# showlab/VideoSwap

Hardware: NVIDIA H100
Metric: denoise-steps/sec, 16f 512^2 SD1.5 UNet3D (CFG UNet fwd + CFG combine + DDIM step) (higher is better)
Workload: dtype f16

## Files before the change

include/videoswap_b200.h:

```cpp
#ifndef VIDEOSWAP_B200_H
#define VIDEOSWAP_B200_H
#include <stddef.h>
#include <stdint.h>

#ifdef __cplusplus
extern "C" {
#endif

const char* vs_last_error(void);
int vs_version(void);

typedef struct vs_unet_config {
  int in_channels, out_channels;
  int block_out_channels[4];
  int layers_per_block;
  int num_heads;
  int cross_attention_dim;
  int norm_num_groups;
  float norm_eps;
  int use_motion_module;
  int motion_down[4];
  int motion_up[4];
  int motion_mid;
  int motion_num_heads;
  int pe_max_len;
} vs_unet_config;

typedef struct vs_unet vs_unet;

int vs_unet_create(const vs_unet_config* cfg, vs_unet** out);
void vs_unet_destroy(vs_unet* h);

int vs_unet_load_weights(vs_unet* h, void* stream, int n, const char* const* names, const void* const* d_ptrs,
                         const int64_t* numels);
int vs_unet_num_params(const vs_unet* h);
const char* vs_unet_param_name(const vs_unet* h, int i);

int vs_unet_forward(vs_unet* h, void* stream, const void* d_sample, int io_f32, int B, int F, int H, int W,
                    const float* d_timesteps, const void* d_ehs, int ehs_tokens, int ehs_layers,
                    const void* const* d_residuals, int residuals_nhwc, float residual_scale, void* d_out);
int vs_unet_forward_features(vs_unet* h, void* stream, const void* d_sample, int io_f32, int B, int F, int H, int W,
                             const float* d_timesteps, const void* d_ehs, int ehs_tokens, int ehs_layers, int up_ft_index,
                             void* d_feat);
int vs_unet_time_embedding(vs_unet* h, void* stream, const float* d_timesteps, int B, float* d_emb, float* d_proj);
size_t vs_unet_workspace_bytes(const vs_unet* h);
int vs_unet_pin_workspace(vs_unet* h, int pin);
int vs_unet_reserve_workspace(vs_unet* h, int B, int F, int H, int W);
typedef struct vs_comm vs_comm;
int vs_comm_unique_id(void* out128);
int vs_comm_create(const void* id128, int rank, int nranks, vs_comm** out);
void vs_comm_destroy(vs_comm* c);
int vs_comm_all_gather(vs_comm* c, void* stream, const void* d_send, void* d_recv, size_t bytes_per_rank);
int vs_comm_all_reduce_sum_f32(vs_comm* c, void* stream, float* d_buf, size_t n);
int vs_unet_set_frame_shard(vs_unet* h, vs_comm* frame_comm, int shard, int nshards);

typedef void (*vs_attention_hook)(void* user, int layer, int is_cross, int place, void* d_probs, int batch, int heads, int nq,
                                  int nk, void* stream);
int vs_unet_set_attention_hook(vs_unet* h, vs_attention_hook hook, void* user, int max_queries);
int vs_attention_probs(void* stream, const void* d_q, int ldq, const void* d_k, int ldk, void* d_probs, int batch, int nq, int nk,
                       int heads, int d, long long q_bstride, long long kv_bstride, int kv_div);
int vs_attention_apply_probs(void* stream, const void* d_probs, const void* d_v, int ldv, void* d_o, int ldo, int batch, int nq,
                             int nk, int heads, int d, long long kv_bstride, long long o_bstride, int kv_div);
int vs_blend_mask(void* stream, const void* const* d_maps, int n_maps, int n_prompts, int frames, int heads, int res_h, int res_w,
                  int words, const float* d_alpha, int pool, int h, int w, float threshold, int both, float* d_mask);
int vs_latent_blend(void* stream, const void* d_x_src, void* d_x_tgt, const float* d_mask, int io_f32, int channels, int frames,
                    int hw);

int vs_unet_enable_taps(vs_unet* h, int enable);
int vs_unet_num_taps(const vs_unet* h);
int vs_unet_get_tap(const vs_unet* h, int i, const char** name, const void** d_ptr, int* nimg, int* hh, int* ww, int* c);
int vs_unet_copy_tap(const vs_unet* h, void* stream, int i, void* d_dst);

int vs_cfg_ddim_step(void* stream, const void* d_eps2, const void* d_latents, int io_f32, size_t n, int cfg,
                     float guidance, float alpha_t, float alpha_prev, void* d_out);

int vs_cfg_ddim_step_dev(void* stream, const void* d_eps2, const void* d_latents, int io_f32, size_t n, int cfg,
                         float guidance, const float* d_coef, void* d_out);

int vs_adapter_level(void* stream, const void* d_w0, const void* d_b0, const void* d_w1, const void* d_b1, int E, int mid,
                     int C, const float* d_point_embedding, const float* d_tracks, const int* d_point_mask, int F, int P,
                     int h, int w, float rate, int coord_fp16, float scale, float* d_ws, void* d_map);

typedef struct vs_gemm_desc {
  const void* A; int K1; int lda1;
  const void* A2; int K2; int lda2;
  const void* Bw;
  int M, N;
  int taps;
  int sub_py, sub_px;
  int nimg, H, W;
  const float* bias;
  const float* rowvec; int ldrv; int pix_per_batch; int rv_mod;
  const float* ln_stats; const float* ln_u;
  const float* ln_parts; int ln_nparts;
  float* ln_sums_out;
  const void* residual; int ldr;
  void* out; int ldc;
  int mode;
  int force_bn;
  int OH, OW;
  int stride2;
} vs_gemm_desc;
int vs_gemm_ex(void* stream, const vs_gemm_desc* desc);
int vs_pack_conv3x3(void* stream, const void* d_w, int cout, int cin, void* d_out);
int vs_pack_geglu(void* stream, const void* d_w, const void* d_b, int hidden, int K, void* d_wout, float* d_bout);
int vs_groupnorm(void* stream, const void* d_x1, int c1, const void* d_x2, int c2, int nimg, int hw, int imgs_per_set,
                 int groups, float eps, const float* d_gamma, const float* d_beta, int silu, float* d_sums, void* d_out);
int vs_groupnorm_stats(void* stream, const void* d_x1, int c1, const void* d_x2, int c2, int nimg, int hw, int imgs_per_set,
                       int groups, float* d_sums, int zero_first);
int vs_groupnorm_apply(void* stream, const void* d_x1, int c1, const void* d_x2, int c2, int nimg, int hw, int imgs_per_set,
                       int groups, const float* d_sums, float eps, const float* d_gamma, const float* d_beta, int silu,
                       int count_scale, void* d_out);
int vs_layernorm(void* stream, const void* d_x, int rows, int C, const float* d_gamma, const float* d_beta,
                 const float* d_pe, int hw, int F, void* d_out);
int vs_ln_linear(void* stream, const void* d_x, int M, int C, const void* d_w, const float* d_bias, int N,
                 const float* d_gamma, const float* d_beta, const float* d_pe, int pe_len, int hw, int frames, int mode,
                 void* d_wf, float* d_u, float* d_c, float* d_cpe, float* d_stats, void* d_out);
int vs_linear_ln_linear(void* stream, const void* d_x0, int M, int K0, const void* d_w0, const float* d_b0,
                        const void* d_residual, int C, void* d_x, const void* d_w, const float* d_bias, int N,
                        const float* d_gamma, const float* d_beta, const float* d_pe, int pe_len, int hw, int frames,
                        int mode, void* d_wf, float* d_u, float* d_c, float* d_cpe, float* d_parts, int parts_capacity,
                        void* d_out);
int vs_attention(void* stream, const void* d_q, int ldq, const void* d_k, int ldk, const void* d_v, int ldv, void* d_o,
                 int ldo, int batch, int nq, int nk, int heads, int d, long long q_bstride, long long kv_bstride,
                 long long o_bstride, int kv_div);
int vs_temporal_attention(void* stream, const void* d_qkv, void* d_o, int B, int F, int HW, int C, int heads);
int vs_conv_in(void* stream, const void* d_x, int nimg, int H, int W, int cin, const void* d_w, const float* d_bias,
               int cout, void* d_scratch, void* d_out);
int vs_upsample2x(void* stream, const void* d_x, int nimg, int H, int W, int C, void* d_out);
int vs_upsample_conv3x3(void* stream, const void* d_x, int nimg, int H, int W, int C, const void* d_w, int Cout,
                        const float* d_bias, void* d_wsub, void* d_out);
int vs_upsample_conv3x3_sized(void* stream, const void* d_x, int nimg, int H, int W, int C, const void* d_w, int Cout,
                              const float* d_bias, int OH, int OW, void* d_wpanels, void* d_out);
int vs_upsample_nearest(void* stream, const void* d_x, int nimg, int H, int W, int C, int OH, int OW, void* d_out);
int vs_conv3x3_s2(void* stream, const void* d_x, int nimg, int H, int W, int C, const void* d_w_packed, int Cout,
                  const float* d_bias, void* d_scratch, void* d_out);

int vs_pack_conv_subpixel(void* stream, const void* d_w, int cout, int cin, void* d_out);
int vs_softmax_rows(void* stream, void* d_s, int rows, int n, int ld, float scale);
int vs_transpose_pad(void* stream, const void* d_src, int rows, int cols, int rows_pad, void* d_dst);
int vs_vae_latent_in(void* stream, const void* d_z, int z_is_f32, int nimg, int h, int w, float divisor, const float* d_wb,
                     void* d_out);
int vs_image_postprocess(void* stream, const void* d_x, int nimg, int H, int W, int channels, int format, void* d_out);

int vs_downsample_conv3x3(void* stream, const void* d_x, int nimg, int H, int W, int C, const void* d_w_packed, int Cout,
                          const float* d_bias, void* d_out);
int vs_vae_image_in(void* stream, const void* d_x, int src_format, int nimg, int H, int W, void* d_out);
int vs_vae_moments(void* stream, const void* d_x, int nimg, int h, int w, const float* d_wb, void* d_out);
int vs_vae_posterior(void* stream, const void* d_params, const void* d_noise, int nimg, int h, int w, float scale, int layout,
                     void* d_out);

int vs_clip_embed(void* stream, const int* d_ids_i32, int n, int L, const void* d_tok, int vocab, const void* d_pos, int C,
                  void* d_out);
int vs_causal_attention(void* stream, const void* d_qkv, int ldqkv, void* d_o, int ldo, int nseq, int L, int heads, int d);

int vs_dift_noise(void* stream, const void* d_moments, const float* d_eps1, const float* d_eps2, int n, int E, int h, int w,
                  float sf, float sqrt_a, float sqrt_1ma, float* d_out);
int vs_dift_point_sample(void* stream, const void* d_feat, int n, int E, int h, int w, int C, int H, int W, const int* d_xy,
                         int P, float* d_out);
int vs_dift_ensemble_mean(void* stream, const void* d_feat, int n, int E, int h, int w, int C, float* d_out);
int vs_dift_point_reduce(void* stream, const float* d_vecs, int n, int P, int C, const float* d_src, const int* d_src_row,
                         float* d_conf, const void* d_accept, float* d_sums, float* d_counts, float* d_means);

typedef struct vs_imlp_desc {
  const float* d_params;
  int input_dim;
  int output_dim;
  int hidden_dim;
  int mlp_layers;
  int pe_dim;
  uint32_t skip_mask;
  int use_tanh;
} vs_imlp_desc;
int vs_imlp_forward(void* stream, const vs_imlp_desc* net, const float* d_x, int rows, float* d_out);
int vs_atlas_propagate(void* stream, const vs_imlp_desc* fg, const vs_imlp_desc* fg_inverse, const vs_imlp_desc* alpha,
                       const float* d_points, float t_key, int P, int F, int larger_dim, float* d_ws, float* d_tracks);

int vs_profile_enable(int on);
int vs_profile_reset(void);
int vs_profile_collect(int category, double* ms, double* work, long long* count);
long long vs_launch_count(void);
int vs_profile_dump(const char* path);
int vs_set_option(const char* name, int value);

#ifdef __cplusplus
}
#endif
#endif
```

videoswap_b200/_lib.py:

```python
from __future__ import annotations

import ctypes as C
import os
import re

HERE = os.path.dirname(os.path.abspath(__file__))
LIB_PATH = os.path.join(HERE, "libvideoswap_b200.so")
HEADER_PATH = os.path.join(os.path.dirname(HERE), "include", "videoswap_b200.h")


class VSError(RuntimeError):
    pass


class UNetConfigStruct(C.Structure):
    _fields_ = [
        ("in_channels", C.c_int), ("out_channels", C.c_int), ("block_out_channels", C.c_int * 4),
        ("layers_per_block", C.c_int), ("num_heads", C.c_int), ("cross_attention_dim", C.c_int),
        ("norm_num_groups", C.c_int), ("norm_eps", C.c_float), ("use_motion_module", C.c_int),
        ("motion_down", C.c_int * 4), ("motion_up", C.c_int * 4), ("motion_mid", C.c_int),
        ("motion_num_heads", C.c_int), ("pe_max_len", C.c_int),
    ]


_P = C.c_void_p
_I = C.c_int
_F = C.c_float
_LL = C.c_longlong
_SZ = C.c_size_t


class ImlpDescStruct(C.Structure):
    _fields_ = [("params", _P), ("input_dim", _I), ("output_dim", _I), ("hidden_dim", _I), ("mlp_layers", _I),
                ("pe_dim", _I), ("skip_mask", C.c_uint32), ("use_tanh", _I)]


class GemmDescStruct(C.Structure):
    _fields_ = [
        ("A", _P), ("K1", _I), ("lda1", _I),
        ("A2", _P), ("K2", _I), ("lda2", _I),
        ("Bw", _P),
        ("M", _I), ("N", _I),
        ("taps", _I),
        ("sub_py", _I), ("sub_px", _I),
        ("nimg", _I), ("H", _I), ("W", _I),
        ("bias", _P),
        ("rowvec", _P), ("ldrv", _I), ("pix_per_batch", _I), ("rv_mod", _I),
        ("ln_stats", _P), ("ln_u", _P),
        ("ln_parts", _P), ("ln_nparts", _I),
        ("ln_sums_out", _P),
        ("residual", _P), ("ldr", _I),
        ("out", _P), ("ldc", _I),
        ("mode", _I),
        ("force_bn", _I),
        ("OH", _I), ("OW", _I),
        ("stride2", _I),
    ]

_SIGNATURES = {
    "vs_last_error": (C.c_char_p, []),
    "vs_version": (_I, []),
    "vs_unet_create": (_I, [C.POINTER(UNetConfigStruct), C.POINTER(_P)]),
    "vs_unet_destroy": (None, [_P]),
    "vs_unet_load_weights": (_I, [_P, _P, _I, C.POINTER(C.c_char_p), C.POINTER(_P), C.POINTER(C.c_int64)]),
    "vs_unet_num_params": (_I, [_P]),
    "vs_unet_param_name": (C.c_char_p, [_P, _I]),
    "vs_unet_forward": (_I, [_P, _P, _P, _I, _I, _I, _I, _I, _P, _P, _I, _I, C.POINTER(_P), _I, _F, _P]),
    "vs_unet_time_embedding": (_I, [_P, _P, _P, _I, _P, _P]),
    "vs_unet_workspace_bytes": (_SZ, [_P]),
    "vs_unet_pin_workspace": (_I, [_P, _I]),
    "vs_unet_reserve_workspace": (_I, [_P, _I, _I, _I, _I]),
    "vs_comm_unique_id": (_I, [_P]),
    "vs_comm_create": (_I, [_P, _I, _I, C.POINTER(_P)]),
    "vs_comm_destroy": (None, [_P]),
    "vs_comm_all_gather": (_I, [_P, _P, _P, _P, _SZ]),
    "vs_comm_all_reduce_sum_f32": (_I, [_P, _P, _P, _SZ]),
    "vs_unet_set_frame_shard": (_I, [_P, _P, _I, _I]),
    "vs_unet_enable_taps": (_I, [_P, _I]),
    "vs_unet_num_taps": (_I, [_P]),
    "vs_unet_get_tap": (_I, [_P, _I, C.POINTER(C.c_char_p), C.POINTER(_P), C.POINTER(_I), C.POINTER(_I), C.POINTER(_I),
                             C.POINTER(_I)]),
    "vs_unet_copy_tap": (_I, [_P, _P, _I, _P]),
    "vs_profile_enable": (_I, [_I]),
    "vs_profile_reset": (_I, []),
    "vs_profile_collect": (_I, [_I, C.POINTER(C.c_double), C.POINTER(C.c_double), C.POINTER(C.c_longlong)]),
    "vs_launch_count": (C.c_longlong, []),
    "vs_set_option": (_I, [C.c_char_p, _I]),
    "vs_profile_dump": (_I, [C.c_char_p]),
    "vs_cfg_ddim_step": (_I, [_P, _P, _P, _I, _SZ, _I, _F, _F, _F, _P]),
    "vs_cfg_ddim_step_dev": (_I, [_P, _P, _P, _I, _SZ, _I, _F, _P, _P]),
    "vs_adapter_level": (_I, [_P, _P, _P, _P, _P, _I, _I, _I, _P, _P, _P, _I, _I, _I, _I, _F, _I, _F, _P, _P]),
    "vs_gemm_ex": (_I, [_P, C.POINTER(GemmDescStruct)]),
    "vs_pack_conv3x3": (_I, [_P, _P, _I, _I, _P]),
    "vs_pack_geglu": (_I, [_P, _P, _P, _I, _I, _P, _P]),
    "vs_groupnorm": (_I, [_P, _P, _I, _P, _I, _I, _I, _I, _I, _F, _P, _P, _I, _P, _P]),
    "vs_groupnorm_stats": (_I, [_P, _P, _I, _P, _I, _I, _I, _I, _I, _P, _I]),
    "vs_groupnorm_apply": (_I, [_P, _P, _I, _P, _I, _I, _I, _I, _I, _P, _F, _P, _P, _I, _I, _P]),
    "vs_layernorm": (_I, [_P, _P, _I, _I, _P, _P, _P, _I, _I, _P]),
    "vs_ln_linear": (_I, [_P, _P, _I, _I, _P, _P, _I, _P, _P, _P, _I, _I, _I, _I, _P, _P, _P, _P, _P, _P]),
    "vs_unet_set_attention_hook": (_I, [_P, _P, _P, _I]),
    "vs_attention_probs": (_I, [_P, _P, _I, _P, _I, _P, _I, _I, _I, _I, _I, _LL, _LL, _I]),
    "vs_attention_apply_probs": (_I, [_P, _P, _P, _I, _P, _I, _I, _I, _I, _I, _I, _LL, _LL, _I]),
    "vs_blend_mask": (_I, [_P, _P, _I, _I, _I, _I, _I, _I, _I, _P, _I, _I, _I, _F, _I, _P]),
    "vs_latent_blend": (_I, [_P, _P, _P, _P, _I, _I, _I, _I]),
    "vs_linear_ln_linear": (_I, [_P, _P, _I, _I, _P, _P, _P, _I, _P, _P, _P, _I, _P, _P, _P, _I, _I, _I, _I, _P, _P, _P, _P,
                                 _P, _I, _P]),
    "vs_attention": (_I, [_P, _P, _I, _P, _I, _P, _I, _P, _I, _I, _I, _I, _I, _I, _LL, _LL, _LL, _I]),
    "vs_temporal_attention": (_I, [_P, _P, _P, _I, _I, _I, _I, _I]),
    "vs_conv_in": (_I, [_P, _P, _I, _I, _I, _I, _P, _P, _I, _P, _P]),
    "vs_upsample2x": (_I, [_P, _P, _I, _I, _I, _I, _P]),
    "vs_upsample_conv3x3": (_I, [_P, _P, _I, _I, _I, _I, _P, _I, _P, _P, _P]),
    "vs_upsample_conv3x3_sized": (_I, [_P, _P, _I, _I, _I, _I, _P, _I, _P, _I, _I, _P, _P]),
    "vs_upsample_nearest": (_I, [_P, _P, _I, _I, _I, _I, _I, _I, _P]),
    "vs_conv3x3_s2": (_I, [_P, _P, _I, _I, _I, _I, _P, _I, _P, _P, _P]),
    "vs_pack_conv_subpixel": (_I, [_P, _P, _I, _I, _P]),
    "vs_softmax_rows": (_I, [_P, _P, _I, _I, _I, _F]),
    "vs_transpose_pad": (_I, [_P, _P, _I, _I, _I, _P]),
    "vs_vae_latent_in": (_I, [_P, _P, _I, _I, _I, _I, _F, _P, _P]),
    "vs_image_postprocess": (_I, [_P, _P, _I, _I, _I, _I, _I, _P]),
    "vs_downsample_conv3x3": (_I, [_P, _P, _I, _I, _I, _I, _P, _I, _P, _P]),
    "vs_vae_image_in": (_I, [_P, _P, _I, _I, _I, _I, _P]),
    "vs_vae_moments": (_I, [_P, _P, _I, _I, _I, _P, _P]),
    "vs_vae_posterior": (_I, [_P, _P, _P, _I, _I, _I, _F, _I, _P]),
    "vs_clip_embed": (_I, [_P, _P, _I, _I, _P, _I, _P, _I, _P]),
    "vs_causal_attention": (_I, [_P, _P, _I, _P, _I, _I, _I, _I, _I]),
    "vs_unet_forward_features": (_I, [_P, _P, _P, _I, _I, _I, _I, _I, _P, _P, _I, _I, _I, _P]),
    "vs_dift_noise": (_I, [_P, _P, _P, _P, _I, _I, _I, _I, _F, _F, _F, _P]),
    "vs_dift_point_sample": (_I, [_P, _P, _I, _I, _I, _I, _I, _I, _I, _P, _I, _P]),
    "vs_dift_ensemble_mean": (_I, [_P, _P, _I, _I, _I, _I, _I, _P]),
    "vs_dift_point_reduce": (_I, [_P, _P, _I, _I, _I, _P, _P, _P, _P, _P, _P, _P]),
    "vs_imlp_forward": (_I, [_P, C.POINTER(ImlpDescStruct), _P, _I, _P]),
    "vs_atlas_propagate": (_I, [_P, C.POINTER(ImlpDescStruct), C.POINTER(ImlpDescStruct), C.POINTER(ImlpDescStruct), _P, _F,
                                _I, _I, _I, _P, _P]),
}

_lib = None


def header_symbols():
    with open(HEADER_PATH) as f:
        text = f.read()
    text = re.sub(r"/\*.*?\*/", "", text, flags=re.S)
    return sorted(set(re.findall(r"\b(vs_[a-z0-9_]+)\s*\(", text)))


def lib() -> C.CDLL:
    global _lib
    if _lib is None:
        if not os.path.exists(LIB_PATH):
            raise VSError(f"{LIB_PATH} is missing: build it with `python -m videoswap_b200.build` "
                          f"(there is no CPU/PyTorch fallback for this path)")
        _lib = C.CDLL(LIB_PATH)
        for name, (res, args) in _SIGNATURES.items():
            fn = getattr(_lib, name)
            fn.restype = res
            fn.argtypes = args
    return _lib


def check(code: int, what: str = ""):
    if code != 0:
        msg = lib().vs_last_error()
        raise VSError(f"{what or 'videoswap_b200 call'} failed ({code}): {msg.decode() if msg else '?'}")


def call(name: str, *args):
    check(getattr(lib(), name)(*args), name)
```

videoswap_b200/build.py:

```python
from __future__ import annotations

import os
import shutil
import subprocess
import sys
from concurrent.futures import ThreadPoolExecutor

HERE = os.path.dirname(os.path.abspath(__file__))
CSRC = os.path.join(HERE, "csrc")
LIB = os.path.join(HERE, "libvideoswap_b200.so")
SOURCES = ["runtime.cu", "gemm.cu", "norm.cu", "attention.cu", "attention_tc.cu", "pointwise.cu", "unet.cu", "api.cu", "comm.cu", "text.cu", "dift.cu", "atlas.cu"]
ARCH = ["-gencode", "arch=compute_90a,code=sm_90a"]
NVCC_FLAGS = ARCH + ["-lineinfo", "-O3", "-std=c++17", "-Xcompiler", "-fPIC",
              "--use_fast_math" if False else "-DVS_NO_FAST_MATH"]


def _nvcc() -> str:
    for cand in (os.environ.get("NVCC"), shutil.which("nvcc"), "/usr/local/cuda/bin/nvcc"):
        if cand and os.path.exists(cand):
            return cand
    raise RuntimeError("nvcc not found")


def _stale(target: str, deps) -> bool:
    if not os.path.exists(target):
        return True
    t = os.path.getmtime(target)
    return any(os.path.getmtime(d) > t for d in deps)


def build(force: bool = False, verbose: bool = False) -> str:
    nvcc = _nvcc()
    objdir = os.path.join(HERE, "build")
    os.makedirs(objdir, exist_ok=True)
    headers = [os.path.join(CSRC, f) for f in os.listdir(CSRC) if f.endswith((".h", ".cuh"))]
    headers.append(os.path.join(os.path.dirname(HERE), "include", "videoswap_b200.h"))

    def compile_one(src):
        obj = os.path.join(objdir, src.replace(".cu", ".o"))
        if force or _stale(obj, [os.path.join(CSRC, src)] + headers):
            cmd = [nvcc] + NVCC_FLAGS + ["-c", os.path.join(CSRC, src), "-o", obj]
            if verbose:
                print(" ".join(cmd))
            r = subprocess.run(cmd, capture_output=True, text=True)
            if r.returncode != 0:
                raise RuntimeError(f"nvcc failed on {src}:\n{r.stdout}\n{r.stderr}")
        return obj

    with ThreadPoolExecutor(max_workers=min(8, len(SOURCES))) as ex:
        objs = list(ex.map(compile_one, SOURCES))
    if force or _stale(LIB, objs):
        cmd = [nvcc, "-shared", "-o", LIB] + objs + ARCH + ["-Xcompiler", "-fPIC", "-ldl"]
        r = subprocess.run(cmd, capture_output=True, text=True)
        if r.returncode != 0:
            raise RuntimeError(f"link failed:\n{r.stdout}\n{r.stderr}")
    return LIB


if __name__ == "__main__":
    print(build(force="--force" in sys.argv, verbose=True))
```

videoswap_b200/csrc/api.cu:

```cuda
#include "../../include/videoswap_b200.h"
#include "common.cuh"
#include "kernels.h"

using namespace vs;

extern "C" const char* vs_last_error(void) { return vs::last_error(); }
extern "C" int vs_version(void) { return 100; }

extern "C" int vs_cfg_ddim_step(void* stream, const void* d_eps2, const void* d_latents, int io_f32, size_t n, int cfg,
                                float guidance, float alpha_t, float alpha_prev, void* d_out) {
  VS_REQUIRE(d_eps2 && d_latents && d_out, "vs_cfg_ddim_step: null pointer");
  VS_REQUIRE(alpha_t > 0.f && alpha_t <= 1.f && alpha_prev > 0.f && alpha_prev <= 1.f, "vs_cfg_ddim_step: alphas must be in (0,1]");
  return cfg_ddim_step((cudaStream_t)stream, d_eps2, d_latents, io_f32, n, cfg, guidance, alpha_t, alpha_prev, d_out);
}

extern "C" int vs_cfg_ddim_step_dev(void* stream, const void* d_eps2, const void* d_latents, int io_f32, size_t n, int cfg,
                                    float guidance, const float* d_coef, void* d_out) {
  VS_REQUIRE(d_eps2 && d_latents && d_out && d_coef, "vs_cfg_ddim_step_dev: null pointer");
  return cfg_ddim_step_dev((cudaStream_t)stream, d_eps2, d_latents, io_f32, n, cfg, guidance, d_coef, d_out);
}

extern "C" int vs_adapter_level(void* stream, const void* d_w0, const void* d_b0, const void* d_w1, const void* d_b1, int E,
                                int mid, int C, const float* d_pe, const float* d_tracks, const int* d_mask, int F, int P,
                                int h, int w, float rate, int coord_fp16, float scale, float* d_ws, void* d_map) {
  cudaStream_t st = (cudaStream_t)stream;
  VS_REQUIRE(d_w0 && d_b0 && d_w1 && d_b1 && d_pe && d_tracks && d_ws && d_map, "vs_adapter_level: null pointer");
  float* b0 = d_ws;
  float* b1 = b0 + mid;
  float* hid = b1 + C;
  float* feat = hid + (size_t)P * mid;
  if (int e = f16_to_f32(st, (const __half*)d_b0, mid, b0)) return e;
  if (int e = f16_to_f32(st, (const __half*)d_b1, C, b1)) return e;
  if (int e = small_linear(st, d_pe, P, E, (const __half*)d_w0, b0, mid, false, true, hid)) return e;
  if (int e = small_linear(st, hid, P, mid, (const __half*)d_w1, b1, C, false, false, feat)) return e;
  return adapter_splat(st, feat, d_tracks, d_mask, F, P, C, h, w, rate, coord_fp16, scale, (__half*)d_map);
}

extern "C" int vs_gemm_ex(void* stream, const vs_gemm_desc* d) {
  VS_REQUIRE(d != nullptr, "vs_gemm_ex: null descriptor");
  GemmArgs g;
  g.A = (const __half*)d->A; g.K1 = d->K1; g.lda1 = d->lda1;
  g.A2 = (const __half*)d->A2; g.K2 = d->K2; g.lda2 = d->lda2;
  g.Bw = (const __half*)d->Bw;
  g.M = d->M; g.N = d->N;
  g.taps = d->taps;
  g.sub_py = d->sub_py; g.sub_px = d->sub_px;
  g.nimg = d->nimg; g.H = d->H; g.W = d->W;
  g.bias = d->bias;
  g.rowvec = d->rowvec; g.ldrv = d->ldrv; g.pix_per_batch = d->pix_per_batch; g.rv_mod = d->rv_mod;
  g.ln_stats = d->ln_stats; g.ln_u = d->ln_u;
  g.ln_parts = d->ln_parts; g.ln_nparts = d->ln_nparts;
  g.ln_sums_out = d->ln_sums_out;
  g.residual = (const __half*)d->residual; g.ldr = d->ldr;
  g.out = (__half*)d->out; g.ldc = d->ldc;
  g.mode = d->mode;
  g.force_bn = d->force_bn;
  g.OH = d->OH; g.OW = d->OW;
  g.stride2 = d->stride2;
  return gemm_tc((cudaStream_t)stream, g);
}

extern "C" int vs_pack_conv3x3(void* stream, const void* d_w, int cout, int cin, void* d_out) {
  return pack_conv3x3((cudaStream_t)stream, (const __half*)d_w, cout, cin, (__half*)d_out);
}
extern "C" int vs_pack_geglu(void* stream, const void* d_w, const void* d_b, int hidden, int K, void* d_wout, float* d_bout) {
  cudaStream_t st = (cudaStream_t)stream;
  if (int e = pack_geglu(st, (const __half*)d_w, nullptr, hidden, K, kGegluGranule, (__half*)d_wout, nullptr)) return e;
  return pack_geglu(st, nullptr, (const __half*)d_b, hidden, 1, kGegluGranule, nullptr, d_bout);
}

extern "C" int vs_groupnorm(void* stream, const void* d_x1, int c1, const void* d_x2, int c2, int nimg, int hw,
                            int imgs_per_set, int groups, float eps, const float* d_gamma, const float* d_beta, int silu,
                            float* d_sums, void* d_out) {
  cudaStream_t st = (cudaStream_t)stream;
  if (imgs_per_set == 1 && c2 == 0) {
    const int e = groupnorm_frame_fused(st, (const __half*)d_x1, c1, nimg, hw, groups, eps, d_gamma, d_beta, silu != 0, (__half*)d_out);
    if (e >= 0) return e;
  }
  if (int e = groupnorm_stats(st, (const __half*)d_x1, c1, (const __half*)d_x2, c2, nimg, hw, imgs_per_set, groups, d_sums)) return e;
  return groupnorm_apply(st, (const __half*)d_x1, c1, (const __half*)d_x2, c2, nimg, hw, imgs_per_set, groups, d_sums, eps,
                         d_gamma, d_beta, silu != 0, (__half*)d_out);
}
extern "C" int vs_groupnorm_stats(void* stream, const void* d_x1, int c1, const void* d_x2, int c2, int nimg, int hw,
                                  int imgs_per_set, int groups, float* d_sums, int zero_first) {
  VS_REQUIRE(d_sums != nullptr, "vs_groupnorm_stats: null sums");
  return groupnorm_stats((cudaStream_t)stream, (const __half*)d_x1, c1, (const __half*)d_x2, c2, nimg, hw, imgs_per_set, groups,
                         d_sums, zero_first != 0);
}
extern "C" int vs_groupnorm_apply(void* stream, const void* d_x1, int c1, const void* d_x2, int c2, int nimg, int hw,
                                  int imgs_per_set, int groups, const float* d_sums, float eps, const float* d_gamma,
                                  const float* d_beta, int silu, int count_scale, void* d_out) {
  VS_REQUIRE(d_sums && d_out, "vs_groupnorm_apply: null pointer");
  VS_REQUIRE(count_scale >= 1, "vs_groupnorm_apply: count_scale must be >= 1");
  return groupnorm_apply((cudaStream_t)stream, (const __half*)d_x1, c1, (const __half*)d_x2, c2, nimg, hw, imgs_per_set, groups,
                         d_sums, eps, d_gamma, d_beta, silu != 0, (__half*)d_out, count_scale);
}
extern "C" int vs_layernorm(void* stream, const void* d_x, int rows, int C, const float* d_gamma, const float* d_beta,
                            const float* d_pe, int hw, int F, void* d_out) {
  return layernorm((cudaStream_t)stream, (const __half*)d_x, rows, C, d_gamma, d_beta, d_pe, hw, F, (__half*)d_out);
}
extern "C" int vs_ln_linear(void* stream, const void* d_x, int M, int C, const void* d_w, const float* d_bias, int N,
                            const float* d_gamma, const float* d_beta, const float* d_pe, int pe_len, int hw, int frames,
                            int mode, void* d_wf, float* d_u, float* d_c, float* d_cpe, float* d_stats, void* d_out) {
  cudaStream_t st = (cudaStream_t)stream;
  if (int e = ln_fold(st, (const __half*)d_w, N, C, d_gamma, d_beta, d_bias, d_pe, pe_len, (__half*)d_wf, d_u, d_c, d_cpe)) return e;
  if (int e = ln_rowstats(st, (const __half*)d_x, M, C, d_stats)) return e;
  GemmArgs g;
  g.A = (const __half*)d_x; g.K1 = C; g.lda1 = C; g.Bw = (const __half*)d_wf; g.M = M; g.N = N; g.bias = d_c;
  g.ln_stats = d_stats; g.ln_u = d_u; g.out = (__half*)d_out; g.ldc = mode == EPI_GEGLU ? N / 2 : N; g.mode = mode;
  if (d_pe) { g.rowvec = d_cpe; g.ldrv = N; g.pix_per_batch = hw; g.rv_mod = frames; }
  return gemm_tc(st, g);
}
extern "C" int vs_upsample_conv3x3(void* stream, const void* d_x, int nimg, int H, int W, int C, const void* d_w, int Cout,
                                   const float* d_bias, void* d_wsub, void* d_out) {
  cudaStream_t st = (cudaStream_t)stream;
  if (int e = pack_conv_subpixel(st, (const __half*)d_w, Cout, C, (__half*)d_wsub)) return e;
  for (int par = 0; par < 4; ++par) {
    GemmArgs g;
    g.A = (const __half*)d_x; g.K1 = C; g.lda1 = C; g.Bw = (const __half*)d_wsub + (size_t)par * Cout * 4 * C; g.taps = 4;
    g.sub_py = par >> 1; g.sub_px = par & 1; g.nimg = nimg; g.H = H; g.W = W; g.M = nimg * H * W; g.N = Cout; g.bias = d_bias;
    g.out = (__half*)d_out; g.ldc = Cout;
    if (int e = gemm_tc(st, g)) return e;
  }
  return 0;
}
extern "C" int vs_upsample_conv3x3_sized(void* stream, const void* d_x, int nimg, int H, int W, int C, const void* d_w, int Cout,
                                         const float* d_bias, int OH, int OW, void* d_wpanels, void* d_out) {
  cudaStream_t st = (cudaStream_t)stream;
  VS_REQUIRE(d_x && d_w && d_wpanels && d_out && nimg >= 1 && H >= 1 && W >= 1, "vs_upsample_conv3x3_sized: bad arguments");
  __half* w3x3 = (__half*)d_wpanels;
  __half* wsub = w3x3 + (size_t)Cout * 9 * C;
  if (int e = pack_conv3x3(st, (const __half*)d_w, Cout, C, w3x3)) return e;
  if (int e = pack_conv_subpixel(st, (const __half*)d_w, Cout, C, wsub, true)) return e;
  return upsample_conv3x3(st, (const __half*)d_x, nimg, H, W, C, w3x3, wsub, d_bias, Cout, OH, OW, (__half*)d_out);
}
extern "C" int vs_upsample_nearest(void* stream, const void* d_x, int nimg, int H, int W, int C, int OH, int OW, void* d_out) {
  return upsample_nearest2x((cudaStream_t)stream, (const __half*)d_x, nimg, H, W, C, (__half*)d_out, OH, OW);
}
extern "C" int vs_attention_probs(void* stream, const void* d_q, int ldq, const void* d_k, int ldk, void* d_probs, int batch, int nq,
                                  int nk, int heads, int d, long long q_bstride, long long kv_bstride, int kv_div) {
  return attention_probs((cudaStream_t)stream, (const __half*)d_q, ldq, (const __half*)d_k, ldk, (__half*)d_probs, batch, nq, nk, heads,
                         d, q_bstride, kv_bstride, kv_div);
}
extern "C" int vs_attention_apply_probs(void* stream, const void* d_probs, const void* d_v, int ldv, void* d_o, int ldo, int batch,
                                        int nq, int nk, int heads, int d, long long kv_bstride, long long o_bstride, int kv_div) {
  return attention_apply_probs((cudaStream_t)stream, (const __half*)d_probs, (const __half*)d_v, ldv, (__half*)d_o, ldo, batch, nq, nk,
                               heads, d, kv_bstride, o_bstride, kv_div);
}
extern "C" int vs_blend_mask(void* stream, const void* const* d_maps, int n_maps, int n_prompts, int frames, int heads, int res_h,
                             int res_w, int words, const float* d_alpha, int pool, int h, int w, float threshold, int both,
                             float* d_mask) {
  const int res[2] = {res_h, res_w};
  return blend_mask((cudaStream_t)stream, (const __half* const*)d_maps, res, n_maps, n_prompts, frames, heads, words, d_alpha, pool, h, w,
                    threshold, both, d_mask);
}
extern "C" int vs_latent_blend(void* stream, const void* d_x_src, void* d_x_tgt, const float* d_mask, int io_f32, int channels,
                               int frames, int hw) {
  return latent_blend((cudaStream_t)stream, d_x_src, d_x_tgt, d_mask, io_f32, channels, frames, hw);
}
extern "C" int vs_linear_ln_linear(void* stream, const void* d_x0, int M, int K0, const void* d_w0, const float* d_b0,
                                   const void* d_residual, int C, void* d_x, const void* d_w, const float* d_bias, int N,
                                   const float* d_gamma, const float* d_beta, const float* d_pe, int pe_len, int hw,
                                   int frames, int mode, void* d_wf, float* d_u, float* d_c, float* d_cpe, float* d_parts,
                                   int parts_capacity, void* d_out) {
  cudaStream_t st = (cudaStream_t)stream;
  if (int e = ln_fold(st, (const __half*)d_w, N, C, d_gamma, d_beta, d_bias, d_pe, pe_len, (__half*)d_wf, d_u, d_c, d_cpe)) return e;
  GemmArgs g0;
  g0.A = (const __half*)d_x0; g0.K1 = K0; g0.lda1 = K0; g0.Bw = (const __half*)d_w0; g0.M = M; g0.N = C; g0.bias = d_b0;
  g0.residual = (const __half*)d_residual; g0.ldr = C; g0.out = (__half*)d_x; g0.ldc = C; g0.ln_sums_out = d_parts;
  const int parts = gemm_n_tiles(g0);
  VS_REQUIRE(parts >= 1 && parts <= parts_capacity, "vs_linear_ln_linear: %d partial-sum slices do not fit the buffer (%d)", parts, parts_capacity);
  if (int e = gemm_tc(st, g0)) return e;
  GemmArgs g;
  g.A = (const __half*)d_x; g.K1 = C; g.lda1 = C; g.Bw = (const __half*)d_wf; g.M = M; g.N = N; g.bias = d_c;
  g.ln_parts = d_parts; g.ln_nparts = parts; g.ln_u = d_u; g.out = (__half*)d_out; g.ldc = mode == EPI_GEGLU ? N / 2 : N; g.mode = mode;
  if (d_pe) { g.rowvec = d_cpe; g.ldrv = N; g.pix_per_batch = hw; g.rv_mod = frames; }
  return gemm_tc(st, g);
}
extern "C" int vs_attention(void* stream, const void* d_q, int ldq, const void* d_k, int ldk, const void* d_v, int ldv,
                            void* d_o, int ldo, int batch, int nq, int nk, int heads, int d, long long q_bstride,
                            long long kv_bstride, long long o_bstride, int kv_div) {
  return attention((cudaStream_t)stream, (const __half*)d_q, ldq, (const __half*)d_k, ldk, (const __half*)d_v, ldv,
                   (__half*)d_o, ldo, batch, nq, nk, heads, d, q_bstride, kv_bstride, o_bstride, kv_div);
}
extern "C" int vs_temporal_attention(void* stream, const void* d_qkv, void* d_o, int B, int F, int HW, int C, int heads) {
  return temporal_attention((cudaStream_t)stream, (const __half*)d_qkv, (__half*)d_o, B, F, HW, C, heads);
}
extern "C" int vs_conv_in(void* stream, const void* d_x, int nimg, int H, int W, int cin, const void* d_w, const float* d_bias,
                          int cout, void* d_scratch, void* d_out) {
  return conv_in_3x3((cudaStream_t)stream, (const __half*)d_x, nimg, H, W, cin, (const __half*)d_w, d_bias, cout, (__half*)d_out,
                     (__half*)d_scratch);
}
extern "C" int vs_upsample2x(void* stream, const void* d_x, int nimg, int H, int W, int C, void* d_out) {
  return upsample_nearest2x((cudaStream_t)stream, (const __half*)d_x, nimg, H, W, C, (__half*)d_out);
}
extern "C" int vs_conv3x3_s2(void* stream, const void* d_x, int nimg, int H, int W, int C, const void* d_w, int Cout,
                             const float* d_bias, void* d_scratch, void* d_out) {
  cudaStream_t st = (cudaStream_t)stream;
  if (int e = im2col_s2(st, (const __half*)d_x, nimg, H, W, C, (__half*)d_scratch)) return e;
  const int Ho = (H - 1) / 2 + 1, Wo = (W - 1) / 2 + 1;
  GemmArgs g;
  g.A = (const __half*)d_scratch; g.K1 = 9 * C; g.lda1 = 9 * C; g.Bw = (const __half*)d_w; g.M = nimg * Ho * Wo; g.N = Cout;
  g.bias = d_bias; g.out = (__half*)d_out; g.ldc = Cout;
  return gemm_tc(st, g);
}

extern "C" int vs_pack_conv_subpixel(void* stream, const void* d_w, int cout, int cin, void* d_out) {
  VS_REQUIRE(d_w && d_out, "vs_pack_conv_subpixel: null pointer");
  return pack_conv_subpixel((cudaStream_t)stream, (const __half*)d_w, cout, cin, (__half*)d_out);
}
extern "C" int vs_softmax_rows(void* stream, void* d_s, int rows, int n, int ld, float scale) {
  return softmax_rows((cudaStream_t)stream, (__half*)d_s, rows, n, ld, scale);
}
extern "C" int vs_transpose_pad(void* stream, const void* d_src, int rows, int cols, int rows_pad, void* d_dst) {
  return transpose_pad((cudaStream_t)stream, (const __half*)d_src, rows, cols, rows_pad, (__half*)d_dst);
}
extern "C" int vs_vae_latent_in(void* stream, const void* d_z, int z_is_f32, int nimg, int h, int w, float divisor,
                                const float* d_wb, void* d_out) {
  return vae_latent_in((cudaStream_t)stream, d_z, z_is_f32, nimg, h, w, divisor, d_wb, (__half*)d_out);
}
extern "C" int vs_image_postprocess(void* stream, const void* d_x, int nimg, int H, int W, int channels, int format, void* d_out) {
  return image_postprocess((cudaStream_t)stream, (const __half*)d_x, nimg, H, W, channels, format, d_out);
}
extern "C" int vs_downsample_conv3x3(void* stream, const void* d_x, int nimg, int H, int W, int C, const void* d_w_packed,
                                     int Cout, const float* d_bias, void* d_out) {
  VS_REQUIRE(d_x && d_w_packed && d_out, "vs_downsample_conv3x3: null pointer");
  GemmArgs g;
  g.A = (const __half*)d_x; g.K1 = C; g.lda1 = C; g.Bw = (const __half*)d_w_packed; g.taps = 9; g.stride2 = 1;
  g.nimg = nimg; g.H = H; g.W = W; g.M = nimg * (H / 2) * (W / 2); g.N = Cout; g.bias = d_bias; g.out = (__half*)d_out;
  g.ldc = Cout;
  return gemm_tc((cudaStream_t)stream, g);
}
extern "C" int vs_vae_image_in(void* stream, const void* d_x, int src_format, int nimg, int H, int W, void* d_out) {
  return vae_image_in((cudaStream_t)stream, d_x, src_format, nimg, H, W, (__half*)d_out);
}
extern "C" int vs_vae_moments(void* stream, const void* d_x, int nimg, int h, int w, const float* d_wb, void* d_out) {
  return vae_moments((cudaStream_t)stream, (const __half*)d_x, nimg, h, w, d_wb, (__half*)d_out);
}
extern "C" int vs_vae_posterior(void* stream, const void* d_params, const void* d_noise, int nimg, int h, int w, float scale,
                                int layout, void* d_out) {
  return vae_posterior((cudaStream_t)stream, (const __half*)d_params, (const __half*)d_noise, nimg, h, w, scale, layout,
                       (__half*)d_out);
}
extern "C" int vs_clip_embed(void* stream, const int* d_ids_i32, int n, int L, const void* d_tok, int vocab, const void* d_pos, int C,
                             void* d_out) {
  return clip_embed((cudaStream_t)stream, d_ids_i32, n, L, (const __half*)d_tok, vocab, (const __half*)d_pos, C, (__half*)d_out);
}
extern "C" int vs_causal_attention(void* stream, const void* d_qkv, int ldqkv, void* d_o, int ldo, int nseq, int L, int heads,
                                   int d) {
  return causal_attention((cudaStream_t)stream, (const __half*)d_qkv, ldqkv, (__half*)d_o, ldo, nseq, L, heads, d);
}

extern "C" int vs_dift_noise(void* stream, const void* d_moments, const float* d_eps1, const float* d_eps2, int n, int E, int h,
                             int w, float sf, float sqrt_a, float sqrt_1ma, float* d_out) {
  return dift_noise((cudaStream_t)stream, (const __half*)d_moments, d_eps1, d_eps2, n, E, h, w, sf, sqrt_a, sqrt_1ma, d_out);
}
extern "C" int vs_dift_point_sample(void* stream, const void* d_feat, int n, int E, int h, int w, int C, int H, int W,
                                    const int* d_xy, int P, float* d_out) {
  return dift_point_sample((cudaStream_t)stream, (const __half*)d_feat, n, E, h, w, C, H, W, d_xy, P, d_out);
}
extern "C" int vs_dift_ensemble_mean(void* stream, const void* d_feat, int n, int E, int h, int w, int C, float* d_out) {
  return dift_ensemble_mean((cudaStream_t)stream, (const __half*)d_feat, n, E, h, w, C, d_out);
}
extern "C" int vs_dift_point_reduce(void* stream, const float* d_vecs, int n, int P, int C, const float* d_src,
                                    const int* d_src_row, float* d_conf, const void* d_accept, float* d_sums, float* d_counts,
                                    float* d_means) {
  return dift_point_reduce((cudaStream_t)stream, d_vecs, n, P, C, d_src, d_src_row, d_conf, (const uint8_t*)d_accept, d_sums,
                           d_counts, d_means);
}

extern "C" int vs_profile_enable(int on) { prof_enable(on != 0); return 0; }
extern "C" int vs_profile_reset(void) { prof_reset(); return 0; }
extern "C" int vs_profile_collect(int category, double* ms, double* work, long long* count) {
  VS_REQUIRE(category >= 0 && category < PC_COUNT && ms && work && count, "vs_profile_collect: bad argument");
  return prof_collect(category, ms, work, count);
}
extern "C" long long vs_launch_count(void) { return launch_count(); }
extern "C" int vs_profile_dump(const char* path) {
  VS_REQUIRE(path != nullptr, "vs_profile_dump: null path");
  return prof_dump(path);
}
extern "C" int vs_set_option(const char* name, int value) {
  VS_REQUIRE(name != nullptr, "vs_set_option: null name");
  return set_option(name, value);
}
```

videoswap_b200/csrc/attention.cu:

```cuda
#include "common.cuh"
#include "kernels.h"

namespace vs {
namespace {

__device__ __forceinline__ void cp_async16(uint32_t dst, const void* src, bool pred) {
  const int sz = pred ? 16 : 0;
  asm volatile("cp.async.cg.shared.global [%0], [%1], 16, %2;" ::"r"(dst), "l"(src), "r"(sz) : "memory");
}
__device__ __forceinline__ void cp_async_commit() { asm volatile("cp.async.commit_group;" ::: "memory"); }
template <int N>
__device__ __forceinline__ void cp_async_wait() {
  asm volatile("cp.async.wait_group %0;" ::"n"(N) : "memory");
}
__device__ __forceinline__ void ldsm_x4(uint32_t addr, uint32_t& r0, uint32_t& r1, uint32_t& r2, uint32_t& r3) {
  asm volatile("ldmatrix.sync.aligned.m8n8.x4.shared.b16 {%0,%1,%2,%3}, [%4];"
               : "=r"(r0), "=r"(r1), "=r"(r2), "=r"(r3)
               : "r"(addr));
}
__device__ __forceinline__ void ldsm_x4_t(uint32_t addr, uint32_t& r0, uint32_t& r1, uint32_t& r2, uint32_t& r3) {
  asm volatile("ldmatrix.sync.aligned.m8n8.x4.trans.shared.b16 {%0,%1,%2,%3}, [%4];"
               : "=r"(r0), "=r"(r1), "=r"(r2), "=r"(r3)
               : "r"(addr));
}
__device__ __forceinline__ void mma16816(float* c, const uint32_t* a, uint32_t b0, uint32_t b1) {
  asm volatile(
      "mma.sync.aligned.m16n8k16.row.col.f32.f16.f16.f32 {%0,%1,%2,%3}, {%4,%5,%6,%7}, {%8,%9}, {%0,%1,%2,%3};"
      : "+f"(c[0]), "+f"(c[1]), "+f"(c[2]), "+f"(c[3])
      : "r"(a[0]), "r"(a[1]), "r"(a[2]), "r"(a[3]), "r"(b0), "r"(b1));
}
__device__ __forceinline__ uint32_t pack_h2(float a, float b) {
  __half2 h = __floats2half2_rn(a, b);
  return *reinterpret_cast<uint32_t*>(&h);
}

template <int DP, int NT>
__device__ __forceinline__ void warp_qk(float (*s)[4], uint32_t q_s, uint32_t k_s, int lds_bytes, int lane) {
#pragma unroll
  for (int n = 0; n < NT; ++n) s[n][0] = s[n][1] = s[n][2] = s[n][3] = 0.f;
#pragma unroll
  for (int kk = 0; kk < DP / 16; ++kk) {
    uint32_t a[4];
    ldsm_x4(q_s + (lane & 15) * lds_bytes + (kk * 16 + (lane >> 4) * 8) * 2, a[0], a[1], a[2], a[3]);
#pragma unroll
    for (int n = 0; n < NT; n += 2) {
      uint32_t b0, b1, b2, b3;
      const int key = n * 8 + (lane & 7) + ((lane >> 4) ? 8 : 0);
      const int ch = kk * 16 + (((lane >> 3) & 1) ? 8 : 0);
      ldsm_x4(k_s + key * lds_bytes + ch * 2, b0, b1, b2, b3);
      mma16816(s[n], a, b0, b1);
      mma16816(s[n + 1], a, b2, b3);
    }
  }
}

template <int NT, int ON>
__device__ __forceinline__ void warp_pv(float (*o)[4], const float (*s)[4], uint32_t v_s, int lds_bytes, int lane) {
#pragma unroll
  for (int kt = 0; kt < NT / 2; ++kt) {
    uint32_t a[4];
    a[0] = pack_h2(s[2 * kt][0], s[2 * kt][1]);
    a[1] = pack_h2(s[2 * kt][2], s[2 * kt][3]);
    a[2] = pack_h2(s[2 * kt + 1][0], s[2 * kt + 1][1]);
    a[3] = pack_h2(s[2 * kt + 1][2], s[2 * kt + 1][3]);
#pragma unroll
    for (int n = 0; n < ON; n += 2) {
      uint32_t b0, b1, b2, b3;
      const int key = kt * 16 + (lane & 7) + (((lane >> 3) & 1) ? 8 : 0);
      const int ch = n * 8 + ((lane >> 4) ? 8 : 0);
      ldsm_x4_t(v_s + key * lds_bytes + ch * 2, b0, b1, b2, b3);
      mma16816(o[n], a, b0, b1);
      mma16816(o[n + 1], a, b2, b3);
    }
  }
}

struct AttnParams {
  const __half* q; const __half* k; const __half* v; __half* o;
  int ldq, ldk, ldv, ldo;
  long long q_bs, kv_bs, o_bs;
  int nq, nk, kv_div;
  float scale_log2;
};

template <int D>
struct ACfg {
  static constexpr int DP = (D + 15) / 16 * 16;
  static constexpr int LDS = DP + 8;
  static constexpr int BQ = 64, BKV = 64;
  static constexpr int SMEM = (BQ + 4 * BKV) * LDS * 2;
};

template <int D>
__device__ __forceinline__ void load_rows(uint32_t dst, const __half* src, int ld, int row0, int nrows_valid, int tid,
                                          int nthreads) {
  using C = ACfg<D>;
  constexpr int CH = C::DP / 8;
  for (int i = tid; i < 64 * CH; i += nthreads) {
    const int r = i / CH, c = i % CH;
    const bool ok = (row0 + r < nrows_valid) && (c * 8 < D);
    const __half* s = ok ? src + (long long)(row0 + r) * ld + c * 8 : src;
    cp_async16(dst + (r * C::LDS + c * 8) * 2, s, ok);
  }
}

template <int D>
__global__ void __launch_bounds__(128) attn_kernel(const AttnParams p) {
  using C = ACfg<D>;
  pdl_trigger();
  pdl_wait();
  constexpr int DP = C::DP, LDSB = C::LDS * 2, NT = C::BKV / 8, ON = DP / 8;
  extern __shared__ __align__(16) uint8_t smem[];
  const uint32_t q_s = smem_u32(smem);
  const uint32_t k_s0 = q_s + C::BQ * LDSB;
  const uint32_t v_s0 = k_s0 + 2 * C::BKV * LDSB;
  const int tid = threadIdx.x, warp = tid >> 5, lane = tid & 31;
  const int qt = blockIdx.x, h = blockIdx.y, b = blockIdx.z;
  const __half* qp = p.q + b * p.q_bs + h * D;
  const __half* kp = p.k + (b / p.kv_div) * p.kv_bs + h * D;
  const __half* vp = p.v + (b / p.kv_div) * p.kv_bs + h * D;
  const int nkt = (p.nk + C::BKV - 1) / C::BKV;

  load_rows<D>(q_s, qp, p.ldq, qt * C::BQ, p.nq, tid, 128);
  load_rows<D>(k_s0, kp, p.ldk, 0, p.nk, tid, 128);
  load_rows<D>(v_s0, vp, p.ldv, 0, p.nk, tid, 128);
  cp_async_commit();

  float o[ON][4];
#pragma unroll
  for (int n = 0; n < ON; ++n) o[n][0] = o[n][1] = o[n][2] = o[n][3] = 0.f;
  float m0 = -INFINITY, m1 = -INFINITY, l0 = 0.f, l1 = 0.f;

  for (int j = 0; j < nkt; ++j) {
    cp_async_wait<0>();
    __syncthreads();
    if (j + 1 < nkt) {
      const int nb = (j + 1) & 1;
      load_rows<D>(k_s0 + nb * C::BKV * LDSB, kp, p.ldk, (j + 1) * C::BKV, p.nk, tid, 128);
      load_rows<D>(v_s0 + nb * C::BKV * LDSB, vp, p.ldv, (j + 1) * C::BKV, p.nk, tid, 128);
      cp_async_commit();
    }
    const uint32_t k_s = k_s0 + (j & 1) * C::BKV * LDSB;
    const uint32_t v_s = v_s0 + (j & 1) * C::BKV * LDSB;
    float s[NT][4];
    warp_qk<DP, NT>(s, q_s + warp * 16 * LDSB, k_s, LDSB, lane);
    const int kbase = j * C::BKV;
    if (kbase + C::BKV > p.nk) {
#pragma unroll
      for (int n = 0; n < NT; ++n) {
        const int c = kbase + n * 8 + (lane & 3) * 2;
        if (c >= p.nk) s[n][0] = s[n][2] = -INFINITY;
        if (c + 1 >= p.nk) s[n][1] = s[n][3] = -INFINITY;
      }
    }
    float mx0 = m0, mx1 = m1;
#pragma unroll
    for (int n = 0; n < NT; ++n) {
      mx0 = fmaxf(mx0, fmaxf(s[n][0], s[n][1]));
      mx1 = fmaxf(mx1, fmaxf(s[n][2], s[n][3]));
    }
    mx0 = fmaxf(mx0, __shfl_xor_sync(0xffffffffu, mx0, 1));
    mx0 = fmaxf(mx0, __shfl_xor_sync(0xffffffffu, mx0, 2));
    mx1 = fmaxf(mx1, __shfl_xor_sync(0xffffffffu, mx1, 1));
    mx1 = fmaxf(mx1, __shfl_xor_sync(0xffffffffu, mx1, 2));
    const float c0 = exp2f((m0 - mx0) * p.scale_log2), c1 = exp2f((m1 - mx1) * p.scale_log2);
    m0 = mx0; m1 = mx1;
    const float ms0 = mx0 * p.scale_log2, ms1 = mx1 * p.scale_log2;
    float rs0 = 0.f, rs1 = 0.f;
#pragma unroll
    for (int n = 0; n < NT; ++n) {
      s[n][0] = exp2f(s[n][0] * p.scale_log2 - ms0);
      s[n][1] = exp2f(s[n][1] * p.scale_log2 - ms0);
      s[n][2] = exp2f(s[n][2] * p.scale_log2 - ms1);
      s[n][3] = exp2f(s[n][3] * p.scale_log2 - ms1);
      rs0 += s[n][0] + s[n][1];
      rs1 += s[n][2] + s[n][3];
    }
    l0 = l0 * c0 + rs0;
    l1 = l1 * c1 + rs1;
#pragma unroll
    for (int n = 0; n < ON; ++n) {
      o[n][0] *= c0; o[n][1] *= c0; o[n][2] *= c1; o[n][3] *= c1;
    }
    warp_pv<NT, ON>(o, s, v_s, LDSB, lane);
  }
  l0 += __shfl_xor_sync(0xffffffffu, l0, 1);
  l0 += __shfl_xor_sync(0xffffffffu, l0, 2);
  l1 += __shfl_xor_sync(0xffffffffu, l1, 1);
  l1 += __shfl_xor_sync(0xffffffffu, l1, 2);
  const float i0 = 1.f / l0, i1 = 1.f / l1;
  const int r0 = qt * C::BQ + warp * 16 + (lane >> 2), r1 = r0 + 8;
  __half* op = p.o + b * p.o_bs + h * D;
#pragma unroll
  for (int n = 0; n < ON; ++n) {
    const int c = n * 8 + (lane & 3) * 2;
    if (c < D) {
      if (r0 < p.nq) *reinterpret_cast<__half2*>(op + (long long)r0 * p.ldo + c) = __floats2half2_rn(o[n][0] * i0, o[n][1] * i0);
      if (r1 < p.nq) *reinterpret_cast<__half2*>(op + (long long)r1 * p.ldo + c) = __floats2half2_rn(o[n][2] * i1, o[n][3] * i1);
    }
  }
}

template <int D>
int launch_attn(cudaStream_t st, const AttnParams& p, int batch, int heads) {
  using C = ACfg<D>;
  static bool configured = false;
  if (!configured) {
    VS_CHECK_CUDA(cudaFuncSetAttribute(attn_kernel<D>, cudaFuncAttributeMaxDynamicSharedMemorySize, C::SMEM));
    configured = true;
  }
  dim3 grid((p.nq + C::BQ - 1) / C::BQ, heads, batch);
  ProfScope prof(st, PC_ATTN, 4.0 * batch * heads * (double)p.nq * p.nk * D);
  return launch_pdl(attn_kernel<D>, grid, dim3(128), C::SMEM, st, 1, p);
}

template <int D>
__global__ void __launch_bounds__(128) attn_probs_kernel(const AttnParams p, __half* __restrict__ probs, int heads) {
  using C = ACfg<D>;
  constexpr int DP = C::DP, LDSB = C::LDS * 2, NT = C::BKV / 8;
  extern __shared__ __align__(16) uint8_t smem[];
  const uint32_t q_s = smem_u32(smem);
  const uint32_t k_s0 = q_s + C::BQ * LDSB;
  const int tid = threadIdx.x, warp = tid >> 5, lane = tid & 31;
  const int qt = blockIdx.x, h = blockIdx.y, b = blockIdx.z;
  const __half* qp = p.q + b * p.q_bs + h * D;
  const __half* kp = p.k + (b / p.kv_div) * p.kv_bs + h * D;
  const int nkt = (p.nk + C::BKV - 1) / C::BKV;
  load_rows<D>(q_s, qp, p.ldq, qt * C::BQ, p.nq, tid, 128);
  float m0 = -INFINITY, m1 = -INFINITY, l0 = 0.f, l1 = 0.f, i0 = 0.f, i1 = 0.f;
  const int r0 = qt * C::BQ + warp * 16 + (lane >> 2), r1 = r0 + 8;
  __half* prow0 = probs + (((long long)b * heads + h) * p.nq + r0) * p.nk;
  __half* prow1 = prow0 + 8LL * p.nk;
  for (int pass = 0; pass < 2; ++pass) {
    load_rows<D>(k_s0, kp, p.ldk, 0, p.nk, tid, 128);
    cp_async_commit();
    for (int j = 0; j < nkt; ++j) {
      cp_async_wait<0>();
      __syncthreads();
      if (j + 1 < nkt) {
        load_rows<D>(k_s0 + ((j + 1) & 1) * C::BKV * LDSB, kp, p.ldk, (j + 1) * C::BKV, p.nk, tid, 128);
        cp_async_commit();
      }
      float s[NT][4];
      warp_qk<DP, NT>(s, q_s + warp * 16 * LDSB, k_s0 + (j & 1) * C::BKV * LDSB, LDSB, lane);
      const int kbase = j * C::BKV;
      if (pass == 0) {
        float mx0 = m0, mx1 = m1;
#pragma unroll
        for (int n = 0; n < NT; ++n) {
          const int c = kbase + n * 8 + (lane & 3) * 2;
          if (c >= p.nk) s[n][0] = s[n][2] = -INFINITY;
          if (c + 1 >= p.nk) s[n][1] = s[n][3] = -INFINITY;
          mx0 = fmaxf(mx0, fmaxf(s[n][0], s[n][1]));
          mx1 = fmaxf(mx1, fmaxf(s[n][2], s[n][3]));
        }
        mx0 = fmaxf(mx0, __shfl_xor_sync(0xffffffffu, mx0, 1));
        mx0 = fmaxf(mx0, __shfl_xor_sync(0xffffffffu, mx0, 2));
        mx1 = fmaxf(mx1, __shfl_xor_sync(0xffffffffu, mx1, 1));
        mx1 = fmaxf(mx1, __shfl_xor_sync(0xffffffffu, mx1, 2));
        float rs0 = 0.f, rs1 = 0.f;
#pragma unroll
        for (int n = 0; n < NT; ++n) {
          rs0 += exp2f((s[n][0] - mx0) * p.scale_log2) + exp2f((s[n][1] - mx0) * p.scale_log2);
          rs1 += exp2f((s[n][2] - mx1) * p.scale_log2) + exp2f((s[n][3] - mx1) * p.scale_log2);
        }
        l0 = l0 * exp2f((m0 - mx0) * p.scale_log2) + rs0;
        l1 = l1 * exp2f((m1 - mx1) * p.scale_log2) + rs1;
        m0 = mx0; m1 = mx1;
      } else {
#pragma unroll
        for (int n = 0; n < NT; ++n) {
          const int c = kbase + n * 8 + (lane & 3) * 2;
          if (r0 < p.nq) {
            if (c < p.nk) prow0[c] = __float2half_rn(exp2f((s[n][0] - m0) * p.scale_log2) * i0);
            if (c + 1 < p.nk) prow0[c + 1] = __float2half_rn(exp2f((s[n][1] - m0) * p.scale_log2) * i0);
          }
          if (r1 < p.nq) {
            if (c < p.nk) prow1[c] = __float2half_rn(exp2f((s[n][2] - m1) * p.scale_log2) * i1);
            if (c + 1 < p.nk) prow1[c + 1] = __float2half_rn(exp2f((s[n][3] - m1) * p.scale_log2) * i1);
          }
        }
      }
      __syncthreads();
    }
    if (pass == 0) {
      l0 += __shfl_xor_sync(0xffffffffu, l0, 1);
      l0 += __shfl_xor_sync(0xffffffffu, l0, 2);
      l1 += __shfl_xor_sync(0xffffffffu, l1, 1);
      l1 += __shfl_xor_sync(0xffffffffu, l1, 2);
      i0 = 1.f / l0; i1 = 1.f / l1;
    }
  }
}

template <int D>
__global__ void __launch_bounds__(128) attn_pv_kernel(const AttnParams p, const __half* __restrict__ probs, int heads) {
  using C = ACfg<D>;
  constexpr int DP = C::DP, LDSB = C::LDS * 2, ON = DP / 8, LDP = C::BKV + 8, LDPB = LDP * 2;
  extern __shared__ __align__(16) uint8_t smem[];
  const uint32_t p_s = smem_u32(smem);
  const uint32_t v_s = p_s + C::BQ * LDPB;
  __half* p_sm = reinterpret_cast<__half*>(smem);
  const int tid = threadIdx.x, warp = tid >> 5, lane = tid & 31;
  const int qt = blockIdx.x, h = blockIdx.y, b = blockIdx.z;
  const __half* vp = p.v + (b / p.kv_div) * p.kv_bs + h * D;
  const __half* pb = probs + (((long long)b * heads + h) * p.nq) * p.nk;
  const int nkt = (p.nk + C::BKV - 1) / C::BKV;
  float o[ON][4];
#pragma unroll
  for (int n = 0; n < ON; ++n) o[n][0] = o[n][1] = o[n][2] = o[n][3] = 0.f;
  for (int j = 0; j < nkt; ++j) {
    __syncthreads();
    load_rows<D>(v_s, vp, p.ldv, j * C::BKV, p.nk, tid, 128);
    cp_async_commit();
    for (int e = tid; e < C::BQ * C::BKV; e += 128) {
      const int r = e / C::BKV, c = e % C::BKV;
      const int q = qt * C::BQ + r, k = j * C::BKV + c;
      p_sm[r * LDP + c] = (q < p.nq && k < p.nk) ? pb[(long long)q * p.nk + k] : __float2half(0.f);
    }
    cp_async_wait<0>();
    __syncthreads();
#pragma unroll
    for (int kt = 0; kt < C::BKV / 16; ++kt) {
      uint32_t a[4];
      ldsm_x4(p_s + (warp * 16 + (lane & 15)) * LDPB + (kt * 16 + (lane >> 4) * 8) * 2, a[0], a[1], a[2], a[3]);
#pragma unroll
      for (int n = 0; n < ON; n += 2) {
        uint32_t b0, b1, b2, b3;
        const int key = kt * 16 + (lane & 7) + (((lane >> 3) & 1) ? 8 : 0);
        const int ch = n * 8 + ((lane >> 4) ? 8 : 0);
        ldsm_x4_t(v_s + key * LDSB + ch * 2, b0, b1, b2, b3);
        mma16816(o[n], a, b0, b1);
        mma16816(o[n + 1], a, b2, b3);
      }
    }
  }
  const int r0 = qt * C::BQ + warp * 16 + (lane >> 2), r1 = r0 + 8;
  __half* op = p.o + b * p.o_bs + h * D;
#pragma unroll
  for (int n = 0; n < ON; ++n) {
    const int c = n * 8 + (lane & 3) * 2;
    if (c < D) {
      if (r0 < p.nq) *reinterpret_cast<__half2*>(op + (long long)r0 * p.ldo + c) = __floats2half2_rn(o[n][0], o[n][1]);
      if (r1 < p.nq) *reinterpret_cast<__half2*>(op + (long long)r1 * p.ldo + c) = __floats2half2_rn(o[n][2], o[n][3]);
    }
  }
}

template <int D>
int launch_explicit(cudaStream_t st, const AttnParams& p, __half* probs, int batch, int heads, bool apply) {
  using C = ACfg<D>;
  constexpr int SMEM_P = (C::BQ + 2 * C::BKV) * C::LDS * 2;
  constexpr int SMEM_V = C::BQ * (C::BKV + 8) * 2 + C::BKV * C::LDS * 2;
  static bool configured = false;
  if (!configured) {
    VS_CHECK_CUDA(cudaFuncSetAttribute(attn_probs_kernel<D>, cudaFuncAttributeMaxDynamicSharedMemorySize, SMEM_P));
    VS_CHECK_CUDA(cudaFuncSetAttribute(attn_pv_kernel<D>, cudaFuncAttributeMaxDynamicSharedMemorySize, SMEM_V));
    configured = true;
  }
  dim3 grid((p.nq + C::BQ - 1) / C::BQ, heads, batch);
  ProfScope prof(st, PC_ATTN, 2.0 * batch * heads * (double)p.nq * p.nk * D);
  if (apply) attn_pv_kernel<D><<<grid, 128, SMEM_V, st>>>(p, probs, heads);
  else attn_probs_kernel<D><<<grid, 128, SMEM_P, st>>>(p, probs, heads);
  count_launch(1);
  VS_CHECK_CUDA(cudaGetLastError());
  return 0;
}

struct TAttnParams {
  const __half* qkv; __half* o;
  int B, F, HW, C, heads;
  float scale_log2;
  long long items;
};

template <int D, int FP, bool VST = true>
__global__ void __launch_bounds__(128) tattn_kernel(const TAttnParams p) {
  pdl_trigger();
  pdl_wait();
  constexpr int DP = (D + 15) / 16 * 16, LDS = DP + 8, LDSB = LDS * 2, CH = DP / 8;
  constexpr int MT = FP / 16, NT = FP / 8, ON = DP / 8;
  extern __shared__ __align__(16) uint8_t smem[];
  const int warp = threadIdx.x >> 5, lane = threadIdx.x & 31;
  const long long item = (long long)blockIdx.x * 4 + warp;
  if (item >= p.items) return;
  const int head = item % p.heads;
  const long long bp = item / p.heads;
  const int pix = bp % p.HW;
  const int b = bp / p.HW;
  const uint32_t base = smem_u32(smem) + warp * (3 * FP * LDSB);
  const uint32_t q_s = base, k_s = base + FP * LDSB, v_s = base + 2 * FP * LDSB;
  const long long row_stride = (long long)p.HW * 3 * p.C;
  const __half* src = p.qkv + ((long long)b * p.F * p.HW + pix) * 3 * p.C + head * D;
  for (int i = lane; i < 3 * FP * CH; i += 32) {
    const int sec = i / (FP * CH), rem = i % (FP * CH), f = rem / CH, c = rem % CH;
    const bool ok = (f < p.F) && (c * 8 < D);
    const __half* s = ok ? src + f * row_stride + sec * p.C + c * 8 : src;
    cp_async16(base + sec * FP * LDSB + (f * LDS + c * 8) * 2, s, ok);
  }
  cp_async_commit();
  cp_async_wait<0>();
  __syncwarp();
  __half* dst = p.o + ((long long)b * p.F * p.HW + pix) * p.C + head * D;
  const long long orow = (long long)p.HW * p.C;
#pragma unroll
  for (int mt = 0; mt < MT; ++mt) {
    float s[NT][4];
    warp_qk<DP, NT>(s, q_s + mt * 16 * LDSB, k_s, LDSB, lane);
    float mx0 = -INFINITY, mx1 = -INFINITY;
#pragma unroll
    for (int n = 0; n < NT; ++n) {
      const int c = n * 8 + (lane & 3) * 2;
      if (c >= p.F) s[n][0] = s[n][2] = -INFINITY;
      if (c + 1 >= p.F) s[n][1] = s[n][3] = -INFINITY;
      mx0 = fmaxf(mx0, fmaxf(s[n][0], s[n][1]));
      mx1 = fmaxf(mx1, fmaxf(s[n][2], s[n][3]));
    }
    mx0 = fmaxf(mx0, __shfl_xor_sync(0xffffffffu, mx0, 1));
    mx0 = fmaxf(mx0, __shfl_xor_sync(0xffffffffu, mx0, 2));
    mx1 = fmaxf(mx1, __shfl_xor_sync(0xffffffffu, mx1, 1));
    mx1 = fmaxf(mx1, __shfl_xor_sync(0xffffffffu, mx1, 2));
    const float ms0 = mx0 * p.scale_log2, ms1 = mx1 * p.scale_log2;
    float l0 = 0.f, l1 = 0.f;
#pragma unroll
    for (int n = 0; n < NT; ++n) {
      s[n][0] = exp2f(s[n][0] * p.scale_log2 - ms0);
      s[n][1] = exp2f(s[n][1] * p.scale_log2 - ms0);
      s[n][2] = exp2f(s[n][2] * p.scale_log2 - ms1);
      s[n][3] = exp2f(s[n][3] * p.scale_log2 - ms1);
      l0 += s[n][0] + s[n][1];
      l1 += s[n][2] + s[n][3];
    }
    l0 += __shfl_xor_sync(0xffffffffu, l0, 1);
    l0 += __shfl_xor_sync(0xffffffffu, l0, 2);
    l1 += __shfl_xor_sync(0xffffffffu, l1, 1);
    l1 += __shfl_xor_sync(0xffffffffu, l1, 2);
    float o[ON][4];
#pragma unroll
    for (int n = 0; n < ON; ++n) o[n][0] = o[n][1] = o[n][2] = o[n][3] = 0.f;
    warp_pv<NT, ON>(o, s, v_s, LDSB, lane);
    const float i0 = 1.f / l0, i1 = 1.f / l1;
    const int f0 = mt * 16 + (lane >> 2), f1 = f0 + 8;
    if (VST) {
      __syncwarp();
      __half* stage = reinterpret_cast<__half*>(smem) + (size_t)warp * (3 * FP * LDS) + (size_t)mt * 16 * LDS;
#pragma unroll
      for (int n = 0; n < ON; ++n) {
        const int c = n * 8 + (lane & 3) * 2;
        *reinterpret_cast<__half2*>(stage + (lane >> 2) * LDS + c) = __floats2half2_rn(o[n][0] * i0, o[n][1] * i0);
        *reinterpret_cast<__half2*>(stage + ((lane >> 2) + 8) * LDS + c) = __floats2half2_rn(o[n][2] * i1, o[n][3] * i1);
      }
      __syncwarp();
      constexpr int VCH = D / 8;
      for (int e = lane; e < 16 * VCH; e += 32) {
        const int fr = e / VCH, ch = e % VCH, f = mt * 16 + fr;
        if (f < p.F) *reinterpret_cast<uint4*>(dst + f * orow + ch * 8) = *reinterpret_cast<const uint4*>(stage + fr * LDS + ch * 8);
      }
    } else {
#pragma unroll
      for (int n = 0; n < ON; ++n) {
        const int c = n * 8 + (lane & 3) * 2;
        if (c < D) {
          if (f0 < p.F) *reinterpret_cast<__half2*>(dst + f0 * orow + c) = __floats2half2_rn(o[n][0] * i0, o[n][1] * i0);
          if (f1 < p.F) *reinterpret_cast<__half2*>(dst + f1 * orow + c) = __floats2half2_rn(o[n][2] * i1, o[n][3] * i1);
        }
      }
    }
  }
}

template <int D, int FP>
int launch_tattn(cudaStream_t st, const TAttnParams& p) {
  constexpr int DP = (D + 15) / 16 * 16;
  constexpr int SMEM = 4 * 3 * FP * (DP + 8) * 2;
  static bool configured = false;
  if (!configured) {
    VS_CHECK_CUDA(cudaFuncSetAttribute(tattn_kernel<D, FP, true>, cudaFuncAttributeMaxDynamicSharedMemorySize, SMEM));
    VS_CHECK_CUDA(cudaFuncSetAttribute(tattn_kernel<D, FP, false>, cudaFuncAttributeMaxDynamicSharedMemorySize, SMEM));
    configured = true;
  }
  const long long blocks = (p.items + 3) / 4;
  ProfScope prof(st, PC_TATTN, 8.0 * p.B * p.F * (double)p.HW * p.C);
  if (get_option("tattn_vst") == 0) return launch_pdl(tattn_kernel<D, FP, false>, dim3((unsigned)blocks), dim3(128), SMEM, st, 1, p);
  return launch_pdl(tattn_kernel<D, FP, true>, dim3((unsigned)blocks), dim3(128), SMEM, st, 1, p);
}

constexpr int kSoftmaxThreads = 256;

__device__ __forceinline__ float block_reduce(float v, bool is_max, float* red) {
#pragma unroll
  for (int o = 16; o > 0; o >>= 1) {
    const float w = __shfl_xor_sync(0xffffffffu, v, o);
    v = is_max ? fmaxf(v, w) : v + w;
  }
  const int lane = threadIdx.x & 31, warp = threadIdx.x >> 5;
  __syncthreads();
  if (lane == 0) red[warp] = v;
  __syncthreads();
  v = red[0];
  for (int i = 1; i < kSoftmaxThreads / 32; ++i) v = is_max ? fmaxf(v, red[i]) : v + red[i];
  return v;
}

__global__ void __launch_bounds__(kSoftmaxThreads) softmax_rows_kernel(__half* __restrict__ s, int n, int ld, float sc) {
  __shared__ float red[kSoftmaxThreads / 32];
  uint4* row = reinterpret_cast<uint4*>(s + (long long)blockIdx.x * ld);
  const int nv = ld / 8;
  float m = -INFINITY;
  for (int v = threadIdx.x; v < nv; v += kSoftmaxThreads) {
    const uint4 x = row[v];
    const __half* h = reinterpret_cast<const __half*>(&x);
#pragma unroll
    for (int j = 0; j < 8; ++j)
      if (v * 8 + j < n) m = fmaxf(m, __half2float(h[j]));
  }
  m = block_reduce(m, true, red);
  float l = 0.f;
  for (int v = threadIdx.x; v < nv; v += kSoftmaxThreads) {
    const uint4 x = row[v];
    const __half* h = reinterpret_cast<const __half*>(&x);
#pragma unroll
    for (int j = 0; j < 8; ++j)
      if (v * 8 + j < n) l += exp2f((__half2float(h[j]) - m) * sc);
  }
  l = block_reduce(l, false, red);
  for (int v = threadIdx.x; v < nv; v += kSoftmaxThreads) {
    const uint4 x = row[v];
    const __half* h = reinterpret_cast<const __half*>(&x);
    uint4 o;
    __half* oh = reinterpret_cast<__half*>(&o);
#pragma unroll
    for (int j = 0; j < 8; ++j)
      oh[j] = v * 8 + j < n ? __float2half_rn(exp2f((__half2float(h[j]) - m) * sc) / l) : __float2half_rn(0.f);
    row[v] = o;
  }
}

__global__ void transpose_pad_kernel(const __half* __restrict__ src, int rows, int cols, int rows_pad, __half* __restrict__ dst) {
  __shared__ __half tile[32][33];
  const int r0 = blockIdx.x * 32, c0 = blockIdx.y * 32;
  for (int j = threadIdx.y; j < 32; j += blockDim.y) {
    const int r = r0 + j, c = c0 + threadIdx.x;
    if (c < cols) tile[j][threadIdx.x] = r < rows ? src[(long long)r * cols + c] : __float2half_rn(0.f);
  }
  __syncthreads();
  for (int j = threadIdx.y; j < 32; j += blockDim.y) {
    const int c = c0 + j, r = r0 + threadIdx.x;
    if (c < cols && r < rows_pad) dst[(long long)c * rows_pad + r] = tile[threadIdx.x][j];
  }
}

}

int attention(cudaStream_t st, const __half* q, int ldq, const __half* k, int ldk, const __half* v, int ldv, __half* o,
              int ldo, int batch, int nq, int nk, int heads, int d, long long q_bstride, long long kv_bstride,
              long long o_bstride, int kv_div) {
  VS_REQUIRE(nq > 0 && nk > 0 && batch > 0, "attention: empty problem");
  VS_REQUIRE((ldq % 8 | ldk % 8 | ldv % 8 | ldo % 2) == 0 && d % 8 == 0, "attention: unaligned leading dims");
  if (get_option("attn_tc") && (d == 40 || d == 80)) {
    const int e = attention_tc(st, q, ldq, k, ldk, v, ldv, o, ldo, batch, nq, nk, heads, d, q_bstride, kv_bstride, o_bstride,
                               kv_div > 0 ? kv_div : 1);
    if (e != -1) return e;
  }
  AttnParams p{q, k, v, o, ldq, ldk, ldv, ldo, q_bstride, kv_bstride, o_bstride, nq, nk, kv_div > 0 ? kv_div : 1,
               1.4426950408889634f / sqrtf((float)d)};
  switch (d) {
    case 40: return launch_attn<40>(st, p, batch, heads);
    case 80: return launch_attn<80>(st, p, batch, heads);
    case 160: return launch_attn<160>(st, p, batch, heads);
    default: VS_REQUIRE(false, "attention: unsupported head dim %d (supported: 40, 80, 160)", d);
  }
}

int attention_probs(cudaStream_t st, const __half* q, int ldq, const __half* k, int ldk, __half* probs, int batch, int nq, int nk,
                    int heads, int d, long long q_bstride, long long kv_bstride, int kv_div) {
  VS_REQUIRE(nq > 0 && nk > 0 && batch > 0 && probs, "attention_probs: empty problem");
  VS_REQUIRE((ldq % 8 | ldk % 8) == 0 && d % 8 == 0, "attention_probs: unaligned leading dims");
  AttnParams p{q, k, nullptr, nullptr, ldq, ldk, 0, 0, q_bstride, kv_bstride, 0, nq, nk, kv_div > 0 ? kv_div : 1,
               1.4426950408889634f / sqrtf((float)d)};
  switch (d) {
    case 40: return launch_explicit<40>(st, p, probs, batch, heads, false);
    case 80: return launch_explicit<80>(st, p, probs, batch, heads, false);
    case 160: return launch_explicit<160>(st, p, probs, batch, heads, false);
    default: VS_REQUIRE(false, "attention_probs: unsupported head dim %d (supported: 40, 80, 160)", d);
  }
}
int attention_apply_probs(cudaStream_t st, const __half* probs, const __half* v, int ldv, __half* o, int ldo, int batch, int nq,
                          int nk, int heads, int d, long long kv_bstride, long long o_bstride, int kv_div) {
  VS_REQUIRE(nq > 0 && nk > 0 && batch > 0 && probs, "attention_apply_probs: empty problem");
  VS_REQUIRE((ldv % 8 | ldo % 2) == 0 && d % 8 == 0, "attention_apply_probs: unaligned leading dims");
  AttnParams p{nullptr, nullptr, v, o, 0, 0, ldv, ldo, 0, kv_bstride, o_bstride, nq, nk, kv_div > 0 ? kv_div : 1, 0.f};
  switch (d) {
    case 40: return launch_explicit<40>(st, p, const_cast<__half*>(probs), batch, heads, true);
    case 80: return launch_explicit<80>(st, p, const_cast<__half*>(probs), batch, heads, true);
    case 160: return launch_explicit<160>(st, p, const_cast<__half*>(probs), batch, heads, true);
    default: VS_REQUIRE(false, "attention_apply_probs: unsupported head dim %d (supported: 40, 80, 160)", d);
  }
}

int temporal_attention(cudaStream_t st, const __half* qkv, __half* o, int B, int F, int HW, int C, int heads) {
  VS_REQUIRE(F >= 1 && F <= 32, "temporal_attention: F=%d out of range (1..32)", F);
  VS_REQUIRE(C % heads == 0, "temporal_attention: C %% heads != 0");
  const int d = C / heads;
  TAttnParams p{qkv, o, B, F, HW, C, heads, 1.4426950408889634f / sqrtf((float)d), (long long)B * HW * heads};
  const bool big = F > 16;
  switch (d) {
    case 40: return big ? launch_tattn<40, 32>(st, p) : launch_tattn<40, 16>(st, p);
    case 80: return big ? launch_tattn<80, 32>(st, p) : launch_tattn<80, 16>(st, p);
    case 160: return big ? launch_tattn<160, 32>(st, p) : launch_tattn<160, 16>(st, p);
    default: VS_REQUIRE(false, "temporal_attention: unsupported head dim %d", d);
  }
}

int softmax_rows(cudaStream_t st, __half* s, int rows, int n, int ld, float scale) {
  VS_REQUIRE(s && rows > 0 && n > 0 && n <= ld && ld % 8 == 0, "softmax_rows: bad shape (rows %d, n %d, ld %d)", rows, n, ld);
  ProfScope prof(st, PC_ATTN, 5.0 * rows * (double)n);
  softmax_rows_kernel<<<rows, kSoftmaxThreads, 0, st>>>(s, n, ld, 1.4426950408889634f * scale);
  VS_CHECK_CUDA(cudaGetLastError());
  return 0;
}

int transpose_pad(cudaStream_t st, const __half* src, int rows, int cols, int rows_pad, __half* dst) {
  VS_REQUIRE(src && dst && rows > 0 && cols > 0 && rows_pad >= rows, "transpose_pad: bad shape (%d x %d, pad %d)", rows, cols, rows_pad);
  ProfScope prof(st, PC_OTHER, 2.0 * ((double)rows + rows_pad) * cols);
  transpose_pad_kernel<<<dim3((rows_pad + 31) / 32, (cols + 31) / 32), dim3(32, 8), 0, st>>>(src, rows, cols, rows_pad, dst);
  VS_CHECK_CUDA(cudaGetLastError());
  return 0;
}

}
```

videoswap_b200/csrc/kernels.h:

```cpp
#pragma once
#include <cuda_fp16.h>
#include <cuda_runtime.h>
#include <stdint.h>

namespace vs {

enum EpiMode { EPI_LINEAR = 0, EPI_GEGLU = 1, EPI_QUICK_GELU = 2 };

struct GemmArgs {
  const __half* A = nullptr;  int K1 = 0;  int lda1 = 0;
  const __half* A2 = nullptr; int K2 = 0;  int lda2 = 0;
  const __half* Bw = nullptr;
  int M = 0, N = 0;
  int taps = 1;
  int sub_py = 0, sub_px = 0;
  int nimg = 0, H = 0, W = 0;
  const float* bias = nullptr;
  const float* rowvec = nullptr;
  int ldrv = 0;
  int pix_per_batch = 1;
  int rv_mod = 0;
  const float* ln_stats = nullptr;
  const float* ln_u = nullptr;
  const float* ln_parts = nullptr;
  int ln_nparts = 0;
  float* ln_sums_out = nullptr;
  const __half* residual = nullptr; int ldr = 0;
  __half* out = nullptr; int ldc = 0;
  int mode = EPI_LINEAR;
  int force_bn = 0;
  int OH = 0, OW = 0;
  int stride2 = 0;
};
int gemm_tc(cudaStream_t st, const GemmArgs& a);
int gemm_n_tiles(const GemmArgs& a);
constexpr int kGegluGranule = 128;

int groupnorm_stats(cudaStream_t st, const __half* x1, int c1, const __half* x2, int c2, int nimg, int hw,
                    int imgs_per_set, int groups, float* sums, bool zero_first = true);
int groupnorm_apply(cudaStream_t st, const __half* x1, int c1, const __half* x2, int c2, int nimg, int hw,
                    int imgs_per_set, int groups, const float* sums, float eps, const float* gamma,
                    const float* beta, bool silu, __half* out, int count_scale = 1);
int groupnorm_frame_fused(cudaStream_t st, const __half* x, int C, int nimg, int hw, int groups, float eps, const float* gamma,
                          const float* beta, bool silu, __half* out);
int layernorm(cudaStream_t st, const __half* x, int rows, int C, const float* gamma, const float* beta,
              const float* pe, int hw, int F, __half* out);

bool ln_fold_supported(int C);
int ln_rowstats(cudaStream_t st, const __half* x, long long rows, int C, float* stats);
int ln_fold(cudaStream_t st, const __half* w, int N, int K, const float* gamma, const float* beta, const float* bias,
            const float* pe, int pe_len, __half* wf, float* u, float* c, float* cpe);

int attention(cudaStream_t st, const __half* q, int ldq, const __half* k, int ldk, const __half* v, int ldv,
              __half* o, int ldo, int batch, int nq, int nk, int heads, int d, long long q_bstride,
              long long kv_bstride, long long o_bstride, int kv_div);
int attention_tc(cudaStream_t st, const __half* q, int ldq, const __half* k, int ldk, const __half* v, int ldv,
                 __half* o, int ldo, int batch, int nq, int nk, int heads, int d, long long q_bstride,
                 long long kv_bstride, long long o_bstride, int kv_div);
int attention_probs(cudaStream_t st, const __half* q, int ldq, const __half* k, int ldk, __half* probs, int batch, int nq, int nk,
                    int heads, int d, long long q_bstride, long long kv_bstride, int kv_div);
int attention_apply_probs(cudaStream_t st, const __half* probs, const __half* v, int ldv, __half* o, int ldo, int batch, int nq,
                          int nk, int heads, int d, long long kv_bstride, long long o_bstride, int kv_div);
int set_option(const char* name, int value);
int get_option(const char* name);
int temporal_attention(cudaStream_t st, const __half* qkv, __half* o, int B, int F, int HW, int C, int heads);
int softmax_rows(cudaStream_t st, __half* s, int rows, int n, int ld, float scale);
int transpose_pad(cudaStream_t st, const __half* src, int rows, int cols, int rows_pad, __half* dst);

int clip_embed(cudaStream_t st, const int* ids, int n, int L, const __half* tok, int vocab, const __half* pos, int C,
               __half* out);
int causal_attention(cudaStream_t st, const __half* qkv, int ldqkv, __half* o, int ldo, int nseq, int L, int heads, int d);

int dift_noise(cudaStream_t st, const __half* moments, const float* eps1, const float* eps2, int n, int E, int h, int w,
               float sf, float sqrt_a, float sqrt_1ma, float* out);
int dift_point_sample(cudaStream_t st, const __half* feat, int n, int E, int h, int w, int C, int H, int W, const int* xy,
                      int P, float* out);
int dift_ensemble_mean(cudaStream_t st, const __half* feat, int n, int E, int h, int w, int C, float* out);
int dift_point_reduce(cudaStream_t st, const float* vecs, int n, int P, int C, const float* src, const int* src_row,
                      float* conf, const uint8_t* accept, float* sums, float* counts, float* means);

int small_linear(cudaStream_t st, const float* x, int rows, int K, const __half* W, const float* bias, int N,
                 bool silu_in, bool silu_out, float* out);
int timestep_embedding(cudaStream_t st, const float* t, int B, int dim, float* out);
int conv_in_3x3(cudaStream_t st, const __half* x, int nimg, int H, int W, int cin, const __half* w, const float* bias,
                int cout, __half* out, __half* scratch = nullptr);
int upsample_nearest2x(cudaStream_t st, const __half* x, int nimg, int H, int W, int C, __half* out, int OH = 0, int OW = 0);
int im2col_s2(cudaStream_t st, const __half* x, int nimg, int H, int W, int C, __half* out);
int add_inplace(cudaStream_t st, __half* x, const __half* r, size_t n, float scale);
int ncfhw_to_nhwc(cudaStream_t st, const void* src, int src_is_f32, int B, int C, int F, int H, int W, __half* dst);
int nhwc_to_ncfhw(cudaStream_t st, const __half* src, int B, int C, int F, int H, int W, void* dst, int dst_is_f32);
int nchw_to_nhwc(cudaStream_t st, const __half* src, int n, int C, int H, int W, float scale, __half* dst);
int vae_latent_in(cudaStream_t st, const void* z, int z_is_f32, int nimg, int h, int w, float divisor, const float* wb, __half* out);
enum ImageFormat { IMG_SAMPLE = 0, IMG_PT = 1, IMG_NP = 2, IMG_PIL = 3 };
int image_postprocess(cudaStream_t st, const __half* x, int nimg, int H, int W, int cs, int format, void* out);
enum VaeImageSource { VAE_IN_U8_NHWC = 0, VAE_IN_F16_NCHW = 1, VAE_IN_F32_NCHW = 2 };
int vae_image_in(cudaStream_t st, const void* x, int src, int nimg, int H, int W, __half* out);
int vae_moments(cudaStream_t st, const __half* x, int nimg, int h, int w, const float* wb, __half* out);
int vae_posterior(cudaStream_t st, const __half* params, const __half* noise, int nimg, int h, int w, float scale, int layout,
                  __half* out);
int cfg_ddim_step(cudaStream_t st, const void* eps2, const void* latents, int is_f32, size_t n, int cfg,
                  float guidance, float a_t, float a_prev, void* out);
int cfg_ddim_step_dev(cudaStream_t st, const void* eps2, const void* latents, int is_f32, size_t n, int cfg,
                      float guidance, const float* d_coef, void* out);
int adapter_splat(cudaStream_t st, const float* feat, const float* tracks, const int* point_mask, int F, int P, int C,
                  int h, int w, float rate, int coord_fp16, float scale, __half* maps);

}
struct vs_comm;
namespace vs {
int comm_rank(const vs_comm* c);
int comm_size(const vs_comm* c);
int comm_all_reduce_sum_f32(vs_comm* c, cudaStream_t st, float* buf, size_t n);
int comm_all_gather(vs_comm* c, cudaStream_t st, const void* send, void* recv, size_t bytes);
int comm_all_to_all_rows(vs_comm* c, cudaStream_t st, const __half* src, __half* dst, int n_outer, size_t chunk, int gather);

int blend_mask(cudaStream_t st, const __half* const* maps, const int* map_res, int n_maps, int n_prompts, int frames, int heads,
               int words, const float* alpha, int pool, int h, int w, float threshold, int both, float* mask);
int latent_blend(cudaStream_t st, const void* x_src, void* x_tgt, const float* mask, int is_f32, int channels, int frames, int hw);

int pack_conv3x3(cudaStream_t st, const __half* w, int cout, int cin, __half* out);
int pack_conv_subpixel(cudaStream_t st, const __half* w, int cout, int cin, __half* out, bool odd_panels = false);
int upsample_conv3x3(cudaStream_t st, const __half* x, int nimg, int H, int W, int C, const __half* w3x3, const __half* wsub,
                     const float* bias, int cout, int OH, int OW, __half* out);
int pack_geglu(cudaStream_t st, const __half* w, const __half* b, int hidden, int K, int granule, __half* wout,
               float* bout);
int f16_to_f32(cudaStream_t st, const __half* x, size_t n, float* out);

}
```

videoswap_b200/csrc/runtime.cu:

```cuda
#include <stdarg.h>
#include <string.h>

#include <mutex>

#include "common.cuh"
#include "kernels.h"

namespace vs {

static thread_local char g_err[1024] = "";

void set_error(const char* fmt, ...) {
  va_list ap;
  va_start(ap, fmt);
  vsnprintf(g_err, sizeof(g_err), fmt, ap);
  va_end(ap);
}
const char* last_error() { return g_err; }

typedef CUresult (*EncodeTiledFn)(CUtensorMap*, CUtensorMapDataType, cuuint32_t, void*, const cuuint64_t*,
                                  const cuuint64_t*, const cuuint32_t*, const cuuint32_t*, CUtensorMapInterleave,
                                  CUtensorMapSwizzle, CUtensorMapL2promotion, CUtensorMapFloatOOBfill);

static EncodeTiledFn get_encode() {
  static EncodeTiledFn fn = nullptr;
  static std::once_flag once;
  std::call_once(once, [] {
    void* p = nullptr;
    cudaDriverEntryPointQueryResult q;
    if (cudaGetDriverEntryPoint("cuTensorMapEncodeTiled", &p, cudaEnableDefault, &q) == cudaSuccess &&
        q == cudaDriverEntryPointSuccess)
      fn = reinterpret_cast<EncodeTiledFn>(p);
  });
  return fn;
}

int make_tmap_f16(CUtensorMap* out, const void* base, int rank, const uint64_t* dims, const uint64_t* strides_bytes,
                  const uint32_t* box, int swizzle) {
  EncodeTiledFn enc = get_encode();
  VS_REQUIRE(enc != nullptr, "cuTensorMapEncodeTiled entry point unavailable (no CUDA driver?)");
  VS_REQUIRE((reinterpret_cast<uintptr_t>(base) & 15) == 0, "TMA base address must be 16-byte aligned");
  cuuint64_t gdim[5];
  cuuint64_t gstr[5];
  cuuint32_t bx[5];
  cuuint32_t es[5];
  for (int i = 0; i < rank; ++i) {
    gdim[i] = dims[i];
    bx[i] = box[i];
    es[i] = 1;
    if (i > 0) {
      gstr[i - 1] = strides_bytes[i - 1];
      VS_REQUIRE(gstr[i - 1] % 16 == 0, "TMA stride %d (%llu bytes) must be a multiple of 16", i,
                 (unsigned long long)gstr[i - 1]);
    }
    VS_REQUIRE(bx[i] >= 1 && bx[i] <= 256, "TMA box dim %d = %u out of range", i, bx[i]);
  }
  CUresult r = enc(out, CU_TENSOR_MAP_DATA_TYPE_FLOAT16, (cuuint32_t)rank, const_cast<void*>(base), gdim, gstr, bx, es,
                   CU_TENSOR_MAP_INTERLEAVE_NONE,
                   swizzle == 1 ? CU_TENSOR_MAP_SWIZZLE_128B : swizzle == 2 ? CU_TENSOR_MAP_SWIZZLE_64B
                   : swizzle == 3 ? CU_TENSOR_MAP_SWIZZLE_32B : CU_TENSOR_MAP_SWIZZLE_NONE,
                   CU_TENSOR_MAP_L2_PROMOTION_L2_256B, CU_TENSOR_MAP_FLOAT_OOB_FILL_NONE);
  VS_REQUIRE(r == CUDA_SUCCESS, "cuTensorMapEncodeTiled failed with CUresult %d (rank %d dims %llu,%llu box %u,%u)",
             (int)r, rank, (unsigned long long)dims[0], (unsigned long long)dims[1], box[0], box[1]);
  return 0;
}

int num_sms() {
  static int n = 0;
  if (n == 0) {
    int dev = 0;
    cudaGetDevice(&dev);
    cudaDeviceGetAttribute(&n, cudaDevAttrMultiProcessorCount, dev);
    if (n <= 0) n = 132;
  }
  return n;
}

}

#include <atomic>
#include <vector>

namespace vs {

static std::atomic<long long> g_launches{0};
static bool g_prof_on = false;
struct ProfEntry { cudaEvent_t a, b; int cat; double work; long long m; int n, k; };
static std::vector<ProfEntry> g_prof;
static std::vector<std::pair<cudaEvent_t, cudaEvent_t>> g_pool;

void count_launch(int n) { g_launches.fetch_add(n, std::memory_order_relaxed); }
long long launch_count() { return g_launches.load(); }

ProfScope::ProfScope(cudaStream_t st, int cat, double work, int nlaunch, long long m, int n, int k) : st_(st), idx_(-1) {
  count_launch(nlaunch);
  if (!g_prof_on) return;
  ProfEntry e;
  if (!g_pool.empty()) { e.a = g_pool.back().first; e.b = g_pool.back().second; g_pool.pop_back(); }
  else { cudaEventCreate(&e.a); cudaEventCreate(&e.b); }
  e.cat = cat; e.work = work; e.m = m; e.n = n; e.k = k;
  cudaEventRecord(e.a, st);
  idx_ = (int)g_prof.size();
  g_prof.push_back(e);
}
ProfScope::~ProfScope() {
  if (idx_ >= 0) cudaEventRecord(g_prof[idx_].b, st_);
}

struct Option { const char* name; int value; };
static Option g_options[] = {
    {"attn_tc", 1},
    {"gemm_stages", 0},
    {"gemm_ctas", 0},
    {"gemm_epi_slot", 1},
    {"ln_fold", 1},
    {"ln_fuse", 1},
    {"tattn_vst", 1},
    {"gn_fused", 1},
    {"gn_stats_v2", 0},
    {"subpixel", 1},
    {"pdl", 1},
};
int set_option(const char* name, int value) {
  for (Option& o : g_options)
    if (strcmp(name, o.name) == 0) { o.value = value; return 0; }
  set_error("unknown option '%s'", name);
  return 2;
}
int get_option(const char* name) {
  for (const Option& o : g_options)
    if (strcmp(name, o.name) == 0) return o.value;
  return 0;
}

int prof_dump(const char* path) {
  struct Agg { int cat; long long m; int n, k; double work, ms; long long count; };
  std::vector<Agg> aggs;
  for (auto& e : g_prof) {
    if (cudaEventSynchronize(e.b) != cudaSuccess) { set_error("profile: event sync failed"); return 1; }
    float ms = 0.f;
    cudaEventElapsedTime(&ms, e.a, e.b);
    Agg* hit = nullptr;
    for (auto& a : aggs)
      if (a.cat == e.cat && a.m == e.m && a.n == e.n && a.k == e.k && a.work == e.work) { hit = &a; break; }
    if (!hit) { aggs.push_back(Agg{e.cat, e.m, e.n, e.k, e.work, 0.0, 0}); hit = &aggs.back(); }
    hit->ms += ms;
    hit->count += 1;
  }
  FILE* f = fopen(path, "w");
  if (!f) { set_error("cannot open %s", path); return 2; }
  fprintf(f, "category,m,n,k,work_per_launch,launches,total_ms\n");
  for (auto& a : aggs) fprintf(f, "%d,%lld,%d,%d,%.6g,%lld,%.4f\n", a.cat, a.m, a.n, a.k, a.work, a.count, a.ms);
  fclose(f);
  return 0;
}

void prof_enable(bool on) { g_prof_on = on; }
void prof_reset() {
  for (auto& e : g_prof) g_pool.push_back({e.a, e.b});
  g_prof.clear();
}
int prof_collect(int cat, double* ms, double* work, long long* count) {
  double t = 0, w = 0; long long n = 0;
  for (auto& e : g_prof) {
    if (e.cat != cat) continue;
    if (cudaEventSynchronize(e.b) != cudaSuccess) { set_error("profile: event sync failed"); return 1; }
    float m = 0.f;
    cudaEventElapsedTime(&m, e.a, e.b);
    t += m; w += e.work; ++n;
  }
  *ms = t; *work = w; *count = n;
  return 0;
}

}
```

videoswap_b200/csrc/unet.cu:

```cuda
#include <math.h>
#include <string.h>

#include <functional>
#include <string>
#include <unordered_map>
#include <vector>

#include "../../include/videoswap_b200.h"
#include "common.cuh"
#include "kernels.h"

using namespace vs;

namespace {

enum LoadKind { LK_COPY_F16, LK_TO_F32, LK_CONV3, LK_CONV_UP, LK_GEGLU_W, LK_GEGLU_B, LK_IGNORE };

struct Loader {
  LoadKind kind;
  void* dst;
  int64_t numel;
  int a, b;
};

struct Lin { __half* w = nullptr; float* b = nullptr; int N = 0, K = 0; };
struct Conv3 { __half* w = nullptr; float* b = nullptr; int co = 0, ci = 0; __half* wsub = nullptr; };
struct Norm { float* g = nullptr; float* b = nullptr; int C = 0; };
struct LnLin { __half* wf = nullptr; float* u = nullptr; float* c = nullptr; float* cpe = nullptr; };
struct FoldJob { const __half* w; int N, K; const float* gamma; const float* beta; const float* bias; const float* pe; int pe_len; LnLin dst; };
struct Resnet {
  Norm n1, n2; Conv3 c1, c2; Lin sc; bool has_sc = false; int cin = 0, cout = 0; int temb_off = 0;
};
struct Transformer {
  int C = 0, layer = 0;
  Norm norm, ln1, ln2, ln3; Lin proj_in, proj_out, out1, out2, ff2;
  __half* wqkv = nullptr; __half* wq = nullptr; __half* wkv = nullptr; __half* ff1w = nullptr; float* ff1b = nullptr;
  LnLin f_qkv, f_q, f_ff;
};
struct Motion {
  int C = 0;
  Norm norm, ln[2], ff_norm; Lin proj_in, proj_out, out[2], ff2;
  __half* wqkv[2] = {nullptr, nullptr}; __half* ff1w = nullptr; float* ff1b = nullptr;
  LnLin f_qkv[2], f_ff;
};
struct Layer { Resnet res; bool has_tr = false; Transformer tr; bool has_mo = false; Motion mo; };
struct Block { std::vector<Layer> layers; bool has_sampler = false; Conv3 sampler; };

struct Act { __half* p; int c; };

}

struct vs_unet {
  vs_unet_config cfg;
  std::vector<void*> allocs;
  std::unordered_map<std::string, Loader> loaders;
  std::vector<std::string> names;
  std::vector<FoldJob> folds;
  bool folds_dirty = true;

  __half* conv_in_w = nullptr; float* conv_in_b = nullptr;
  Lin te1, te2;
  __half* tproj_w = nullptr; float* tproj_b = nullptr; int tproj_n = 0;
  Block down[4], up[4];
  Layer mid0; Resnet mid1;
  Norm norm_out; Conv3 conv_out;
  float* pe[4] = {nullptr, nullptr, nullptr, nullptr};

  size_t ws_bytes = 0; void* ws = nullptr;
  int wsB = 0, wsF = 0, wsH = 0, wsW = 0;
  int ws_pinned = 0;
  int n_groupnorms = 0;
  __half *XIN, *XN, *T, *TN, *QKV, *ATT, *HH, *SC, *P0, *P1, *SCR, *KV, *RES, *OUT;
  std::vector<__half*> skip;
  float *F_T, *F_TE0, *F_TE1, *F_EMB, *F_TPROJ, *F_SUMS, *F_LNS, *F_LNP;

  vs_comm* fcomm = nullptr;
  int fshard = 0, fnshards = 1;

  vs_attention_hook hook = nullptr; void* hook_user = nullptr; int hook_max_q = 0;
  __half* probs = nullptr; size_t probs_elems = 0;

  bool taps_on = false;
  struct Tap { std::string name; void* p; int n, h, w, c; };
  std::vector<Tap> taps;

  ~vs_unet() {
    for (void* p : allocs) cudaFree(p);
    if (ws) cudaFree(ws);
    if (probs) cudaFree(probs);
    for (auto& t : taps) cudaFree(t.p);
  }

  template <typename T>
  T* alloc(size_t n) {
    void* p = nullptr;
    if (cudaMalloc(&p, n * sizeof(T)) != cudaSuccess) { set_error("cudaMalloc of %zu bytes failed", n * sizeof(T)); return nullptr; }
    cudaMemset(p, 0, n * sizeof(T));
    allocs.push_back(p);
    return reinterpret_cast<T*>(p);
  }
  void reg(const std::string& name, LoadKind k, void* dst, int64_t numel, int a = 0, int b = 0) {
    loaders[name] = Loader{k, dst, numel, a, b};
    names.push_back(name);
  }
  float* f32(const std::string& name, int64_t n) { float* p = alloc<float>(n); reg(name, LK_TO_F32, p, n); return p; }
  __half* f16(const std::string& name, int64_t n) { __half* p = alloc<__half>(n); reg(name, LK_COPY_F16, p, n); return p; }
  Norm norm(const std::string& p, int C) { Norm n; n.C = C; n.g = f32(p + ".weight", C); n.b = f32(p + ".bias", C); return n; }
  Lin lin(const std::string& p, int N, int K, bool bias = true) {
    Lin l; l.N = N; l.K = K; l.w = f16(p + ".weight", (int64_t)N * K); if (bias) l.b = f32(p + ".bias", N); return l;
  }
  LnLin fold(const __half* w, int N, int K, const Norm& n, const float* bias, const float* pe, int pe_len) {
    LnLin f;
    if (!ln_fold_supported(K)) return f;
    f.wf = alloc<__half>((size_t)N * K);
    f.u = alloc<float>(N);
    f.c = alloc<float>(N);
    if (pe) f.cpe = alloc<float>((size_t)pe_len * N);
    folds.push_back(FoldJob{w, N, K, n.g, n.b, bias, pe, pe_len, f});
    return f;
  }
  Conv3 conv3(const std::string& p, int co, int ci) {
    Conv3 c; c.co = co; c.ci = ci;
    const int co_pad = co < 64 ? 64 : co;
    c.w = alloc<__half>((int64_t)co_pad * 9 * ci);
    reg(p + ".weight", LK_CONV3, c.w, (int64_t)co * ci * 9, co, ci);
    c.b = f32(p + ".bias", co);
    return c;
  }
};

namespace {

void build_resnet(vs_unet* h, Resnet& r, const std::string& p, int cin, int cout, int temb, int& toff) {
  r.cin = cin; r.cout = cout;
  r.n1 = h->norm(p + ".norm1", cin);
  r.c1 = h->conv3(p + ".conv1", cout, cin);
  r.temb_off = toff;
  h->reg(p + ".time_emb_proj.weight", LK_COPY_F16, h->tproj_w + (int64_t)toff * temb, (int64_t)cout * temb);
  h->reg(p + ".time_emb_proj.bias", LK_TO_F32, h->tproj_b + toff, cout);
  toff += cout;
  r.n2 = h->norm(p + ".norm2", cout);
  r.c2 = h->conv3(p + ".conv2", cout, cout);
  r.has_sc = cin != cout;
  if (r.has_sc) r.sc = h->lin(p + ".conv_shortcut", cout, cin);
}

void build_attn_fused(vs_unet* h, const std::string& p, int C, __half*& wqkv, Lin& out) {
  wqkv = h->alloc<__half>((int64_t)3 * C * C);
  h->reg(p + ".to_q.weight", LK_COPY_F16, wqkv, (int64_t)C * C);
  h->reg(p + ".to_k.weight", LK_COPY_F16, wqkv + (int64_t)C * C, (int64_t)C * C);
  h->reg(p + ".to_v.weight", LK_COPY_F16, wqkv + (int64_t)2 * C * C, (int64_t)C * C);
  out = h->lin(p + ".to_out.0", C, C);
}

void build_ff(vs_unet* h, const std::string& p, int C, __half*& w1, float*& b1, Lin& ff2) {
  w1 = h->alloc<__half>((int64_t)8 * C * C);
  b1 = h->alloc<float>(8 * C);
  h->reg(p + ".net.0.proj.weight", LK_GEGLU_W, w1, (int64_t)8 * C * C, 4 * C, C);
  h->reg(p + ".net.0.proj.bias", LK_GEGLU_B, b1, 8 * C, 4 * C, 1);
  ff2 = h->lin(p + ".net.2", C, 4 * C);
}

void build_transformer(vs_unet* h, Transformer& t, const std::string& p, int C, int ctx, int layer) {
  t.C = C; t.layer = layer;
  t.norm = h->norm(p + ".norm", C);
  t.proj_in = h->lin(p + ".proj_in", C, C);
  const std::string q = p + ".transformer_blocks.0";
  build_attn_fused(h, q + ".attn1", C, t.wqkv, t.out1);
  t.ln1 = h->norm(q + ".norm1", C);
  t.wq = h->f16(q + ".attn2.to_q.weight", (int64_t)C * C);
  t.wkv = h->alloc<__half>((int64_t)2 * C * ctx);
  h->reg(q + ".attn2.to_k.weight", LK_COPY_F16, t.wkv, (int64_t)C * ctx);
  h->reg(q + ".attn2.to_v.weight", LK_COPY_F16, t.wkv + (int64_t)C * ctx, (int64_t)C * ctx);
  t.out2 = h->lin(q + ".attn2.to_out.0", C, C);
  t.ln2 = h->norm(q + ".norm2", C);
  build_ff(h, q + ".ff", C, t.ff1w, t.ff1b, t.ff2);
  t.ln3 = h->norm(q + ".norm3", C);
  t.proj_out = h->lin(p + ".proj_out", C, C);
  t.f_qkv = h->fold(t.wqkv, 3 * C, C, t.ln1, nullptr, nullptr, 0);
  t.f_q = h->fold(t.wq, C, C, t.ln2, nullptr, nullptr, 0);
  t.f_ff = h->fold(t.ff1w, 8 * C, C, t.ln3, t.ff1b, nullptr, 0);
}

void build_motion(vs_unet* h, Motion& m, const std::string& p0, int C) {
  const std::string p = p0 + ".temporal_transformer";
  m.C = C;
  m.norm = h->norm(p + ".norm", C);
  m.proj_in = h->lin(p + ".proj_in", C, C);
  const std::string q = p + ".transformer_blocks.0";
  for (int i = 0; i < 2; ++i) {
    const std::string a = q + ".attention_blocks." + std::to_string(i);
    build_attn_fused(h, a, C, m.wqkv[i], m.out[i]);
    h->reg(a + ".processor.pos_encoder.pe", LK_IGNORE, nullptr, 0);
  }
  for (int i = 0; i < 2; ++i) m.ln[i] = h->norm(q + ".norms." + std::to_string(i), C);
  build_ff(h, q + ".ff", C, m.ff1w, m.ff1b, m.ff2);
  m.ff_norm = h->norm(q + ".ff_norm", C);
  m.proj_out = h->lin(p + ".proj_out", C, C);
  const float* pe = nullptr;
  for (int l = 0; l < 4; ++l) if (h->cfg.block_out_channels[l] == C) pe = h->pe[l];
  if (pe && h->cfg.pe_max_len <= 32) {
    for (int i = 0; i < 2; ++i) m.f_qkv[i] = h->fold(m.wqkv[i], 3 * C, C, m.ln[i], nullptr, pe, h->cfg.pe_max_len);
    m.f_ff = h->fold(m.ff1w, 8 * C, C, m.ff_norm, m.ff1b, nullptr, 0);
  }
}

int up_in_channels(const vs_unet_config& c, int i, int j, int* skip) {
  const int n = 4;
  int rev[4];
  for (int k = 0; k < n; ++k) rev[k] = c.block_out_channels[n - 1 - k];
  const int out_c = rev[i];
  const int prev = rev[i > 0 ? i - 1 : 0];
  const int in_c = rev[i + 1 < n ? i + 1 : n - 1];
  const int nl = c.layers_per_block + 1;
  *skip = (j == nl - 1) ? in_c : out_c;
  return (j == 0) ? prev : out_c;
}

}

extern "C" int vs_unet_create(const vs_unet_config* cfg, vs_unet** out) {
  VS_REQUIRE(cfg && out, "vs_unet_create: null argument");
  VS_REQUIRE(cfg->layers_per_block >= 1 && cfg->layers_per_block <= 4, "bad layers_per_block");
  for (int i = 0; i < 4; ++i)
    VS_REQUIRE(cfg->block_out_channels[i] % 64 == 0 && (cfg->block_out_channels[i] / cfg->num_heads == 40 ||
               cfg->block_out_channels[i] / cfg->num_heads == 80 || cfg->block_out_channels[i] / cfg->num_heads == 160),
               "block_out_channels[%d]=%d unsupported (need C %% 64 == 0 and head dim in {40,80,160})", i,
               cfg->block_out_channels[i]);
  VS_REQUIRE(cfg->cross_attention_dim % 64 == 0, "cross_attention_dim must be a multiple of 64");
  VS_REQUIRE(cfg->norm_num_groups >= 1 && cfg->norm_num_groups <= 32, "norm_num_groups must be in [1, 32] (statistics slices hold 32 groups)");
  vs_unet* h = new vs_unet();
  h->cfg = *cfg;
  const int* boc = cfg->block_out_channels;
  const int temb = boc[0] * 4, ctx = cfg->cross_attention_dim, lpb = cfg->layers_per_block;
  for (int l = 0; l < 4; ++l) {
    const int C = boc[l], L = cfg->pe_max_len;
    std::vector<float> t((size_t)L * C);
    for (int pos = 0; pos < L; ++pos)
      for (int i2 = 0; i2 < C; i2 += 2) {
        const float div = expf((float)i2 * (-logf(10000.0f) / (float)C));
        t[(size_t)pos * C + i2] = sinf((float)pos * div);
        if (i2 + 1 < C) t[(size_t)pos * C + i2 + 1] = cosf((float)pos * div);
      }
    h->pe[l] = h->alloc<float>((size_t)L * C);
    if (!h->pe[l]) { delete h; return 1; }
    cudaMemcpy(h->pe[l], t.data(), t.size() * sizeof(float), cudaMemcpyHostToDevice);
  }
  h->conv_in_w = h->f16("conv_in.weight", (int64_t)boc[0] * cfg->in_channels * 9);
  h->conv_in_b = h->f32("conv_in.bias", boc[0]);
  h->te1 = h->lin("time_embedding.linear_1", temb, boc[0]);
  h->te2 = h->lin("time_embedding.linear_2", temb, temb);
  int tn = 0;
  {
    int cout = boc[0];
    for (int i = 0; i < 4; ++i) { cout = boc[i]; tn += lpb * cout; }
    tn += 2 * boc[3];
    for (int i = 0; i < 4; ++i) tn += (lpb + 1) * boc[3 - i];
  }
  h->tproj_n = tn;
  h->tproj_w = h->alloc<__half>((int64_t)tn * temb);
  h->tproj_b = h->alloc<float>(tn);
  int toff = 0, layer = 0;
  int cout = boc[0];
  for (int i = 0; i < 4; ++i) {
    const int cin = cout;
    cout = boc[i];
    const std::string p = "down_blocks." + std::to_string(i);
    Block& b = h->down[i];
    b.layers.resize(lpb);
    for (int j = 0; j < lpb; ++j) {
      Layer& L = b.layers[j];
      build_resnet(h, L.res, p + ".resnets." + std::to_string(j), j == 0 ? cin : cout, cout, temb, toff);
      if (i < 3) { L.has_tr = true; build_transformer(h, L.tr, p + ".attentions." + std::to_string(j), cout, ctx, layer++); }
      if (cfg->use_motion_module && cfg->motion_down[i]) { L.has_mo = true; build_motion(h, L.mo, p + ".motion_modules." + std::to_string(j), cout); }
    }
    if (i < 3) { b.has_sampler = true; b.sampler = h->conv3(p + ".downsamplers.0.conv", cout, cout); }
  }
  build_resnet(h, h->mid0.res, "mid_block.resnets.0", boc[3], boc[3], temb, toff);
  h->mid0.has_tr = true;
  build_transformer(h, h->mid0.tr, "mid_block.attentions.0", boc[3], ctx, layer++);
  if (cfg->use_motion_module && cfg->motion_mid) { h->mid0.has_mo = true; build_motion(h, h->mid0.mo, "mid_block.motion_modules.0", boc[3]); }
  build_resnet(h, h->mid1, "mid_block.resnets.1", boc[3], boc[3], temb, toff);
  for (int i = 0; i < 4; ++i) {
    const std::string p = "up_blocks." + std::to_string(i);
    Block& b = h->up[i];
    const int oc = boc[3 - i];
    b.layers.resize(lpb + 1);
    for (int j = 0; j <= lpb; ++j) {
      Layer& L = b.layers[j];
      int skipc;
      const int run = up_in_channels(*cfg, i, j, &skipc);
      build_resnet(h, L.res, p + ".resnets." + std::to_string(j), run + skipc, oc, temb, toff);
      if (i > 0) { L.has_tr = true; build_transformer(h, L.tr, p + ".attentions." + std::to_string(j), oc, ctx, layer++); }
      if (cfg->use_motion_module && cfg->motion_up[i]) { L.has_mo = true; build_motion(h, L.mo, p + ".motion_modules." + std::to_string(j), oc); }
    }
    if (i < 3) {
      b.has_sampler = true;
      Conv3& c = b.sampler;
      c.co = oc; c.ci = oc;
      c.w = h->alloc<__half>((size_t)oc * 9 * oc + (size_t)40 * oc * oc);
      c.wsub = c.w + (size_t)oc * 9 * oc;
      h->reg(p + ".upsamplers.0.conv.weight", LK_CONV_UP, c.w, (int64_t)oc * oc * 9, oc, oc);
      c.b = h->f32(p + ".upsamplers.0.conv.bias", oc);
    }
  }
  h->norm_out = h->norm("conv_norm_out", boc[0]);
  h->conv_out = h->conv3("conv_out", cfg->out_channels, boc[0]);
  VS_REQUIRE(toff == tn, "internal: time_emb_proj stacking mismatch (%d vs %d)", toff, tn);
  {
    int n = 1 + 2 ;
    auto count = [&](const Layer& L) { n += 2 + (L.has_tr ? 1 : 0) + (L.has_mo ? 1 : 0); };
    for (int i = 0; i < 4; ++i) { for (const Layer& L : h->down[i].layers) count(L); for (const Layer& L : h->up[i].layers) count(L); }
    count(h->mid0);
    h->n_groupnorms = n;
  }
  for (void* p : h->allocs) if (!p) { delete h; return 1; }
  VS_CHECK_CUDA(cudaGetLastError());
  *out = h;
  return 0;
}

extern "C" void vs_unet_destroy(vs_unet* h) { delete h; }
extern "C" int vs_unet_num_params(const vs_unet* h) { return (int)h->names.size(); }
extern "C" const char* vs_unet_param_name(const vs_unet* h, int i) { return h->names[i].c_str(); }
extern "C" size_t vs_unet_workspace_bytes(const vs_unet* h) { return h->ws_bytes; }

extern "C" int vs_unet_load_weights(vs_unet* h, void* stream, int n, const char* const* names, const void* const* ptrs,
                                    const int64_t* numels) {
  cudaStream_t st = (cudaStream_t)stream;
  for (int i = 0; i < n; ++i) {
    auto it = h->loaders.find(names[i]);
    VS_REQUIRE(it != h->loaders.end(), "vs_unet_load_weights: unknown parameter '%s'", names[i]);
    const Loader& L = it->second;
    if (L.kind == LK_IGNORE) continue;
    VS_REQUIRE(numels[i] == L.numel, "vs_unet_load_weights: '%s' has %lld elements, expected %lld", names[i],
               (long long)numels[i], (long long)L.numel);
    const __half* src = (const __half*)ptrs[i];
    int e = 0;
    switch (L.kind) {
      case LK_COPY_F16:
        VS_CHECK_CUDA(cudaMemcpyAsync(L.dst, src, (size_t)L.numel * 2, cudaMemcpyDeviceToDevice, st));
        break;
      case LK_TO_F32: e = f16_to_f32(st, src, (size_t)L.numel, (float*)L.dst); break;
      case LK_CONV3: e = pack_conv3x3(st, src, L.a, L.b, (__half*)L.dst); break;
      case LK_CONV_UP:
        e = pack_conv3x3(st, src, L.a, L.b, (__half*)L.dst);
        if (!e) e = pack_conv_subpixel(st, src, L.a, L.b, (__half*)L.dst + (size_t)L.a * 9 * L.b, true);
        break;
      case LK_GEGLU_W: e = pack_geglu(st, src, nullptr, L.a, L.b, kGegluGranule, (__half*)L.dst, nullptr); break;
      case LK_GEGLU_B: e = pack_geglu(st, nullptr, src, L.a, 1, kGegluGranule, nullptr, (float*)L.dst); break;
      default: break;
    }
    if (e) return e;
  }
  h->folds_dirty = true;
  return 0;
}

namespace {

struct Ctx {
  vs_unet* h; cudaStream_t st;
  int B, F, NI, H, W;
  const __half* ehs; int ehs_tokens, ehs_layers;
  int gn_idx = 0;
  int place = 0;
  int ln_parts = 0;
};

inline float* next_sums(Ctx& c) {
  if (c.gn_idx >= c.h->n_groupnorms) { set_error("internal: more GroupNorm calls (%d) than statistics slices (%d)", c.gn_idx + 1, c.h->n_groupnorms); return nullptr; }
  return c.h->F_SUMS + (size_t)(c.gn_idx++) * ((size_t)c.NI * 64);
}
#define NEXT_SUMS(var) float* var = next_sums(c); if (!var) return 2

#define RUN(expr) do { if (int _e = (expr)) return _e; } while (0)

int tap(Ctx& c, const std::string& name, const __half* p, int C) {
  vs_unet* h = c.h;
  if (!h->taps_on) return 0;
  const size_t bytes = (size_t)c.NI * c.H * c.W * C * 2;
  void* d = nullptr;
  VS_CHECK_CUDA(cudaMalloc(&d, bytes));
  VS_CHECK_CUDA(cudaMemcpyAsync(d, p, bytes, cudaMemcpyDeviceToDevice, c.st));
  h->taps.push_back({name, d, c.NI, c.H, c.W, C});
  return 0;
}

int linear(Ctx& c, const __half* A, int M, const Lin& l, const __half* residual, __half* out, bool ln_out = false) {
  GemmArgs g;
  g.A = A; g.K1 = l.K; g.lda1 = l.K; g.Bw = l.w; g.M = M; g.N = l.N; g.bias = l.b;
  g.residual = residual; g.ldr = l.N; g.out = out; g.ldc = l.N;
  c.ln_parts = 0;
  if (ln_out && get_option("ln_fuse") != 0 && get_option("ln_fold") != 0 && ln_fold_supported(l.N) && l.N % 32 == 0) {
    const int parts = gemm_n_tiles(g);
    if (parts >= 1 && (long long)M * parts <= 4LL * c.NI * c.h->wsH * c.h->wsW) {
      g.ln_sums_out = c.h->F_LNP;
      c.ln_parts = parts;
    }
  }
  return gemm_tc(c.st, g);
}

int conv(Ctx& c, const __half* x, int C1, const Conv3& w, const float* rowvec, const __half* residual, __half* out) {
  GemmArgs g;
  g.A = x; g.K1 = C1; g.lda1 = C1; g.Bw = w.w; g.taps = 9; g.nimg = c.NI; g.H = c.H; g.W = c.W;
  g.M = c.NI * c.H * c.W; g.N = w.co; g.bias = w.b; g.rowvec = rowvec; g.ldrv = c.h->tproj_n; g.pix_per_batch = c.F * c.H * c.W;
  g.residual = residual; g.ldr = w.co; g.out = out; g.ldc = w.co;
  return gemm_tc(c.st, g);
}

int resnet(Ctx& c, const Resnet& r, const __half* in1, int C1, const __half* in2, int C2, __half* out) {
  vs_unet* h = c.h;
  const int hw = c.H * c.W, G = h->cfg.norm_num_groups;
  const float eps = h->cfg.norm_eps;
  VS_REQUIRE(C1 + C2 == r.cin, "internal: resnet input channels %d+%d != %d", C1, C2, r.cin);
  const int k = h->fnshards;
  NEXT_SUMS(sums);
  RUN(groupnorm_stats(c.st, in1, C1, in2, C2, c.NI, hw, c.F, G, sums, false));
  if (k > 1) RUN(comm_all_reduce_sum_f32(h->fcomm, c.st, sums, (size_t)c.B * G * 2));
  RUN(groupnorm_apply(c.st, in1, C1, in2, C2, c.NI, hw, c.F, G, sums, eps, r.n1.g, r.n1.b, true, h->XN, k));
  RUN(conv(c, h->XN, r.cin, r.c1, h->F_TPROJ + r.temb_off, nullptr, h->T));
  sums = next_sums(c);
  if (!sums) return 2;
  RUN(groupnorm_stats(c.st, h->T, r.cout, nullptr, 0, c.NI, hw, c.F, G, sums, false));
  if (k > 1) RUN(comm_all_reduce_sum_f32(h->fcomm, c.st, sums, (size_t)c.B * G * 2));
  RUN(groupnorm_apply(c.st, h->T, r.cout, nullptr, 0, c.NI, hw, c.F, G, sums, eps, r.n2.g, r.n2.b, true, h->XN, k));
  const __half* residual = in1;
  if (r.has_sc) {
    GemmArgs g;
    g.A = in1; g.K1 = C1; g.lda1 = C1; g.A2 = in2; g.K2 = C2; g.lda2 = C2; g.Bw = r.sc.w; g.M = c.NI * hw; g.N = r.cout;
    g.bias = r.sc.b; g.out = h->SC; g.ldc = r.cout;
    RUN(gemm_tc(c.st, g));
    residual = h->SC;
  } else {
    VS_REQUIRE(in2 == nullptr, "internal: concat input without shortcut conv");
  }
  RUN(conv(c, h->XN, r.cout, r.c2, nullptr, residual, out));
  return 0;
}

bool use_fold(const LnLin& f) { return f.wf != nullptr && get_option("ln_fold") != 0; }
int ln_linear(Ctx& c, const __half* x, int M, int C, const LnLin& f, int N, int mode, int hw, int pe_frames, __half* out, int ldc) {
  vs_unet* h = c.h;
  GemmArgs g;
  g.A = x; g.K1 = C; g.lda1 = C; g.Bw = f.wf; g.M = M; g.N = N; g.bias = f.c; g.ln_u = f.u;
  if (c.ln_parts > 0) {
    g.ln_parts = h->F_LNP; g.ln_nparts = c.ln_parts;
    c.ln_parts = 0;
  } else {
    RUN(ln_rowstats(c.st, x, M, C, h->F_LNS));
    g.ln_stats = h->F_LNS;
  }
  g.out = out; g.ldc = ldc; g.mode = mode;
  if (pe_frames > 0) { g.rowvec = f.cpe; g.ldrv = N; g.pix_per_batch = hw; g.rv_mod = pe_frames; }
  return gemm_tc(c.st, g);
}

int geglu_ff(Ctx& c, const __half* tn, int M, int C, const __half* w1, const float* b1, const Lin& ff2, __half* t) {
  vs_unet* h = c.h;
  GemmArgs g;
  g.A = tn; g.K1 = C; g.lda1 = C; g.Bw = w1; g.M = M; g.N = 8 * C; g.bias = b1; g.out = h->HH; g.ldc = 4 * C; g.mode = EPI_GEGLU;
  RUN(gemm_tc(c.st, g));
  return linear(c, h->HH, M, ff2, t, t);
}

int attention_hooked(Ctx& c, const Transformer& t, int is_cross, int place, const __half* q, int ldq, const __half* k, int ldk,
                     const __half* v, int ldv, __half* o, int ldo, int nq, int nk, int heads, int d, long long q_bs, long long kv_bs,
                     long long o_bs, int kv_div) {
  vs_unet* h = c.h;
  if (h->hook == nullptr || nq >= h->hook_max_q)
    return attention(c.st, q, ldq, k, ldk, v, ldv, o, ldo, c.NI, nq, nk, heads, d, q_bs, kv_bs, o_bs, kv_div);
  const size_t need = (size_t)c.NI * heads * nq * nk;
  if (need > h->probs_elems) {
    if (h->probs) { VS_CHECK_CUDA(cudaStreamSynchronize(c.st)); cudaFree(h->probs); h->probs = nullptr; }
    VS_CHECK_CUDA(cudaMalloc(&h->probs, need * sizeof(__half)));
    h->probs_elems = need;
  }
  RUN(attention_probs(c.st, q, ldq, k, ldk, h->probs, c.NI, nq, nk, heads, d, q_bs, kv_bs, kv_div));
  h->hook(h->hook_user, t.layer, is_cross, place, h->probs, c.NI, heads, nq, nk, (void*)c.st);
  return attention_apply_probs(c.st, h->probs, v, ldv, o, ldo, c.NI, nq, nk, heads, d, kv_bs, o_bs, kv_div);
}

int transformer(Ctx& c, const Transformer& t, __half* x) {
  vs_unet* h = c.h;
  const int hw = c.H * c.W, C = t.C, M = c.NI * hw, heads = h->cfg.num_heads, d = C / heads;
  NEXT_SUMS(sums);
  {
    const int e = groupnorm_frame_fused(c.st, x, C, c.NI, hw, h->cfg.norm_num_groups, 1e-6f, t.norm.g, t.norm.b, false, h->XN);
    if (e > 0) return e;
    if (e < 0) {
      RUN(groupnorm_stats(c.st, x, C, nullptr, 0, c.NI, hw, 1, h->cfg.norm_num_groups, sums, false));
      RUN(groupnorm_apply(c.st, x, C, nullptr, 0, c.NI, hw, 1, h->cfg.norm_num_groups, sums, 1e-6f, t.norm.g, t.norm.b, false, h->XN));
    }
  }
  RUN(linear(c, h->XN, M, t.proj_in, nullptr, h->T, use_fold(t.f_qkv)));
  if (use_fold(t.f_qkv)) {
    RUN(ln_linear(c, h->T, M, C, t.f_qkv, 3 * C, EPI_LINEAR, hw, 0, h->QKV, 3 * C));
  } else {
    RUN(layernorm(c.st, h->T, M, C, t.ln1.g, t.ln1.b, nullptr, 1, 1, h->TN));
    GemmArgs g; g.A = h->TN; g.K1 = C; g.lda1 = C; g.Bw = t.wqkv; g.M = M; g.N = 3 * C; g.out = h->QKV; g.ldc = 3 * C; RUN(gemm_tc(c.st, g));
  }
  RUN(attention_hooked(c, t, 0, c.place, h->QKV, 3 * C, h->QKV + C, 3 * C, h->QKV + 2 * C, 3 * C, h->ATT, C, hw, hw, heads, d,
                       (long long)hw * 3 * C, (long long)hw * 3 * C, (long long)hw * C, 1));
  RUN(linear(c, h->ATT, M, t.out1, h->T, h->T, use_fold(t.f_q)));
  if (use_fold(t.f_q)) {
    RUN(ln_linear(c, h->T, M, C, t.f_q, C, EPI_LINEAR, hw, 0, h->QKV, C));
  } else {
    RUN(layernorm(c.st, h->T, M, C, t.ln2.g, t.ln2.b, nullptr, 1, 1, h->TN));
    GemmArgs g; g.A = h->TN; g.K1 = C; g.lda1 = C; g.Bw = t.wq; g.M = M; g.N = C; g.out = h->QKV; g.ldc = C; RUN(gemm_tc(c.st, g));
  }
  {
    const int nk = c.ehs_tokens;
    const int ctx = h->cfg.cross_attention_dim;
    const int L = c.ehs_layers > 0 ? c.ehs_layers : 1;
    const int li = c.ehs_layers > 0 ? t.layer : 0;
    VS_REQUIRE(li < L, "ED-LoRA embeddings have %d layers but layer %d was requested", L, li);
    for (int b = 0; b < c.B; ++b) {
      GemmArgs g;
      g.A = c.ehs + ((long long)(b * L + li) * nk) * ctx; g.K1 = ctx; g.lda1 = ctx; g.Bw = t.wkv; g.M = nk; g.N = 2 * C;
      g.out = h->KV + (long long)b * nk * 2 * C; g.ldc = 2 * C;
      RUN(gemm_tc(c.st, g));
    }
    RUN(attention_hooked(c, t, 1, c.place, h->QKV, C, h->KV, 2 * C, h->KV + C, 2 * C, h->ATT, C, hw, nk, heads, d, (long long)hw * C,
                         (long long)nk * 2 * C, (long long)hw * C, c.F));
  }
  RUN(linear(c, h->ATT, M, t.out2, h->T, h->T, use_fold(t.f_ff)));
  if (use_fold(t.f_ff)) {
    RUN(ln_linear(c, h->T, M, C, t.f_ff, 8 * C, EPI_GEGLU, hw, 0, h->HH, 4 * C));
    RUN(linear(c, h->HH, M, t.ff2, h->T, h->T));
  } else {
    RUN(layernorm(c.st, h->T, M, C, t.ln3.g, t.ln3.b, nullptr, 1, 1, h->TN));
    RUN(geglu_ff(c, h->TN, M, C, t.ff1w, t.ff1b, t.ff2, h->T));
  }
  RUN(linear(c, h->T, M, t.proj_out, x, x));
  return 0;
}

int motion(Ctx& c, const Motion& m, int level, __half* x) {
  vs_unet* h = c.h;
  const int hw_all = c.H * c.W, C = m.C, M = c.NI * hw_all;
  const int k = h->fnshards;
  const int Ft = c.F * k;
  const int hw = hw_all / k;
  VS_REQUIRE(Ft <= h->cfg.pe_max_len, "video_length %d exceeds temporal_position_encoding_max_len %d", Ft, h->cfg.pe_max_len);
  if (k > 1) VS_REQUIRE(c.B == 1 && hw_all % k == 0, "frame sharding needs batch 1 per rank and h*w (%d) divisible by the %d shards", hw_all, k);
  NEXT_SUMS(sums);
  {
    const int e = groupnorm_frame_fused(c.st, x, C, c.NI, hw_all, 32, 1e-6f, m.norm.g, m.norm.b, false, h->XN);
    if (e > 0) return e;
    if (e < 0) {
      RUN(groupnorm_stats(c.st, x, C, nullptr, 0, c.NI, hw_all, 1, 32, sums, false));
      RUN(groupnorm_apply(c.st, x, C, nullptr, 0, c.NI, hw_all, 1, 32, sums, 1e-6f, m.norm.g, m.norm.b, false, h->XN));
    }
  }
  const __half* xin = h->XN;
  if (k > 1) {
    RUN(comm_all_to_all_rows(h->fcomm, c.st, h->XN, h->SC, c.F, (size_t)hw * C, 0));
    xin = h->SC;
  }
  RUN(linear(c, xin, M, m.proj_in, nullptr, h->T, use_fold(m.f_qkv[0])));
  for (int i = 0; i < 2; ++i) {
    if (use_fold(m.f_qkv[i])) {
      RUN(ln_linear(c, h->T, M, C, m.f_qkv[i], 3 * C, EPI_LINEAR, hw, Ft, h->QKV, 3 * C));
    } else {
      RUN(layernorm(c.st, h->T, M, C, m.ln[i].g, m.ln[i].b, h->pe[level], hw, Ft, h->TN));
      GemmArgs g; g.A = h->TN; g.K1 = C; g.lda1 = C; g.Bw = m.wqkv[i]; g.M = M; g.N = 3 * C; g.out = h->QKV; g.ldc = 3 * C; RUN(gemm_tc(c.st, g));
    }
    RUN(temporal_attention(c.st, h->QKV, h->ATT, c.B, Ft, hw, C, h->cfg.motion_num_heads));
    RUN(linear(c, h->ATT, M, m.out[i], h->T, h->T, i == 0 ? use_fold(m.f_qkv[1]) : use_fold(m.f_ff)));
  }
  if (use_fold(m.f_ff)) {
    RUN(ln_linear(c, h->T, M, C, m.f_ff, 8 * C, EPI_GEGLU, hw, 0, h->HH, 4 * C));
    RUN(linear(c, h->HH, M, m.ff2, h->T, h->T));
  } else {
    RUN(layernorm(c.st, h->T, M, C, m.ff_norm.g, m.ff_norm.b, nullptr, 1, 1, h->TN));
    RUN(geglu_ff(c, h->TN, M, C, m.ff1w, m.ff1b, m.ff2, h->T));
  }
  if (k > 1) {
    RUN(linear(c, h->T, M, m.proj_out, nullptr, h->XN));
    RUN(comm_all_to_all_rows(h->fcomm, c.st, h->XN, h->SC, c.F, (size_t)hw * C, 1));
    return add_inplace(c.st, x, h->SC, (size_t)M * C, 1.f);
  }
  RUN(linear(c, h->T, M, m.proj_out, x, x));
  return 0;
}

size_t align_up(size_t v) { return (v + 255) & ~(size_t)255; }

int ensure_workspace(vs_unet* h, int B, int F, int H, int W) {
  if (h->ws && h->wsB == B && h->wsF == F && h->wsH == H && h->wsW == W) return 0;
  const int* boc = h->cfg.block_out_channels;
  const size_t NI = (size_t)B * F;
  size_t hw[4]; int hh = H, ww = W;
  for (int l = 0; l < 4; ++l) { hw[l] = (size_t)hh * ww; hh = (hh - 1) / 2 + 1; ww = (ww - 1) / 2 + 1; }
  size_t maxC = 0, maxCat = 0;
  for (int l = 0; l < 4; ++l) {
    maxC = std::max(maxC, NI * hw[l] * boc[l]);
    maxCat = std::max(maxCat, NI * hw[l] * (size_t)(boc[l] + boc[std::min(l + 1, 3)]) );
    maxCat = std::max(maxCat, NI * hw[l] * (size_t)(2 * boc[l]));
  }
  std::vector<std::pair<__half**, size_t>> req;
  auto want = [&](__half** p, size_t elems) { req.push_back({p, elems}); };
  want(&h->XIN, NI * hw[0] * 8);
  want(&h->XN, maxCat);
  want(&h->T, maxC); want(&h->TN, maxC); want(&h->QKV, 3 * maxC); want(&h->ATT, maxC); want(&h->HH, 4 * maxC);
  size_t maxP = maxC;
  for (int l = 0; l < 3; ++l) maxP = std::max(maxP, NI * hw[l] * (size_t)boc[l + 1]);
  want(&h->SC, maxC); want(&h->P0, maxP); want(&h->P1, maxP);
  want(&h->SCR, std::max(std::max(NI * hw[1] * 9 * boc[0], 4 * maxC), (NI * hw[0] + boc[0]) * 64));
  want(&h->KV, (size_t)B * 128 * 2 * boc[3]);
  want(&h->RES, maxC);
  want(&h->OUT, NI * hw[0] * 8);
  h->skip.assign(0, nullptr);
  std::vector<size_t> skip_elems;
  skip_elems.push_back(NI * hw[0] * boc[0]);
  for (int i = 0; i < 4; ++i) {
    for (int j = 0; j < h->cfg.layers_per_block; ++j) skip_elems.push_back(NI * hw[i] * boc[i]);
    if (i < 3) skip_elems.push_back(NI * hw[i + 1] * boc[i]);
  }
  h->skip.resize(skip_elems.size());
  for (size_t i = 0; i < skip_elems.size(); ++i) want(&h->skip[i], skip_elems[i]);
  size_t total = 0;
  for (auto& r : req) total += align_up(r.second * 2);
  const int temb = boc[0] * 4;
  const size_t fl = align_up(4 * 64) + align_up((size_t)B * boc[0] * 4) + 2 * align_up((size_t)B * temb * 4) +
                    align_up((size_t)B * h->tproj_n * 4) + align_up((size_t)h->n_groupnorms * NI * 64 * 4) +
                    align_up(NI * hw[0] * 2 * 4) + align_up(NI * hw[0] * 4 * 2 * 4);
  total += fl;
  if (total > h->ws_bytes) {
    VS_REQUIRE(h->ws_pinned == 0, "vs_unet_forward: shape [%d,%d,%d,%d] needs a %zu-byte workspace but the current one "
               "(%zu bytes) is pinned by a captured CUDA graph; run the largest shape first or call "
               "vs_unet_reserve_workspace before capturing", B, F, H, W, total, h->ws_bytes);
    if (h->ws) { VS_CHECK_CUDA(cudaDeviceSynchronize()); cudaFree(h->ws); h->ws = nullptr; h->ws_bytes = 0; }
    VS_CHECK_CUDA(cudaMalloc(&h->ws, total));
    h->ws_bytes = total;
  }
  char* p = (char*)h->ws;
  for (auto& r : req) { *r.first = (__half*)p; p += align_up(r.second * 2); }
  h->F_T = (float*)p; p += align_up(4 * 64);
  h->F_TE0 = (float*)p; p += align_up((size_t)B * boc[0] * 4);
  h->F_TE1 = (float*)p; p += align_up((size_t)B * temb * 4);
  h->F_EMB = (float*)p; p += align_up((size_t)B * temb * 4);
  h->F_TPROJ = (float*)p; p += align_up((size_t)B * h->tproj_n * 4);
  h->F_SUMS = (float*)p; p += align_up((size_t)h->n_groupnorms * NI * 64 * 4);
  h->F_LNS = (float*)p; p += align_up(NI * hw[0] * 2 * 4);
  h->F_LNP = (float*)p;
  h->wsB = B; h->wsF = F; h->wsH = H; h->wsW = W;
  return 0;
}

}

extern "C" int vs_unet_set_frame_shard(vs_unet* h, vs_comm* comm, int shard, int nshards) {
  VS_REQUIRE(h != nullptr && nshards >= 1 && shard >= 0 && shard < nshards, "vs_unet_set_frame_shard: bad arguments");
  VS_REQUIRE(nshards == 1 || (comm != nullptr && comm_size(comm) == nshards && comm_rank(comm) == shard),
             "vs_unet_set_frame_shard: the communicator must have exactly one rank per shard, ranked by shard");
  h->fcomm = nshards > 1 ? comm : nullptr;
  h->fshard = shard; h->fnshards = nshards;
  return 0;
}

extern "C" int vs_unet_set_attention_hook(vs_unet* h, vs_attention_hook hook, void* user, int max_queries) {
  VS_REQUIRE(h != nullptr, "vs_unet_set_attention_hook: null handle");
  VS_REQUIRE(hook == nullptr || h->ws_pinned == 0, "attention hooks run eagerly: release the captured CUDA graph first");
  h->hook = hook; h->hook_user = user; h->hook_max_q = max_queries > 0 ? max_queries : 32 * 32;
  return 0;
}

extern "C" int vs_unet_pin_workspace(vs_unet* h, int pin) {
  VS_REQUIRE(h != nullptr, "vs_unet_pin_workspace: null handle");
  h->ws_pinned += pin ? 1 : -1;
  if (h->ws_pinned < 0) h->ws_pinned = 0;
  return 0;
}
extern "C" int vs_unet_reserve_workspace(vs_unet* h, int B, int F, int H, int W) {
  VS_REQUIRE(h && B >= 1 && F >= 1 && H >= 1 && W >= 1, "vs_unet_reserve_workspace: bad arguments");
  return ensure_workspace(h, B, F, H, W);
}

extern "C" int vs_unet_enable_taps(vs_unet* h, int enable) {
  for (auto& t : h->taps) cudaFree(t.p);
  h->taps.clear();
  h->taps_on = enable != 0;
  return 0;
}
extern "C" int vs_unet_num_taps(const vs_unet* h) { return (int)h->taps.size(); }
extern "C" int vs_unet_get_tap(const vs_unet* h, int i, const char** name, const void** p, int* n, int* hh, int* ww, int* c) {
  VS_REQUIRE(i >= 0 && i < (int)h->taps.size(), "tap index out of range");
  const auto& t = h->taps[i];
  *name = t.name.c_str(); *p = t.p; *n = t.n; *hh = t.h; *ww = t.w; *c = t.c;
  return 0;
}

extern "C" int vs_unet_copy_tap(const vs_unet* h, void* stream, int i, void* d_dst) {
  VS_REQUIRE(i >= 0 && i < (int)h->taps.size(), "tap index out of range");
  const auto& t = h->taps[i];
  VS_CHECK_CUDA(cudaMemcpyAsync(d_dst, t.p, (size_t)t.n * t.h * t.w * t.c * 2, cudaMemcpyDeviceToDevice, (cudaStream_t)stream));
  return 0;
}

namespace {

int time_embedding(const vs_unet* h, cudaStream_t st, const float* d_t, int B, float* te0, float* te1, float* emb,
                   float* proj) {
  const int c0 = h->cfg.block_out_channels[0], temb = c0 * 4;
  RUN(timestep_embedding(st, d_t, B, c0, te0));
  RUN(small_linear(st, te0, B, c0, h->te1.w, h->te1.b, temb, false, true, te1));
  RUN(small_linear(st, te1, B, temb, h->te2.w, h->te2.b, temb, false, false, emb));
  RUN(small_linear(st, emb, B, temb, h->tproj_w, h->tproj_b, h->tproj_n, true, false, proj));
  return 0;
}

int unet_run(vs_unet* h, void* stream, const void* d_sample, int io_f32, int B, int F, int H, int W, const float* d_timesteps,
             const void* d_ehs, int ehs_tokens, int ehs_layers, const void* const* d_residuals, int residuals_nhwc,
             float residual_scale, int stop_up, void* d_out) {
  VS_REQUIRE(h && d_sample && d_timesteps && d_ehs && d_out, "vs_unet_forward: null argument");
  VS_REQUIRE(B >= 1 && F >= 1 && H >= 1 && W >= 1, "vs_unet_forward: bad shape");
  VS_REQUIRE(ehs_tokens >= 1 && ehs_tokens <= 128, "vs_unet_forward: ehs_tokens out of range");
  VS_REQUIRE(h->cfg.in_channels <= 8 && h->cfg.out_channels <= 8, "in/out channels > 8 unsupported");
  VS_REQUIRE(h->fnshards == 1 || B == 1, "frame-sharded forward: one batch element per rank (got B = %d)", B);
  int lvH[4], lvW[4];
  lvH[0] = H; lvW[0] = W;
  for (int l = 1; l < 4; ++l) { lvH[l] = (lvH[l - 1] + 1) / 2; lvW[l] = (lvW[l - 1] + 1) / 2; }
  if (h->fnshards > 1) {
    for (int l = 0; l < 4; ++l)
      VS_REQUIRE((lvH[l] * lvW[l]) % h->fnshards == 0, "frame sharding needs h*w of every level divisible by the %d shards "
                 "(level %d is %dx%d)", h->fnshards, l, lvH[l], lvW[l]);
  }
  cudaStream_t st = (cudaStream_t)stream;
  RUN(ensure_workspace(h, B, F, H, W));
  if (h->folds_dirty) {
    for (const FoldJob& f : h->folds)
      RUN(ln_fold(st, f.w, f.N, f.K, f.gamma, f.beta, f.bias, f.pe, f.pe_len, f.dst.wf, f.dst.u, f.dst.c, f.dst.cpe));
    h->folds_dirty = false;
  }
  if (h->taps_on) { for (auto& t : h->taps) cudaFree(t.p); h->taps.clear(); }
  const vs_unet_config& cf = h->cfg;
  const int* boc = cf.block_out_channels;
  const int temb = boc[0] * 4, lpb = cf.layers_per_block;
  Ctx c{h, st, B, F, B * F, H, W, (const __half*)d_ehs, ehs_tokens, ehs_layers};

  VS_CHECK_CUDA(cudaMemsetAsync(h->F_SUMS, 0, (size_t)h->n_groupnorms * c.NI * 64 * sizeof(float), st));
  RUN(time_embedding(h, st, d_timesteps, B, h->F_TE0, h->F_TE1, h->F_EMB, h->F_TPROJ));

  RUN(ncfhw_to_nhwc(st, d_sample, io_f32, B, cf.in_channels, F, H, W, h->XIN));
  int si = 0;
  RUN(conv_in_3x3(st, h->XIN, c.NI, H, W, cf.in_channels, h->conv_in_w, h->conv_in_b, boc[0], h->skip[si], h->SCR));
  RUN(tap(c, "conv_in", h->skip[si], boc[0]));
  const __half* cur = h->skip[si];
  int curC = boc[0];
  std::vector<std::pair<const __half*, int>> skips;
  skips.push_back({cur, curC});
  ++si;

  for (int i = 0; i < 4; ++i) {
    const Block& blk = h->down[i];
    const __half* res_l = nullptr;
    if (d_residuals && d_residuals[i]) {
      if (residuals_nhwc) res_l = (const __half*)d_residuals[i];
      else {
        res_l = h->RES;
      }
    }
    for (int j = 0; j < lpb; ++j) {
      const Layer& L = blk.layers[j];
      __half* out = h->skip[si];
      RUN(resnet(c, L.res, cur, curC, nullptr, 0, out));
      curC = L.res.cout;
      if (L.has_tr) RUN(transformer(c, L.tr, out));
      if (L.has_mo && stop_up < 0) RUN(motion(c, L.mo, i, out));
      if (i < 3 && j == lpb - 1 && res_l) {
        const size_t n = (size_t)c.NI * c.H * c.W * curC;
        if (!residuals_nhwc) RUN(nchw_to_nhwc(st, (const __half*)d_residuals[i], c.NI, curC, c.H, c.W, residual_scale, h->RES));
        RUN(add_inplace(st, out, res_l, n, residuals_nhwc ? residual_scale : 1.f));
      }
      RUN(tap(c, "down_blocks." + std::to_string(i) + "." + std::to_string(j), out, curC));
      cur = out;
      skips.push_back({cur, curC});
      ++si;
    }
    if (blk.has_sampler) {
      const int Ho = (c.H - 1) / 2 + 1, Wo = (c.W - 1) / 2 + 1;
      RUN(im2col_s2(st, cur, c.NI, c.H, c.W, curC, h->SCR));
      GemmArgs g;
      g.A = h->SCR; g.K1 = 9 * curC; g.lda1 = 9 * curC; g.Bw = blk.sampler.w; g.M = c.NI * Ho * Wo; g.N = blk.sampler.co;
      g.bias = blk.sampler.b; g.out = h->skip[si]; g.ldc = blk.sampler.co;
      RUN(gemm_tc(st, g));
      c.H = Ho; c.W = Wo;
      cur = h->skip[si];
      skips.push_back({cur, curC});
      ++si;
    }
    if (i == 3 && res_l) {
      const size_t n = (size_t)c.NI * c.H * c.W * curC;
      if (!residuals_nhwc) RUN(nchw_to_nhwc(st, (const __half*)d_residuals[i], c.NI, curC, c.H, c.W, residual_scale, h->RES));
      VS_CHECK_CUDA(cudaMemcpyAsync(h->P0, cur, n * 2, cudaMemcpyDeviceToDevice, st));
      RUN(add_inplace(st, h->P0, res_l, n, residuals_nhwc ? residual_scale : 1.f));
      cur = h->P0;
    }
  }
  c.place = 1;
  {
    __half* o = (cur == h->P0) ? h->P1 : h->P0;
    RUN(resnet(c, h->mid0.res, cur, curC, nullptr, 0, o));
    RUN(transformer(c, h->mid0.tr, o));
    if (h->mid0.has_mo && stop_up < 0) RUN(motion(c, h->mid0.mo, 3, o));
    __half* o2 = (o == h->P0) ? h->P1 : h->P0;
    RUN(resnet(c, h->mid1, o, curC, nullptr, 0, o2));
    RUN(tap(c, "mid_block", o2, curC));
    cur = o2;
  }
  c.place = 2;
  for (int i = 0; i < 4; ++i) {
    const Block& blk = h->up[i];
    for (int j = 0; j <= lpb; ++j) {
      const Layer& L = blk.layers[j];
      const auto sk = skips.back();
      skips.pop_back();
      __half* o = (cur == h->P0) ? h->P1 : h->P0;
      RUN(resnet(c, L.res, cur, curC, sk.first, sk.second, o));
      curC = L.res.cout;
      if (L.has_tr) RUN(transformer(c, L.tr, o));
      if (L.has_mo && stop_up < 0) RUN(motion(c, L.mo, 3 - i, o));
      RUN(tap(c, "up_blocks." + std::to_string(i) + "." + std::to_string(j), o, curC));
      cur = o;
    }
    if (blk.has_sampler) {
      __half* o = (cur == h->P0) ? h->P1 : h->P0;
      const int OH = lvH[2 - i], OW = lvW[2 - i];
      if (get_option("subpixel") != 0) {
        RUN(upsample_conv3x3(st, cur, c.NI, c.H, c.W, curC, blk.sampler.w, blk.sampler.wsub, blk.sampler.b, blk.sampler.co,
                             OH, OW, o));
        c.H = OH; c.W = OW;
      } else {
        RUN(upsample_nearest2x(st, cur, c.NI, c.H, c.W, curC, h->SCR, OH, OW));
        c.H = OH; c.W = OW;
        RUN(conv(c, h->SCR, curC, blk.sampler, nullptr, nullptr, o));
      }
      cur = o;
    }
    if (i == stop_up) {
      VS_CHECK_CUDA(cudaMemcpyAsync(d_out, cur, (size_t)c.NI * c.H * c.W * curC * 2, cudaMemcpyDeviceToDevice, st));
      return 0;
    }
  }
  VS_REQUIRE(c.H == H && c.W == W, "internal: the up path ended at %dx%d, not at the input's %dx%d", c.H, c.W, H, W);
  NEXT_SUMS(osums);
  RUN(groupnorm_stats(st, cur, curC, nullptr, 0, c.NI, H * W, F, cf.norm_num_groups, osums, false));
  if (h->fnshards > 1) RUN(comm_all_reduce_sum_f32(h->fcomm, st, osums, (size_t)B * cf.norm_num_groups * 2));
  RUN(groupnorm_apply(st, cur, curC, nullptr, 0, c.NI, H * W, F, cf.norm_num_groups, osums, cf.norm_eps, h->norm_out.g, h->norm_out.b, true, h->XN,
                      h->fnshards));
  {
    GemmArgs g;
    g.A = h->XN; g.K1 = curC; g.lda1 = curC; g.Bw = h->conv_out.w; g.taps = 9; g.nimg = c.NI; g.H = H; g.W = W;
    g.M = c.NI * H * W; g.N = cf.out_channels; g.bias = h->conv_out.b; g.out = h->OUT; g.ldc = cf.out_channels;
    RUN(gemm_tc(st, g));
  }
  RUN(tap(c, "conv_out", h->OUT, cf.out_channels));
  RUN(nhwc_to_ncfhw(st, h->OUT, B, cf.out_channels, F, H, W, d_out, io_f32));
  return 0;
}

}

extern "C" int vs_unet_forward(vs_unet* h, void* stream, const void* d_sample, int io_f32, int B, int F, int H, int W,
                               const float* d_timesteps, const void* d_ehs, int ehs_tokens, int ehs_layers,
                               const void* const* d_residuals, int residuals_nhwc, float residual_scale, void* d_out) {
  return unet_run(h, stream, d_sample, io_f32, B, F, H, W, d_timesteps, d_ehs, ehs_tokens, ehs_layers, d_residuals,
                  residuals_nhwc, residual_scale, -1, d_out);
}

extern "C" int vs_unet_forward_features(vs_unet* h, void* stream, const void* d_sample, int io_f32, int B, int F, int H, int W,
                                        const float* d_timesteps, const void* d_ehs, int ehs_tokens, int ehs_layers,
                                        int up_ft_index, void* d_feat) {
  VS_REQUIRE(h && d_feat, "vs_unet_forward_features: null argument");
  VS_REQUIRE(up_ft_index >= 0 && up_ft_index <= 3, "vs_unet_forward_features: up_ft_index %d is outside 0..3", up_ft_index);
  VS_REQUIRE(h->fnshards == 1, "vs_unet_forward_features: the featurizer runs unsharded (frame sharding is set)");
  VS_REQUIRE(h->hook == nullptr, "vs_unet_forward_features: the featurizer runs without attention controllers (a hook is set)");
  return unet_run(h, stream, d_sample, io_f32, B, F, H, W, d_timesteps, d_ehs, ehs_tokens, ehs_layers, nullptr, 0, 1.f,
                  up_ft_index, d_feat);
}

extern "C" int vs_unet_time_embedding(vs_unet* h, void* stream, const float* d_timesteps, int B, float* d_emb, float* d_proj) {
  VS_REQUIRE(h && d_timesteps && d_emb && d_proj, "vs_unet_time_embedding: null argument");
  VS_REQUIRE(B >= 1, "vs_unet_time_embedding: bad batch %d", B);
  const int c0 = h->cfg.block_out_channels[0];
  VS_REQUIRE(h->tproj_n >= 5 * c0, "vs_unet_time_embedding: projections too narrow to hold the scratch rows");
  float* te0 = d_proj;
  float* te1 = d_proj + (size_t)B * c0;
  return time_embedding(h, (cudaStream_t)stream, d_timesteps, B, te0, te1, d_emb, d_proj);
}
```

videoswap_b200/ops.py:

```python
from __future__ import annotations

import ctypes as C
from typing import Optional, Sequence

import torch

from . import _lib

GEGLU_GRANULE = 128
EPI_LINEAR, EPI_GEGLU, EPI_QUICK_GELU = 0, 1, 2


def set_option(name: str, value: int):
    _lib.call("vs_set_option", name.encode(), int(value))


def _stream() -> int:
    return torch.cuda.current_stream().cuda_stream


def _p(t: Optional[torch.Tensor]):
    return None if t is None else C.c_void_p(t.data_ptr())


def _chk16(*ts):
    for t in ts:
        if t is not None:
            assert t.is_cuda and t.dtype == torch.float16 and t.is_contiguous(), "expected contiguous fp16 CUDA tensor"


def _chk32(*ts):
    for t in ts:
        if t is not None:
            assert t.is_cuda and t.dtype == torch.float32 and t.is_contiguous(), "expected contiguous fp32 CUDA tensor"


def _ptr(t: Optional[torch.Tensor]) -> int:
    return 0 if t is None else t.data_ptr()


def _out16(out, shape, device):
    if out is None:
        return torch.empty(shape, dtype=torch.float16, device=device)
    _chk16(out)
    assert tuple(out.shape) == tuple(shape), f"out has shape {tuple(out.shape)}, expected {tuple(shape)}"
    return out


def _chk_rowvec(rv, N):
    if rv is not None:
        assert rv.is_cuda and rv.dtype == torch.float32 and rv.dim() == 2 and rv.shape[1] == N and rv.stride(1) == 1, \
            "expected an fp32 [rows, N] CUDA row-vector table with unit column stride"


def max_column_tiles(N, force_bn=0):
    bn = force_bn or (64 if N <= 64 else 128)
    return -(-N // bn)


def _gemm_ex(**fields):
    d = _lib.GemmDescStruct()
    d.taps = 1
    d.pix_per_batch = 1
    for k, v in fields.items():
        setattr(d, k, v)
    _lib.call("vs_gemm_ex", _stream(), C.byref(d))


def gemm(A, W, bias=None, residual=None, A2=None, rowvec=None, pix_per_batch=1, mode=EPI_LINEAR, force_bn=0, out=None,
         ln_sums=None):
    _chk16(A, W, residual, A2)
    _chk32(bias, ln_sums)
    M, K1 = A.shape
    K2 = 0 if A2 is None else A2.shape[1]
    N = W.shape[0]
    assert W.shape[1] == K1 + K2
    _chk_rowvec(rowvec, N)
    oc = N // 2 if mode == EPI_GEGLU else N
    out = _out16(out, (M, oc), A.device)
    if ln_sums is not None:
        assert ln_sums.dim() == 3 and ln_sums.shape[1:] == (M, 2) and ln_sums.shape[0] >= max_column_tiles(N, force_bn)
    _gemm_ex(A=_ptr(A), K1=K1, lda1=K1, A2=_ptr(A2), K2=K2, lda2=K2, Bw=_ptr(W), M=M, N=N, bias=_ptr(bias),
             rowvec=_ptr(rowvec), ldrv=0 if rowvec is None else rowvec.stride(0), pix_per_batch=pix_per_batch,
             ln_sums_out=_ptr(ln_sums), residual=_ptr(residual), ldr=oc, out=_ptr(out), ldc=oc, mode=mode, force_bn=force_bn)
    return out


def pack_conv3x3(w):
    _chk16(w)
    co, ci = w.shape[:2]
    out = torch.empty((co, 9 * ci), dtype=torch.float16, device=w.device)
    _lib.call("vs_pack_conv3x3", _stream(), _p(w), co, ci, _p(out))
    return out


def pack_geglu(w, b):
    _chk16(w, b)
    hidden, K = w.shape[0] // 2, w.shape[1]
    wout = torch.empty_like(w)
    bout = torch.empty((2 * hidden,), dtype=torch.float32, device=w.device)
    _lib.call("vs_pack_geglu", _stream(), _p(w), _p(b), hidden, K, _p(wout), _p(bout))
    return wout, bout


def conv3x3(x, w_packed, bias=None, x2=None, rowvec=None, imgs_per_batch=1, residual=None, out=None):
    _chk16(x, w_packed, x2, residual)
    _chk32(bias)
    n, H, W, C1 = x.shape
    C2 = 0 if x2 is None else x2.shape[3]
    co = w_packed.shape[0]
    _chk_rowvec(rowvec, co)
    out = _out16(out, (n, H, W, co), x.device)
    _gemm_ex(A=_ptr(x), K1=C1, lda1=C1, A2=_ptr(x2), K2=C2, lda2=C2, Bw=_ptr(w_packed), M=n * H * W, N=co, taps=9, nimg=n,
             H=H, W=W, bias=_ptr(bias), rowvec=_ptr(rowvec), ldrv=0 if rowvec is None else rowvec.stride(0),
             pix_per_batch=imgs_per_batch * H * W, residual=_ptr(residual), ldr=co, out=_ptr(out), ldc=co)
    return out


def conv3x3_s2(x, w_packed, bias=None):
    _chk16(x, w_packed)
    n, H, W, Ci = x.shape
    co = w_packed.shape[0]
    Ho, Wo = (H - 1) // 2 + 1, (W - 1) // 2 + 1
    scratch = torch.empty((n * Ho * Wo, 9 * Ci), dtype=torch.float16, device=x.device)
    out = torch.empty((n, Ho, Wo, co), dtype=torch.float16, device=x.device)
    _lib.call("vs_conv3x3_s2", _stream(), _p(x), n, H, W, Ci, _p(w_packed), co, _p(bias), _p(scratch), _p(out))
    return out


def upsample_conv3x3(x, w, bias=None):
    _chk16(x, w)
    _chk32(bias)
    n, H, W, Ci = x.shape
    co = w.shape[0]
    wsub = torch.empty((16 * co * Ci,), dtype=torch.float16, device=x.device)
    out = torch.empty((n, 2 * H, 2 * W, co), dtype=torch.float16, device=x.device)
    _lib.call("vs_upsample_conv3x3", _stream(), _p(x), n, H, W, Ci, _p(w), co, _p(bias), _p(wsub), _p(out))
    return out


def pack_conv_subpixel(w):
    _chk16(w)
    co, ci = w.shape[:2]
    out = torch.empty((4, co, 4 * ci), dtype=torch.float16, device=w.device)
    _lib.call("vs_pack_conv_subpixel", _stream(), _p(w), co, ci, _p(out))
    return out


def upsample_conv3x3_packed(x, wsub, bias=None):
    _chk16(x, wsub)
    _chk32(bias)
    n, H, W, Ci = x.shape
    co = wsub.shape[1]
    assert tuple(wsub.shape) == (4, co, 4 * Ci), "expected pack_conv_subpixel panels"
    out = torch.empty((n, 2 * H, 2 * W, co), dtype=torch.float16, device=x.device)
    for par in range(4):
        _gemm_ex(A=_ptr(x), K1=Ci, lda1=Ci, Bw=_ptr(wsub[par]), M=n * H * W, N=co, taps=4, sub_py=par >> 1, sub_px=par & 1,
                 nimg=n, H=H, W=W, bias=_ptr(bias), out=_ptr(out), ldc=co)
    return out


def upsample_conv3x3_sized(x, w, bias, OH, OW, out=None):
    _chk16(x, w, out)
    _chk32(bias)
    n, H, W, Ci = x.shape
    co = w.shape[0]
    panels = torch.empty((49 * co * Ci,), dtype=torch.float16, device=x.device)
    if out is None:
        out = torch.empty((n, OH, OW, co), dtype=torch.float16, device=x.device)
    assert out.is_contiguous() and out.numel() >= n * OH * OW * co
    _lib.call("vs_upsample_conv3x3_sized", _stream(), _p(x), n, H, W, Ci, _p(w), co, _p(bias), OH, OW, _p(panels), _p(out))
    return out


def upsample_nearest(x, OH, OW):
    _chk16(x)
    n, H, W, Cc = x.shape
    out = torch.empty((n, OH, OW, Cc), dtype=torch.float16, device=x.device)
    _lib.call("vs_upsample_nearest", _stream(), _p(x), n, H, W, Cc, OH, OW, _p(out))
    return out


def groupnorm(x1, gamma, beta, groups, eps, imgs_per_set=1, silu=False, x2=None):
    _chk16(x1, x2)
    _chk32(gamma, beta)
    n, H, W, c1 = x1.shape
    c2 = 0 if x2 is None else x2.shape[3]
    sums = torch.empty((n // imgs_per_set, groups, 2), dtype=torch.float32, device=x1.device)
    out = torch.empty((n, H, W, c1 + c2), dtype=torch.float16, device=x1.device)
    _lib.call("vs_groupnorm", _stream(), _p(x1), c1, _p(x2), c2, n, H * W, imgs_per_set, groups, eps, _p(gamma), _p(beta),
              int(silu), _p(sums), _p(out))
    return out


def groupnorm_stats(x1, sums, groups, imgs_per_set, x2=None, zero_first=True):
    _chk16(x1, x2)
    _chk32(sums)
    n, H, W, c1 = x1.shape
    c2 = 0 if x2 is None else x2.shape[3]
    assert tuple(sums.shape) == (n // imgs_per_set, groups, 2)
    _lib.call("vs_groupnorm_stats", _stream(), _p(x1), c1, _p(x2), c2, n, H * W, imgs_per_set, groups, _p(sums),
              int(zero_first))
    return sums


def groupnorm_apply(x1, sums, gamma, beta, groups, eps, imgs_per_set, count_scale=1, silu=False, x2=None):
    _chk16(x1, x2)
    _chk32(sums, gamma, beta)
    n, H, W, c1 = x1.shape
    c2 = 0 if x2 is None else x2.shape[3]
    out = torch.empty((n, H, W, c1 + c2), dtype=torch.float16, device=x1.device)
    _lib.call("vs_groupnorm_apply", _stream(), _p(x1), c1, _p(x2), c2, n, H * W, imgs_per_set, groups, _p(sums), eps,
              _p(gamma), _p(beta), int(silu), int(count_scale), _p(out))
    return out


def layernorm(x, gamma, beta, pe=None, hw=1, F=1):
    _chk16(x)
    _chk32(gamma, beta, pe)
    rows, Cc = x.shape
    out = torch.empty_like(x)
    _lib.call("vs_layernorm", _stream(), _p(x), rows, Cc, _p(gamma), _p(beta), _p(pe), hw, F, _p(out))
    return out


def ln_linear(x, W, gamma, beta, bias=None, pe=None, hw=1, frames=1, mode=EPI_LINEAR):
    _chk16(x, W)
    _chk32(gamma, beta, bias, pe)
    M, Cc = x.shape
    N = W.shape[0]
    dev = x.device
    wf = torch.empty_like(W)
    u = torch.empty((N,), dtype=torch.float32, device=dev)
    c = torch.empty((N,), dtype=torch.float32, device=dev)
    cpe = torch.empty((pe.shape[0], N), dtype=torch.float32, device=dev) if pe is not None else None
    stats = torch.empty((M, 2), dtype=torch.float32, device=dev)
    out = torch.empty((M, N // 2 if mode == EPI_GEGLU else N), dtype=torch.float16, device=dev)
    _lib.call("vs_ln_linear", _stream(), _p(x), M, Cc, _p(W), _p(bias), N, _p(gamma), _p(beta), _p(pe),
              0 if pe is None else pe.shape[0], hw, frames, mode, _p(wf), _p(u), _p(c), _p(cpe), _p(stats), _p(out))
    return out


def linear_ln_linear(x0, W0, b0, W, gamma, beta, residual=None, bias=None, mode=EPI_LINEAR, pe=None, hw=1, frames=1):
    _chk16(x0, W0, W, residual)
    _chk32(b0, gamma, beta, bias, pe)
    M, K0 = x0.shape
    Cc, N = W0.shape[0], W.shape[0]
    dev = x0.device
    x = torch.empty((M, Cc), dtype=torch.float16, device=dev)
    wf = torch.empty_like(W)
    u = torch.empty((N,), dtype=torch.float32, device=dev)
    c = torch.empty((N,), dtype=torch.float32, device=dev)
    cpe = torch.empty((pe.shape[0], N), dtype=torch.float32, device=dev) if pe is not None else None
    cap = 16
    parts = torch.empty((cap, M, 2), dtype=torch.float32, device=dev)
    out = torch.empty((M, N // 2 if mode == EPI_GEGLU else N), dtype=torch.float16, device=dev)
    _lib.call("vs_linear_ln_linear", _stream(), _p(x0), M, K0, _p(W0), _p(b0), _p(residual), Cc, _p(x), _p(W), _p(bias), N,
              _p(gamma), _p(beta), _p(pe), 0 if pe is None else pe.shape[0], hw, frames, mode, _p(wf), _p(u), _p(c), _p(cpe),
              _p(parts), cap, _p(out))
    return x, out


def attention(q, k, v, heads, kv_div=1):
    B, nq, Cc = q.shape
    nk = k.shape[1]
    d = Cc // heads
    for t in (q, k, v):
        assert t.dtype == torch.float16 and t.stride(2) == 1
    out = torch.empty((B, nq, Cc), dtype=torch.float16, device=q.device)
    _lib.call("vs_attention", _stream(), _p(q), q.stride(1), _p(k), k.stride(1), _p(v), v.stride(1), _p(out), Cc, B, nq, nk,
              heads, d, q.stride(0), k.stride(0), nq * Cc, kv_div)
    return out


def attention_probs(q, k, heads, kv_div=1):
    B, nq, Cc = q.shape
    nk = k.shape[1]
    probs = torch.empty((B, heads, nq, nk), dtype=torch.float16, device=q.device)
    _lib.call("vs_attention_probs", _stream(), _p(q), q.stride(1), _p(k), k.stride(1), _p(probs), B, nq, nk, heads, Cc // heads,
              q.stride(0), k.stride(0), kv_div)
    return probs


def attention_apply_probs(probs, v, heads, kv_div=1):
    _chk16(probs)
    B, _, nq, nk = probs.shape
    Cc = v.shape[2]
    out = torch.empty((B, nq, Cc), dtype=torch.float16, device=probs.device)
    _lib.call("vs_attention_apply_probs", _stream(), _p(probs), _p(v), v.stride(1), _p(out), Cc, B, nq, nk, heads, Cc // heads,
              v.stride(0), nq * Cc, kv_div)
    return out


def scores(q, k, out):
    _chk16(q, k, out)
    nq, d = q.shape
    nk = k.shape[0]
    assert k.shape[1] == d and out.dim() == 2 and out.shape[0] == nq and out.shape[1] >= nk
    _gemm_ex(A=_ptr(q), K1=d, lda1=d, Bw=_ptr(k), M=nq, N=nk, out=_ptr(out), ldc=out.shape[1])
    return out


def softmax_rows(s, n, scale):
    _chk16(s)
    rows, ld = s.shape
    _lib.call("vs_softmax_rows", _stream(), _p(s), rows, n, ld, float(scale))
    return s


def transpose_pad(x, rows_pad, out=None):
    _chk16(x)
    rows, cols = x.shape
    out = _out16(out, (cols, rows_pad), x.device)
    _lib.call("vs_transpose_pad", _stream(), _p(x), rows, cols, rows_pad, _p(out))
    return out


def vae_latent_in(z, divisor, wb):
    assert z.is_cuda and z.dtype in (torch.float16, torch.float32) and z.is_contiguous() and z.dim() == 4 and z.shape[1] == 4, \
        "expected contiguous [n, 4, h, w] fp16 / fp32 CUDA latents"
    _chk32(wb)
    assert wb.numel() == 20
    n, _, h, w = z.shape
    out = torch.empty((n, h, w, 4), dtype=torch.float16, device=z.device)
    _lib.call("vs_vae_latent_in", _stream(), _p(z), int(z.dtype == torch.float32), n, h, w, float(divisor), _p(wb), _p(out))
    return out


IMG_SAMPLE, IMG_PT, IMG_NP, IMG_PIL = 0, 1, 2, 3


def image_postprocess(x, fmt):
    _chk16(x)
    n, H, W, Cc = x.shape
    shape = (n, 3, H, W) if fmt in (IMG_SAMPLE, IMG_PT) else (n, H, W, 3)
    dtype = {IMG_SAMPLE: torch.float16, IMG_PT: torch.float32, IMG_NP: torch.float32, IMG_PIL: torch.uint8}[fmt]
    out = torch.empty(shape, dtype=dtype, device=x.device)
    _lib.call("vs_image_postprocess", _stream(), _p(x), n, H, W, Cc, fmt, _p(out))
    return out


def downsample_conv3x3(x, w_packed, bias=None):
    _chk16(x, w_packed)
    _chk32(bias)
    n, H, W, Ci = x.shape
    co = w_packed.shape[0]
    assert w_packed.shape[1] == 9 * Ci, "expected a pack_conv3x3 panel"
    out = torch.empty((n, H // 2, W // 2, co), dtype=torch.float16, device=x.device)
    _lib.call("vs_downsample_conv3x3", _stream(), _p(x), n, H, W, Ci, _p(w_packed), co, _p(bias), _p(out))
    return out


VAE_IN_U8_NHWC, VAE_IN_F16_NCHW, VAE_IN_F32_NCHW = 0, 1, 2


def vae_image_in(x):
    assert x.is_cuda and x.is_contiguous() and x.dim() == 4, "expected a contiguous 4-D CUDA tensor"
    if x.dtype == torch.uint8:
        assert x.shape[3] == 3, "uint8 frames are [n, H, W, 3]"
        src, (n, H, W) = VAE_IN_U8_NHWC, x.shape[:3]
    else:
        assert x.dtype in (torch.float16, torch.float32) and x.shape[1] == 3, "float images are [n, 3, H, W] fp16 / fp32"
        src = VAE_IN_F16_NCHW if x.dtype == torch.float16 else VAE_IN_F32_NCHW
        n, _, H, W = x.shape
    out = torch.empty((n, H, W, 4), dtype=torch.float16, device=x.device)
    _lib.call("vs_vae_image_in", _stream(), _p(x), src, n, H, W, _p(out))
    return out


def vae_moments(x, wb):
    _chk16(x)
    _chk32(wb)
    n, h, w, Cc = x.shape
    assert Cc == 8 and wb.numel() == 72
    out = torch.empty((n, 8, h, w), dtype=torch.float16, device=x.device)
    _lib.call("vs_vae_moments", _stream(), _p(x), n, h, w, _p(wb), _p(out))
    return out


def vae_posterior(params, noise=None, scale=1.0, video=False):
    _chk16(params, noise)
    n, c8, h, w = params.shape
    assert c8 == 8 and (noise is None or tuple(noise.shape) == (n, 4, h, w))
    out = torch.empty((1, 4, n, h, w) if video else (n, 4, h, w), dtype=torch.float16, device=params.device)
    _lib.call("vs_vae_posterior", _stream(), _p(params), _p(noise), n, h, w, float(scale), int(video), _p(out))
    return out


def clip_embed(ids, tok, pos):
    _chk16(tok, pos)
    assert ids.is_cuda and ids.dtype == torch.int32 and ids.is_contiguous() and ids.dim() == 2, "expected int32 [n, L] CUDA ids"
    n, L = ids.shape
    vocab, Cc = tok.shape
    assert pos.shape[1] == Cc and pos.shape[0] >= L
    out = torch.empty((n * L, Cc), dtype=torch.float16, device=tok.device)
    _lib.call("vs_clip_embed", _stream(), _p(ids), n, L, _p(tok), vocab, _p(pos), Cc, _p(out))
    return out


def causal_attention(qkv, nseq, L, heads, out=None):
    assert qkv.is_cuda and qkv.dtype == torch.float16 and qkv.dim() == 2 and qkv.stride(1) == 1 and qkv.shape[0] == nseq * L
    Cc = qkv.shape[1] // 3
    if out is None:
        out = torch.empty((nseq * L, Cc), dtype=torch.float16, device=qkv.device)
    assert out.is_cuda and out.dtype == torch.float16 and out.stride(1) == 1 and tuple(out.shape) == (nseq * L, Cc), \
        "out: fp16 [nseq L, C] CUDA tensor with unit column stride"
    _lib.call("vs_causal_attention", _stream(), _p(qkv), qkv.stride(0), _p(out), out.stride(0), nseq, L, heads, Cc // heads)
    return out


def temporal_attention(qkv, heads):
    _chk16(qkv)
    B, F, HW, C3 = qkv.shape
    out = torch.empty((B, F, HW, C3 // 3), dtype=torch.float16, device=qkv.device)
    _lib.call("vs_temporal_attention", _stream(), _p(qkv), _p(out), B, F, HW, C3 // 3, heads)
    return out


def conv_in(x, w, bias, scratch="alloc"):
    _chk16(x, w)
    _chk32(bias)
    n, H, W, ci = x.shape
    co = w.shape[0]
    if isinstance(scratch, str):
        assert scratch == "alloc"
        scratch = torch.empty(((n * H * W + co) * 64,), dtype=torch.float16, device=x.device) if ci == 4 else None
    _chk16(scratch)
    if scratch is not None:
        assert scratch.numel() >= (n * H * W + co) * 64
    out = torch.empty((n, H, W, co), dtype=torch.float16, device=x.device)
    _lib.call("vs_conv_in", _stream(), _p(x), n, H, W, ci, _p(w), _p(bias), co, _p(scratch), _p(out))
    return out


def upsample2x(x):
    _chk16(x)
    n, H, W, Cc = x.shape
    out = torch.empty((n, 2 * H, 2 * W, Cc), dtype=torch.float16, device=x.device)
    _lib.call("vs_upsample2x", _stream(), _p(x), n, H, W, Cc, _p(out))
    return out


def ddim_coefficients(alpha_t: float, alpha_prev: float):
    import math
    c_x = math.sqrt(alpha_prev) / math.sqrt(alpha_t)
    c_e = math.sqrt(1.0 - alpha_prev) - math.sqrt(alpha_prev) * math.sqrt(1.0 - alpha_t) / math.sqrt(alpha_t)
    return c_x, c_e


def cfg_ddim_step(eps2, latents, guidance, alpha_t=None, alpha_prev=None, cfg=True, out=None, coef=None):
    assert eps2.dtype == latents.dtype and eps2.is_contiguous() and latents.is_contiguous()
    is_f32 = int(latents.dtype == torch.float32)
    if out is None:
        out = torch.empty_like(latents)
    if coef is not None:
        _chk32(coef)
        _lib.call("vs_cfg_ddim_step_dev", _stream(), _p(eps2), _p(latents), is_f32, latents.numel(), int(cfg), float(guidance),
                  _p(coef), _p(out))
        return out
    _lib.call("vs_cfg_ddim_step", _stream(), _p(eps2), _p(latents), is_f32, latents.numel(), int(cfg), float(guidance),
              float(alpha_t), float(alpha_prev), _p(out))
    return out


def adapter_level(w0, b0, w1, b1, point_embedding, tracks, h, w, rate, point_mask=None, coord_fp16=True, scale=1.0):
    _chk16(w0, b0, w1, b1)
    _chk32(point_embedding, tracks)
    mid, E = w0.shape
    Cc = w1.shape[0]
    F, P = tracks.shape[:2]
    ws = torch.empty((mid + Cc + P * (mid + Cc),), dtype=torch.float32, device=w0.device)
    out = torch.empty((F, h, w, Cc), dtype=torch.float16, device=w0.device)
    _lib.call("vs_adapter_level", _stream(), _p(w0), _p(b0), _p(w1), _p(b1), E, mid, Cc, _p(point_embedding), _p(tracks),
              _p(point_mask), F, P, h, w, float(rate), int(coord_fp16), float(scale), _p(ws), _p(out))
    return out


def dift_noise(moments, eps1, eps2, scaling_factor, sqrt_a, sqrt_1ma):
    _chk16(moments)
    _chk32(eps1, eps2)
    n, c8, h, w = moments.shape
    assert c8 == 8 and eps1.shape == eps2.shape and eps1.dim() == 4 and tuple(eps1.shape[1:]) == (4, h, w)
    assert eps1.shape[0] % n == 0, "noise rows must be a whole ensemble per frame"
    E = eps1.shape[0] // n
    out = torch.empty((n * E, 4, 1, h, w), dtype=torch.float32, device=moments.device)
    _lib.call("vs_dift_noise", _stream(), _p(moments), _p(eps1), _p(eps2), n, E, h, w, float(scaling_factor), float(sqrt_a),
              float(sqrt_1ma), _p(out))
    return out


def dift_point_sample(feat, size, xy):
    _chk16(feat)
    assert xy.is_cuda and xy.dtype == torch.int32 and xy.is_contiguous() and xy.dim() == 3 and xy.shape[2] == 2
    n, E, h, w, Cc = feat.shape
    assert xy.shape[0] == n
    P = xy.shape[1]
    out = torch.empty((n, P, Cc), dtype=torch.float32, device=feat.device)
    if P:
        _lib.call("vs_dift_point_sample", _stream(), _p(feat), n, E, h, w, Cc, int(size[0]), int(size[1]), _p(xy), P, _p(out))
    return out


def dift_ensemble_mean(feat):
    _chk16(feat)
    n, E, h, w, Cc = feat.shape
    out = torch.empty((n, Cc, h, w), dtype=torch.float32, device=feat.device)
    _lib.call("vs_dift_ensemble_mean", _stream(), _p(feat), n, E, h, w, Cc, _p(out))
    return out


def dift_point_cosine(vecs, src, src_row):
    _chk32(vecs, src)
    assert src_row.is_cuda and src_row.dtype == torch.int32 and src_row.is_contiguous()
    n, P, Cc = vecs.shape
    assert src.dim() == 2 and src.shape[1] == Cc and tuple(src_row.shape) == (n, P)
    conf = torch.empty((n, P), dtype=torch.float32, device=vecs.device)
    _lib.call("vs_dift_point_reduce", _stream(), _p(vecs), n, P, Cc, _p(src), _p(src_row), _p(conf), None, None, None, None)
    return conf


def dift_point_reduce(vecs, accept):
    _chk32(vecs)
    n, P, Cc = vecs.shape
    acc = accept.to(device=vecs.device, dtype=torch.uint8).contiguous()
    assert tuple(acc.shape) == (n, P)
    sums = torch.empty((P, Cc), dtype=torch.float32, device=vecs.device)
    means = torch.empty_like(sums)
    counts = torch.empty((P,), dtype=torch.float32, device=vecs.device)
    _lib.call("vs_dift_point_reduce", _stream(), _p(vecs), n, P, Cc, None, None, None, _p(acc), _p(sums), _p(counts), _p(means))
    return sums, counts, means
```

Baseline: 11.51.

## Fuse motion-module LN-QKV GEMM, temporal attention, and out-projection into one kernel

Adds a persistent warp-specialized Hopper kernel for the C=320, 8-head, 16-frame motion attention sublayer. It computes the LayerNorm-folded QKV projection with WGMMA from TMA-loaded weights, runs per-pixel temporal attention in registers, and applies the output projection with residual and next-LN partial sums. The aim is to avoid writing and reading the QKV and attention intermediates through global memory and to cut launches. The fused path only covers the first-level channel count, and other shapes fall back to the three-launch path, which now goes through the new wrapper.

After: 11.65, median of 6. 1.01x the previous value.

```diff
diff --git a/include/videoswap_b200.h b/include/videoswap_b200.h
--- a/include/videoswap_b200.h
+++ b/include/videoswap_b200.h
@@ -125,6 +125,10 @@
                  int ldo, int batch, int nq, int nk, int heads, int d, long long q_bstride, long long kv_bstride,
                  long long o_bstride, int kv_div);
 int vs_temporal_attention(void* stream, const void* d_qkv, void* d_o, int B, int F, int HW, int C, int heads);
+int vs_motion_attn(void* stream, void* d_x, int B, int F, int hw, int C, int heads, const void* d_wf, const float* d_c,
+                   const float* d_u, const float* d_cpe, const float* d_ln_parts, int ln_nparts, float* d_ln_stats,
+                   const void* d_wo, const float* d_bo, float* d_ln_sums_out, void* d_qkv, void* d_att);
+int vs_motion_attn_out_parts(int M, int C);
 int vs_conv_in(void* stream, const void* d_x, int nimg, int H, int W, int cin, const void* d_w, const float* d_bias,
                int cout, void* d_scratch, void* d_out);
 int vs_upsample2x(void* stream, const void* d_x, int nimg, int H, int W, int C, void* d_out);
diff --git a/videoswap_b200/_lib.py b/videoswap_b200/_lib.py
--- a/videoswap_b200/_lib.py
+++ b/videoswap_b200/_lib.py
@@ -107,6 +107,8 @@
                                  _P, _I, _P]),
     "vs_attention": (_I, [_P, _P, _I, _P, _I, _P, _I, _P, _I, _I, _I, _I, _I, _I, _LL, _LL, _LL, _I]),
     "vs_temporal_attention": (_I, [_P, _P, _P, _I, _I, _I, _I, _I]),
+    "vs_motion_attn": (_I, [_P, _P, _I, _I, _I, _I, _I, _P, _P, _P, _P, _P, _I, _P, _P, _P, _P, _P, _P]),
+    "vs_motion_attn_out_parts": (_I, [_I, _I]),
     "vs_conv_in": (_I, [_P, _P, _I, _I, _I, _I, _P, _P, _I, _P, _P]),
     "vs_upsample2x": (_I, [_P, _P, _I, _I, _I, _I, _P]),
     "vs_upsample_conv3x3": (_I, [_P, _P, _I, _I, _I, _I, _P, _I, _P, _P, _P]),
diff --git a/videoswap_b200/build.py b/videoswap_b200/build.py
--- a/videoswap_b200/build.py
+++ b/videoswap_b200/build.py
@@ -9,7 +9,7 @@
 HERE = os.path.dirname(os.path.abspath(__file__))
 CSRC = os.path.join(HERE, "csrc")
 LIB = os.path.join(HERE, "libvideoswap_b200.so")
-SOURCES = ["runtime.cu", "gemm.cu", "norm.cu", "attention.cu", "attention_tc.cu", "pointwise.cu", "unet.cu", "api.cu", "comm.cu", "text.cu", "dift.cu", "atlas.cu"]
+SOURCES = ["runtime.cu", "gemm.cu", "norm.cu", "attention.cu", "attention_tc.cu", "pointwise.cu", "unet.cu", "api.cu", "comm.cu", "text.cu", "dift.cu", "atlas.cu", "motion_block.cu"]
 ARCH = ["-gencode", "arch=compute_90a,code=sm_90a"]
 NVCC_FLAGS = ARCH + ["-lineinfo", "-O3", "-std=c++17", "-Xcompiler", "-fPIC",
               "--use_fast_math" if False else "-DVS_NO_FAST_MATH"]
diff --git a/videoswap_b200/csrc/api.cu b/videoswap_b200/csrc/api.cu
--- a/videoswap_b200/csrc/api.cu
+++ b/videoswap_b200/csrc/api.cu
@@ -186,6 +186,19 @@
 extern "C" int vs_temporal_attention(void* stream, const void* d_qkv, void* d_o, int B, int F, int HW, int C, int heads) {
   return temporal_attention((cudaStream_t)stream, (const __half*)d_qkv, (__half*)d_o, B, F, HW, C, heads);
 }
+extern "C" int vs_motion_attn(void* stream, void* d_x, int B, int F, int hw, int C, int heads, const void* d_wf,
+                              const float* d_c, const float* d_u, const float* d_cpe, const float* d_ln_parts, int ln_nparts,
+                              float* d_ln_stats, const void* d_wo, const float* d_bo, float* d_ln_sums_out, void* d_qkv,
+                              void* d_att) {
+  MotionAttnArgs a;
+  a.x = (__half*)d_x; a.B = B; a.F = F; a.hw = hw; a.C = C; a.heads = heads;
+  a.wf = (const __half*)d_wf; a.c = d_c; a.u = d_u; a.cpe = d_cpe;
+  a.ln_parts = d_ln_parts; a.ln_nparts = ln_nparts; a.ln_stats = d_ln_stats;
+  a.wo = (const __half*)d_wo; a.bo = d_bo; a.ln_sums_out = d_ln_sums_out;
+  a.qkv = (__half*)d_qkv; a.att = (__half*)d_att;
+  return motion_attn((cudaStream_t)stream, a);
+}
+extern "C" int vs_motion_attn_out_parts(int M, int C) { return motion_attn_out_parts(M, C); }
 extern "C" int vs_conv_in(void* stream, const void* d_x, int nimg, int H, int W, int cin, const void* d_w, const float* d_bias,
                           int cout, void* d_scratch, void* d_out) {
   return conv_in_3x3((cudaStream_t)stream, (const __half*)d_x, nimg, H, W, cin, (const __half*)d_w, d_bias, cout, (__half*)d_out,
diff --git a/videoswap_b200/csrc/attention.cu b/videoswap_b200/csrc/attention.cu
--- a/videoswap_b200/csrc/attention.cu
+++ b/videoswap_b200/csrc/attention.cu
@@ -1,5 +1,6 @@
 #include "common.cuh"
 #include "kernels.h"
+#include "tattn_warp.cuh"
 
 namespace vs {
 namespace {
@@ -22,16 +23,6 @@
   asm volatile("ldmatrix.sync.aligned.m8n8.x4.trans.shared.b16 {%0,%1,%2,%3}, [%4];"
                : "=r"(r0), "=r"(r1), "=r"(r2), "=r"(r3)
                : "r"(addr));
-}
-__device__ __forceinline__ void mma16816(float* c, const uint32_t* a, uint32_t b0, uint32_t b1) {
-  asm volatile(
-      "mma.sync.aligned.m16n8k16.row.col.f32.f16.f16.f32 {%0,%1,%2,%3}, {%4,%5,%6,%7}, {%8,%9}, {%0,%1,%2,%3};"
-      : "+f"(c[0]), "+f"(c[1]), "+f"(c[2]), "+f"(c[3])
-      : "r"(a[0]), "r"(a[1]), "r"(a[2]), "r"(a[3]), "r"(b0), "r"(b1));
-}
-__device__ __forceinline__ uint32_t pack_h2(float a, float b) {
-  __half2 h = __floats2half2_rn(a, b);
-  return *reinterpret_cast<uint32_t*>(&h);
 }
 
 template <int DP, int NT>
@@ -405,41 +396,10 @@
   const long long orow = (long long)p.HW * p.C;
 #pragma unroll
   for (int mt = 0; mt < MT; ++mt) {
-    float s[NT][4];
-    warp_qk<DP, NT>(s, q_s + mt * 16 * LDSB, k_s, LDSB, lane);
-    float mx0 = -INFINITY, mx1 = -INFINITY;
-#pragma unroll
-    for (int n = 0; n < NT; ++n) {
-      const int c = n * 8 + (lane & 3) * 2;
-      if (c >= p.F) s[n][0] = s[n][2] = -INFINITY;
-      if (c + 1 >= p.F) s[n][1] = s[n][3] = -INFINITY;
-      mx0 = fmaxf(mx0, fmaxf(s[n][0], s[n][1]));
-      mx1 = fmaxf(mx1, fmaxf(s[n][2], s[n][3]));
-    }
-    mx0 = fmaxf(mx0, __shfl_xor_sync(0xffffffffu, mx0, 1));
-    mx0 = fmaxf(mx0, __shfl_xor_sync(0xffffffffu, mx0, 2));
-    mx1 = fmaxf(mx1, __shfl_xor_sync(0xffffffffu, mx1, 1));
-    mx1 = fmaxf(mx1, __shfl_xor_sync(0xffffffffu, mx1, 2));
-    const float ms0 = mx0 * p.scale_log2, ms1 = mx1 * p.scale_log2;
-    float l0 = 0.f, l1 = 0.f;
-#pragma unroll
-    for (int n = 0; n < NT; ++n) {
-      s[n][0] = exp2f(s[n][0] * p.scale_log2 - ms0);
-      s[n][1] = exp2f(s[n][1] * p.scale_log2 - ms0);
-      s[n][2] = exp2f(s[n][2] * p.scale_log2 - ms1);
-      s[n][3] = exp2f(s[n][3] * p.scale_log2 - ms1);
-      l0 += s[n][0] + s[n][1];
-      l1 += s[n][2] + s[n][3];
-    }
-    l0 += __shfl_xor_sync(0xffffffffu, l0, 1);
-    l0 += __shfl_xor_sync(0xffffffffu, l0, 2);
-    l1 += __shfl_xor_sync(0xffffffffu, l1, 1);
-    l1 += __shfl_xor_sync(0xffffffffu, l1, 2);
-    float o[ON][4];
-#pragma unroll
-    for (int n = 0; n < ON; ++n) o[n][0] = o[n][1] = o[n][2] = o[n][3] = 0.f;
-    warp_pv<NT, ON>(o, s, v_s, LDSB, lane);
-    const float i0 = 1.f / l0, i1 = 1.f / l1;
+    float o[ON][4], i0, i1;
+    tattn_rows16<NT, ON>(o, i0, i1, p.F, p.scale_log2, lane,
+                         [&](float (*s)[4]) { warp_qk<DP, NT>(s, q_s + mt * 16 * LDSB, k_s, LDSB, lane); },
+                         [&](float (*o)[4], const float (*s)[4]) { warp_pv<NT, ON>(o, s, v_s, LDSB, lane); });
     const int f0 = mt * 16 + (lane >> 2), f1 = f0 + 8;
     if (VST) {
       __syncwarp();
diff --git a/videoswap_b200/csrc/kernels.h b/videoswap_b200/csrc/kernels.h
--- a/videoswap_b200/csrc/kernels.h
+++ b/videoswap_b200/csrc/kernels.h
@@ -64,6 +64,18 @@
 int set_option(const char* name, int value);
 int get_option(const char* name);
 int temporal_attention(cudaStream_t st, const __half* qkv, __half* o, int B, int F, int HW, int C, int heads);
+struct MotionAttnArgs {
+  __half* x = nullptr;
+  int B = 0, F = 0, hw = 0, C = 0, heads = 0;
+  const __half* wf = nullptr; const float* c = nullptr; const float* u = nullptr; const float* cpe = nullptr;
+  const float* ln_parts = nullptr; int ln_nparts = 0;
+  float* ln_stats = nullptr;
+  const __half* wo = nullptr; const float* bo = nullptr;
+  float* ln_sums_out = nullptr;
+  __half* qkv = nullptr; __half* att = nullptr;
+};
+int motion_attn(cudaStream_t st, const MotionAttnArgs& a);
+int motion_attn_out_parts(int M, int C);
 int softmax_rows(cudaStream_t st, __half* s, int rows, int n, int ld, float scale);
 int transpose_pad(cudaStream_t st, const __half* src, int rows, int cols, int rows_pad, __half* dst);
 
diff --git a/videoswap_b200/csrc/motion_block.cu b/videoswap_b200/csrc/motion_block.cu
--- /dev/null
+++ b/videoswap_b200/csrc/motion_block.cu
@@ -0,0 +1,399 @@
+#include "common.cuh"
+#include "kernels.h"
+#include "tattn_warp.cuh"
+
+namespace vs {
+namespace {
+
+constexpr int MB_C = 320, MB_D = 40, MB_HEADS = 8, MB_F = 16, MB_KB = MB_C / 64;
+constexpr int MB_THREADS = 384;
+constexpr int MB_X_BYTES = 64 * MB_C * 2;
+constexpr int MB_KB_BYTES = 64 * 128;
+constexpr int MB_QKV_TX = 3 * MB_D * 128;
+constexpr int MB_STAGE = 160 * 128;
+constexpr int MB_STAGES = (227 * 1024 - 1024 - 256 - 2 * MB_X_BYTES) / MB_STAGE;
+constexpr int MB_SMEM = 2 * MB_X_BYTES + MB_STAGES * MB_STAGE + 1024 + 256;
+constexpr int MB_BLOCKS = MB_HEADS * MB_KB + 2 * MB_KB;
+static_assert(MB_STAGES >= 4 && MB_SMEM <= 227 * 1024, "shared memory");
+
+struct MotionBlockParams {
+  CUtensorMap tmX, tmWqkv, tmWo;
+  int B, hw, npg, units, tiles;
+  const float* c; const float* u; const float* cpe;
+  const float2* ln_stats; const float2* ln_parts; int ln_nparts; float ln_inv_c;
+  const float* bo;
+  float2* ln_sums_out; int out_bn;
+  __half* x;
+  long long M;
+  float scale_log2;
+};
+
+#define MB_R8(i) "+f"(d[i]), "+f"(d[i + 1]), "+f"(d[i + 2]), "+f"(d[i + 3]), "+f"(d[i + 4]), "+f"(d[i + 5]), "+f"(d[i + 6]), "+f"(d[i + 7])
+__device__ __forceinline__ void wgmma_n120_ss(float* d, uint64_t da, uint64_t db, uint32_t scale_d) {
+  asm volatile(
+      "{\n\t.reg .pred p;\n\tsetp.ne.b32 p, %62, 0;\n\t"
+      "wgmma.mma_async.sync.aligned.m64n120k16.f32.f16.f16 "
+      "{%0,%1,%2,%3,%4,%5,%6,%7,%8,%9,%10,%11,%12,%13,%14,%15,%16,%17,%18,%19,%20,%21,%22,%23,%24,%25,%26,%27,%28,%29,"
+      "%30,%31,%32,%33,%34,%35,%36,%37,%38,%39,%40,%41,%42,%43,%44,%45,%46,%47,%48,%49,%50,%51,%52,%53,%54,%55,%56,%57,"
+      "%58,%59}, %60, %61, p, 1, 1, 0, 0;\n\t}"
+      : MB_R8(0), MB_R8(8), MB_R8(16), MB_R8(24), MB_R8(32), MB_R8(40), MB_R8(48), "+f"(d[56]), "+f"(d[57]), "+f"(d[58]),
+        "+f"(d[59])
+      : "l"(da), "l"(db), "r"(scale_d));
+}
+__device__ __forceinline__ void wgmma_n160_rs(float* d, const uint32_t* a, uint64_t db, uint32_t scale_d) {
+  asm volatile(
+      "{\n\t.reg .pred p;\n\tsetp.ne.b32 p, %85, 0;\n\t"
+      "wgmma.mma_async.sync.aligned.m64n160k16.f32.f16.f16 "
+      "{%0,%1,%2,%3,%4,%5,%6,%7,%8,%9,%10,%11,%12,%13,%14,%15,%16,%17,%18,%19,%20,%21,%22,%23,%24,%25,%26,%27,%28,%29,"
+      "%30,%31,%32,%33,%34,%35,%36,%37,%38,%39,%40,%41,%42,%43,%44,%45,%46,%47,%48,%49,%50,%51,%52,%53,%54,%55,%56,%57,"
+      "%58,%59,%60,%61,%62,%63,%64,%65,%66,%67,%68,%69,%70,%71,%72,%73,%74,%75,%76,%77,%78,%79}, "
+      "{%80,%81,%82,%83}, %84, p, 1, 1, 0;\n\t}"
+      : MB_R8(0), MB_R8(8), MB_R8(16), MB_R8(24), MB_R8(32), MB_R8(40), MB_R8(48), MB_R8(56), MB_R8(64), MB_R8(72)
+      : "r"(a[0]), "r"(a[1]), "r"(a[2]), "r"(a[3]), "l"(db), "r"(scale_d));
+}
+#undef MB_R8
+
+__device__ __forceinline__ uint32_t movmatrix_t(uint32_t a) {
+  uint32_t d;
+  asm volatile("movmatrix.sync.aligned.m8n8.trans.b16 %0, %1;" : "=r"(d) : "r"(a));
+  return d;
+}
+__device__ __forceinline__ uint32_t x_off(int row, int col) {
+  return (uint32_t)((col >> 6) * MB_KB_BYTES + row * 128 + ((((col & 63) >> 3) ^ (row & 7)) << 4) + (col & 7) * 2);
+}
+
+__global__ void __launch_bounds__(MB_THREADS, 1) motion_block_kernel(const __grid_constant__ MotionBlockParams p) {
+  extern __shared__ uint8_t smem_raw[];
+  const uint32_t smem_base = (smem_u32(smem_raw) + 1023u) & ~1023u;
+  const uint32_t ring_base = smem_base + 2 * MB_X_BYTES;
+  const uint32_t bar_base = ring_base + MB_STAGES * MB_STAGE;
+  auto full_bar = [&](int s) { return bar_base + 8u * s; };
+  auto empty_bar = [&](int s) { return bar_base + 8u * (MB_STAGES + s); };
+  auto x_full = [&](int g) { return bar_base + 8u * (2 * MB_STAGES + g); };
+  auto x_empty = [&](int g) { return bar_base + 8u * (2 * MB_STAGES + 2 + g); };
+  const int warp = threadIdx.x >> 5, lane = threadIdx.x & 31, wg = threadIdx.x >> 7;
+
+  if (threadIdx.x == 0) {
+    prefetch_tmap(&p.tmX);
+    prefetch_tmap(&p.tmWqkv);
+    prefetch_tmap(&p.tmWo);
+    for (int s = 0; s < MB_STAGES; ++s) {
+      mbar_init(full_bar(s), 1);
+      mbar_init(empty_bar(s), 8);
+    }
+    for (int g = 0; g < 2; ++g) {
+      mbar_init(x_full(g), 1);
+      mbar_init(x_empty(g), 4);
+    }
+    fence_barrier_init();
+  }
+  __syncthreads();
+  pdl_trigger();
+  pdl_wait();
+
+  if (wg == 0) {
+    setmaxnreg_dec<40>();
+    if (warp == 1) {
+      for (int t = blockIdx.x, j = 0; t < p.tiles; t += gridDim.x, ++j) {
+        for (int g = 0; g < 2; ++g) {
+          mbar_wait(x_empty(g), (uint32_t)(j & 1) ^ 1u);
+          if (elect_one()) {
+            const int unit = 2 * t + g;
+            const int b = unit < p.units ? unit / p.npg : p.B, pix0 = unit < p.units ? (unit % p.npg) * 4 : 0;
+            const uint32_t dst = smem_base + (uint32_t)g * MB_X_BYTES;
+            mbar_expect_tx(x_full(g), MB_X_BYTES);
+            for (int kb = 0; kb < MB_KB; ++kb) tma_load_4d(dst + kb * MB_KB_BYTES, &p.tmX, x_full(g), kb * 64, 0, pix0, b);
+          }
+          __syncwarp();
+        }
+      }
+      return;
+    }
+    if (warp != 0) return;
+    uint32_t s = 0, ph = 0;
+    for (int t = blockIdx.x; t < p.tiles; t += gridDim.x) {
+      for (int blk = 0; blk < MB_BLOCKS; ++blk) {
+        mbar_wait(empty_bar(s), ph ^ 1);
+        if (elect_one()) {
+          const uint32_t dst = ring_base + s * MB_STAGE, fb = full_bar(s);
+          if (blk < MB_HEADS * MB_KB) {
+            const int h = blk / MB_KB, kb = blk % MB_KB;
+            mbar_expect_tx(fb, MB_QKV_TX);
+            for (int part = 0; part < 3; ++part)
+              tma_load_2d(dst + part * (MB_D * 128), &p.tmWqkv, fb, kb * 64, part * MB_C + h * MB_D);
+          } else {
+            const int n = (blk - MB_HEADS * MB_KB) / MB_KB, kb = (blk - MB_HEADS * MB_KB) % MB_KB;
+            mbar_expect_tx(fb, MB_STAGE);
+            tma_load_2d(dst, &p.tmWo, fb, kb * 64, n * 160);
+          }
+        }
+        __syncwarp();
+        if (++s == (uint32_t)MB_STAGES) { s = 0; ph ^= 1; }
+      }
+    }
+    return;
+  }
+
+  setmaxnreg_inc<232>();
+  const int g = wg - 1, wq = warp & 3, q = lane & 3, r8 = lane >> 2;
+  const uint32_t xs = smem_base + (uint32_t)g * MB_X_BYTES;
+  const uint8_t* xg = smem_raw + (xs - smem_u32(smem_raw));
+  uint32_t s = 0, ph = 0;
+  for (int t = blockIdx.x, j = 0; t < p.tiles; t += gridDim.x, ++j) {
+    const int unit = 2 * t + g;
+    const int b = unit / p.npg, pix = (unit % p.npg) * 4 + wq;
+    const bool valid = unit < p.units && pix < p.hw;
+    long long m[2];
+    float la[2] = {1.f, 1.f}, lb[2] = {0.f, 0.f};
+#pragma unroll
+    for (int h = 0; h < 2; ++h) {
+      m[h] = ((long long)b * MB_F + r8 + 8 * h) * p.hw + pix;
+      if (!valid) continue;
+      if (p.ln_nparts > 0) {
+        float S = 0.f, Q = 0.f;
+        for (int k = 0; k < p.ln_nparts; ++k) {
+          const float2 v = __ldg(p.ln_parts + (long long)k * p.M + m[h]);
+          S += v.x; Q += v.y;
+        }
+        const float mean = S * p.ln_inv_c;
+        la[h] = rsqrtf(fmaxf(fmaf(-mean, mean, Q * p.ln_inv_c), 0.f) + 1e-5f);
+        lb[h] = -mean * la[h];
+      } else {
+        const float2 st2 = __ldg(p.ln_stats + m[h]);
+        la[h] = st2.x; lb[h] = st2.y;
+      }
+    }
+    mbar_wait(x_full(g), (uint32_t)j & 1u);
+
+    uint32_t att[MB_C / 8][2];
+#pragma unroll
+    for (int hd = 0; hd < MB_HEADS; ++hd) {
+      float acc[60];
+      uint32_t prev = 0;
+#pragma unroll
+      for (int kb = 0; kb < MB_KB; ++kb) {
+        mbar_wait(full_bar(s), ph);
+        wgmma_fence();
+        const uint64_t da = gmma_desc_sw128(xs + kb * MB_KB_BYTES), db = gmma_desc_sw128(ring_base + s * MB_STAGE);
+#pragma unroll
+        for (int k = 0; k < 4; ++k) wgmma_n120_ss(acc, da + 2 * k, db + 2 * k, (kb | k) != 0 ? 1u : 0u);
+        wgmma_commit();
+        if (kb > 0) {
+          wgmma_wait<1>();
+          if (lane == 0) mbar_arrive(empty_bar(prev));
+        }
+        prev = s;
+        if (++s == (uint32_t)MB_STAGES) { s = 0; ph ^= 1; }
+      }
+      wgmma_wait<0>();
+      if (lane == 0) mbar_arrive(empty_bar(prev));
+      uint32_t f16[15][2];
+#pragma unroll
+      for (int jt = 0; jt < 15; ++jt) {
+        const int n = (jt / 5) * MB_C + hd * MB_D + (jt % 5) * 8 + 2 * q;
+        const float2 c2 = __ldg(reinterpret_cast<const float2*>(p.c + n));
+        const float2 u2 = __ldg(reinterpret_cast<const float2*>(p.u + n));
+#pragma unroll
+        for (int h = 0; h < 2; ++h) {
+          const float2 r2 = __ldg(reinterpret_cast<const float2*>(p.cpe + (r8 + 8 * h) * (3 * MB_C) + n));
+          float f0 = fmaf(la[h], acc[4 * jt + 2 * h], fmaf(lb[h], u2.x, c2.x));
+          float f1 = fmaf(la[h], acc[4 * jt + 2 * h + 1], fmaf(lb[h], u2.y, c2.y));
+          f0 += r2.x; f1 += r2.y;
+          f16[jt][h] = pack_h2(f0, f1);
+        }
+      }
+      float o[6][4], i0, i1;
+      tattn_rows16<2, 6>(
+          o, i0, i1, MB_F, p.scale_log2, lane,
+          [&](float (*sc)[4]) {
+#pragma unroll
+            for (int n = 0; n < 2; ++n) sc[n][0] = sc[n][1] = sc[n][2] = sc[n][3] = 0.f;
+#pragma unroll
+            for (int kk = 0; kk < 3; ++kk) {
+              const bool hi = 2 * kk + 1 < 5;
+              const uint32_t a[4] = {f16[2 * kk][0], f16[2 * kk][1], hi ? f16[2 * kk + 1][0] : 0u, hi ? f16[2 * kk + 1][1] : 0u};
+#pragma unroll
+              for (int n = 0; n < 2; ++n)
+                mma16816(sc[n], a, f16[5 + 2 * kk][n], hi ? f16[5 + 2 * kk + 1][n] : 0u);
+            }
+          },
+          [&](float (*oo)[4], const float (*sc)[4]) {
+            const uint32_t a[4] = {pack_h2(sc[0][0], sc[0][1]), pack_h2(sc[0][2], sc[0][3]), pack_h2(sc[1][0], sc[1][1]),
+                                   pack_h2(sc[1][2], sc[1][3])};
+#pragma unroll
+            for (int n = 0; n < 6; ++n) {
+              const uint32_t b0 = n < 5 ? movmatrix_t(f16[10 + n][0]) : 0u, b1 = n < 5 ? movmatrix_t(f16[10 + n][1]) : 0u;
+              mma16816(oo[n], a, b0, b1);
+            }
+          });
+#pragma unroll
+      for (int n = 0; n < 5; ++n) {
+        att[5 * hd + n][0] = pack_h2(o[n][0] * i0, o[n][1] * i0);
+        att[5 * hd + n][1] = pack_h2(o[n][2] * i1, o[n][3] * i1);
+      }
+    }
+
+    float rs[2] = {0.f, 0.f}, rq[2] = {0.f, 0.f};
+#pragma unroll
+    for (int nh = 0; nh < 2; ++nh) {
+      float acc[80];
+      uint32_t prev = 0;
+#pragma unroll
+      for (int kb = 0; kb < MB_KB; ++kb) {
+        mbar_wait(full_bar(s), ph);
+        wgmma_fence();
+        const uint64_t db = gmma_desc_sw128(ring_base + s * MB_STAGE);
+#pragma unroll
+        for (int k = 0; k < 4; ++k) {
+          const int kk = 4 * kb + k;
+          const uint32_t a[4] = {att[2 * kk][0], att[2 * kk][1], att[2 * kk + 1][0], att[2 * kk + 1][1]};
+          wgmma_n160_rs(acc, a, db + 2 * k, (kb | k) != 0 ? 1u : 0u);
+        }
+        wgmma_commit();
+        if (kb > 0) {
+          wgmma_wait<1>();
+          if (lane == 0) mbar_arrive(empty_bar(prev));
+        }
+        prev = s;
+        if (++s == (uint32_t)MB_STAGES) { s = 0; ph ^= 1; }
+      }
+      wgmma_wait<0>();
+      if (lane == 0) mbar_arrive(empty_bar(prev));
+#pragma unroll
+      for (int jt = 0; jt < 20; ++jt) {
+        const int col = nh * 160 + 8 * jt + 2 * q;
+        const float2 b2 = __ldg(reinterpret_cast<const float2*>(p.bo + col));
+#pragma unroll
+        for (int h = 0; h < 2; ++h) {
+          float f0 = acc[4 * jt + 2 * h], f1 = acc[4 * jt + 2 * h + 1];
+          f0 += b2.x; f1 += b2.y;
+          const __half2 hv = __floats2half2_rn(f0, f1);
+          __half2* px = reinterpret_cast<__half2*>(const_cast<uint8_t*>(xg) + x_off(16 * wq + r8 + 8 * h, col));
+          *px = __hadd2(hv, *px);
+        }
+      }
+      __syncwarp();
+#pragma unroll
+      for (int sb = 0; sb < 5; ++sb) {
+        const int col0 = nh * 160 + sb * 32;
+#pragma unroll
+        for (int h = 0; h < 2; ++h) {
+          const uint4 ov = *reinterpret_cast<const uint4*>(xg + x_off(16 * wq + r8 + 8 * h, col0 + 8 * q));
+          if (valid) *reinterpret_cast<uint4*>(p.x + m[h] * MB_C + col0 + 8 * q) = ov;
+          if (p.ln_sums_out != nullptr) {
+            const __half2* oh = reinterpret_cast<const __half2*>(&ov);
+            const float2 a = __half22float2(oh[0]), b2 = __half22float2(oh[1]), c2 = __half22float2(oh[2]), d2 = __half22float2(oh[3]);
+            rs[h] += ((a.x + a.y) + (b2.x + b2.y)) + ((c2.x + c2.y) + (d2.x + d2.y));
+            const float q0 = fmaf(a.x, a.x, a.y * a.y), q1 = fmaf(b2.x, b2.x, b2.y * b2.y);
+            const float q2 = fmaf(c2.x, c2.x, c2.y * c2.y), q3 = fmaf(d2.x, d2.x, d2.y * d2.y);
+            rq[h] += (q0 + q1) + (q2 + q3);
+          }
+        }
+        const int end = col0 + 32;
+        if (p.ln_sums_out != nullptr && (end % p.out_bn == 0 || end == MB_C)) {
+          const int slice = col0 / p.out_bn;
+#pragma unroll
+          for (int h = 0; h < 2; ++h) {
+            rs[h] += __shfl_xor_sync(0xffffffffu, rs[h], 1); rq[h] += __shfl_xor_sync(0xffffffffu, rq[h], 1);
+            rs[h] += __shfl_xor_sync(0xffffffffu, rs[h], 2); rq[h] += __shfl_xor_sync(0xffffffffu, rq[h], 2);
+            if (q == 0 && valid) p.ln_sums_out[(long long)slice * p.M + m[h]] = make_float2(rs[h], rq[h]);
+            rs[h] = 0.f; rq[h] = 0.f;
+          }
+        }
+      }
+    }
+    fence_proxy_async();
+    __syncwarp();
+    if (lane == 0) mbar_arrive(x_empty(g));
+  }
+}
+
+}
+
+int motion_attn_out_parts(int M, int C) {
+  GemmArgs g;
+  g.M = M; g.N = C; g.K1 = C;
+  return gemm_n_tiles(g);
+}
+
+namespace {
+
+int motion_attn_fused(cudaStream_t st, const MotionAttnArgs& a, const float* stats) {
+  MotionBlockParams p;
+  memset(&p, 0, sizeof(p));
+  const long long M = (long long)a.B * MB_F * a.hw;
+  p.B = a.B; p.hw = a.hw; p.npg = (a.hw + 3) / 4; p.units = a.B * p.npg; p.tiles = (p.units + 1) / 2;
+  p.c = a.c; p.u = a.u; p.cpe = a.cpe;
+  p.ln_stats = reinterpret_cast<const float2*>(stats);
+  p.ln_parts = reinterpret_cast<const float2*>(a.ln_parts);
+  p.ln_nparts = a.ln_parts ? a.ln_nparts : 0;
+  p.ln_inv_c = 1.f / (float)MB_C;
+  p.bo = a.bo;
+  p.ln_sums_out = reinterpret_cast<float2*>(a.ln_sums_out);
+  if (a.ln_sums_out) {
+    const int parts = motion_attn_out_parts((int)M, MB_C);
+    VS_REQUIRE(parts == 2 || parts == 3, "motion_attn: unsupported number of statistics slices %d", parts);
+    p.out_bn = parts == 2 ? 160 : 128;
+  }
+  p.x = a.x; p.M = M;
+  p.scale_log2 = 1.4426950408889634f / sqrtf((float)MB_D);
+  {
+    const uint64_t dims[4] = {(uint64_t)MB_C, (uint64_t)MB_F, (uint64_t)a.hw, (uint64_t)a.B};
+    const uint64_t str[3] = {(uint64_t)a.hw * MB_C * 2, (uint64_t)MB_C * 2, (uint64_t)MB_F * a.hw * MB_C * 2};
+    const uint32_t box[4] = {64, MB_F, 4, 1};
+    if (make_tmap_f16(&p.tmX, a.x, 4, dims, str, box, 1)) return 3;
+  }
+  {
+    const uint64_t dims[2] = {(uint64_t)MB_C, (uint64_t)(3 * MB_C)};
+    const uint64_t str[1] = {(uint64_t)MB_C * 2};
+    const uint32_t box[2] = {64, MB_D};
+    if (make_tmap_f16(&p.tmWqkv, a.wf, 2, dims, str, box, 1)) return 3;
+  }
+  {
+    const uint64_t dims[2] = {(uint64_t)MB_C, (uint64_t)MB_C};
+    const uint64_t str[1] = {(uint64_t)MB_C * 2};
+    const uint32_t box[2] = {64, 160};
+    if (make_tmap_f16(&p.tmWo, a.wo, 2, dims, str, box, 1)) return 3;
+  }
+  static bool configured = false;
+  if (!configured) {
+    VS_CHECK_CUDA(cudaFuncSetAttribute(motion_block_kernel, cudaFuncAttributeMaxDynamicSharedMemorySize, MB_SMEM));
+    configured = true;
+  }
+  const double flops = 2.0 * M * MB_C * 4 * MB_C + 4.0 * M * MB_F * MB_C;
+  ProfScope prof(st, PC_GEMM, flops, 1, M, 4 * MB_C, MB_C);
+  const int ctas = p.tiles < num_sms() ? p.tiles : num_sms();
+  return launch_pdl(motion_block_kernel, dim3(ctas), dim3(MB_THREADS), MB_SMEM, st, 1, p);
+}
+
+}
+
+int motion_attn(cudaStream_t st, const MotionAttnArgs& a) {
+  VS_REQUIRE(a.x && a.wf && a.c && a.u && a.cpe && a.wo && a.bo, "motion_attn: null pointer");
+  VS_REQUIRE(a.B >= 1 && a.F >= 1 && a.hw >= 1 && a.heads >= 1 && a.C % a.heads == 0, "motion_attn: bad shape");
+  VS_REQUIRE(a.ln_parts ? a.ln_nparts >= 1 : a.ln_stats != nullptr, "motion_attn: no row statistics for the LayerNorm");
+  const long long Ml = (long long)a.B * a.F * a.hw;
+  VS_REQUIRE(Ml < (1LL << 30), "motion_attn: too many rows");
+  const int M = (int)Ml, C = a.C;
+  const float* stats = nullptr;
+  if (!a.ln_parts) {
+    if (int e = ln_rowstats(st, a.x, M, C, a.ln_stats)) return e;
+    stats = a.ln_stats;
+  }
+  if (get_option("motion_fuse") != 0 && C == MB_C && a.heads == MB_HEADS && a.F == MB_F) return motion_attn_fused(st, a, stats);
+  VS_REQUIRE(a.qkv && a.att, "motion_attn: the three-launch path needs q|k|v and attention scratch");
+  GemmArgs g;
+  g.A = a.x; g.K1 = C; g.lda1 = C; g.Bw = a.wf; g.M = M; g.N = 3 * C; g.bias = a.c; g.ln_u = a.u;
+  if (a.ln_parts) { g.ln_parts = a.ln_parts; g.ln_nparts = a.ln_nparts; }
+  else g.ln_stats = stats;
+  g.out = a.qkv; g.ldc = 3 * C;
+  g.rowvec = a.cpe; g.ldrv = 3 * C; g.pix_per_batch = a.hw; g.rv_mod = a.F;
+  if (int e = gemm_tc(st, g)) return e;
+  if (int e = temporal_attention(st, a.qkv, a.att, a.B, a.F, a.hw, C, a.heads)) return e;
+  GemmArgs o;
+  o.A = a.att; o.K1 = C; o.lda1 = C; o.Bw = a.wo; o.M = M; o.N = C; o.bias = a.bo;
+  o.residual = a.x; o.ldr = C; o.out = a.x; o.ldc = C; o.ln_sums_out = a.ln_sums_out;
+  return gemm_tc(st, o);
+}
+
+}
diff --git a/videoswap_b200/csrc/runtime.cu b/videoswap_b200/csrc/runtime.cu
--- a/videoswap_b200/csrc/runtime.cu
+++ b/videoswap_b200/csrc/runtime.cu
@@ -115,6 +115,7 @@
     {"gemm_epi_slot", 1},
     {"ln_fold", 1},
     {"ln_fuse", 1},
+    {"motion_fuse", 1},
     {"tattn_vst", 1},
     {"gn_fused", 1},
     {"gn_stats_v2", 0},
diff --git a/videoswap_b200/csrc/tattn_warp.cuh b/videoswap_b200/csrc/tattn_warp.cuh
--- /dev/null
+++ b/videoswap_b200/csrc/tattn_warp.cuh
@@ -0,0 +1,57 @@
+#pragma once
+#include "common.cuh"
+
+namespace vs {
+
+__device__ __forceinline__ void mma16816(float* c, const uint32_t* a, uint32_t b0, uint32_t b1) {
+  asm volatile(
+      "mma.sync.aligned.m16n8k16.row.col.f32.f16.f16.f32 {%0,%1,%2,%3}, {%4,%5,%6,%7}, {%8,%9}, {%0,%1,%2,%3};"
+      : "+f"(c[0]), "+f"(c[1]), "+f"(c[2]), "+f"(c[3])
+      : "r"(a[0]), "r"(a[1]), "r"(a[2]), "r"(a[3]), "r"(b0), "r"(b1));
+}
+__device__ __forceinline__ uint32_t pack_h2(float a, float b) {
+  __half2 h = __floats2half2_rn(a, b);
+  return *reinterpret_cast<uint32_t*>(&h);
+}
+
+template <int NT, int ON, class QK, class PV>
+__device__ __forceinline__ void tattn_rows16(float (*o)[4], float& i0, float& i1, int F, float scale_log2, int lane, QK qk,
+                                             PV pv) {
+  float s[NT][4];
+  qk(s);
+  float mx0 = -INFINITY, mx1 = -INFINITY;
+#pragma unroll
+  for (int n = 0; n < NT; ++n) {
+    const int c = n * 8 + (lane & 3) * 2;
+    if (c >= F) s[n][0] = s[n][2] = -INFINITY;
+    if (c + 1 >= F) s[n][1] = s[n][3] = -INFINITY;
+    mx0 = fmaxf(mx0, fmaxf(s[n][0], s[n][1]));
+    mx1 = fmaxf(mx1, fmaxf(s[n][2], s[n][3]));
+  }
+  mx0 = fmaxf(mx0, __shfl_xor_sync(0xffffffffu, mx0, 1));
+  mx0 = fmaxf(mx0, __shfl_xor_sync(0xffffffffu, mx0, 2));
+  mx1 = fmaxf(mx1, __shfl_xor_sync(0xffffffffu, mx1, 1));
+  mx1 = fmaxf(mx1, __shfl_xor_sync(0xffffffffu, mx1, 2));
+  const float ms0 = mx0 * scale_log2, ms1 = mx1 * scale_log2;
+  float l0 = 0.f, l1 = 0.f;
+#pragma unroll
+  for (int n = 0; n < NT; ++n) {
+    s[n][0] = exp2f(s[n][0] * scale_log2 - ms0);
+    s[n][1] = exp2f(s[n][1] * scale_log2 - ms0);
+    s[n][2] = exp2f(s[n][2] * scale_log2 - ms1);
+    s[n][3] = exp2f(s[n][3] * scale_log2 - ms1);
+    l0 += s[n][0] + s[n][1];
+    l1 += s[n][2] + s[n][3];
+  }
+  l0 += __shfl_xor_sync(0xffffffffu, l0, 1);
+  l0 += __shfl_xor_sync(0xffffffffu, l0, 2);
+  l1 += __shfl_xor_sync(0xffffffffu, l1, 1);
+  l1 += __shfl_xor_sync(0xffffffffu, l1, 2);
+#pragma unroll
+  for (int n = 0; n < ON; ++n) o[n][0] = o[n][1] = o[n][2] = o[n][3] = 0.f;
+  pv(o, s);
+  i0 = 1.f / l0;
+  i1 = 1.f / l1;
+}
+
+}
diff --git a/videoswap_b200/csrc/unet.cu b/videoswap_b200/csrc/unet.cu
--- a/videoswap_b200/csrc/unet.cu
+++ b/videoswap_b200/csrc/unet.cu
@@ -537,6 +537,27 @@
   return 0;
 }
 
+int motion_attn_block(Ctx& c, const Motion& m, int i, int M, int hw, int Ft, bool ln_out) {
+  vs_unet* h = c.h;
+  const int C = m.C;
+  MotionAttnArgs a;
+  a.x = h->T; a.B = M / (Ft * hw); a.F = Ft; a.hw = hw; a.C = C; a.heads = h->cfg.motion_num_heads;
+  a.wf = m.f_qkv[i].wf; a.c = m.f_qkv[i].c; a.u = m.f_qkv[i].u; a.cpe = m.f_qkv[i].cpe;
+  if (c.ln_parts > 0) { a.ln_parts = h->F_LNP; a.ln_nparts = c.ln_parts; }
+  else a.ln_stats = h->F_LNS;
+  a.wo = m.out[i].w; a.bo = m.out[i].b;
+  a.qkv = h->QKV; a.att = h->ATT;
+  c.ln_parts = 0;
+  if (ln_out && get_option("ln_fuse") != 0 && get_option("ln_fold") != 0 && ln_fold_supported(C) && C % 32 == 0) {
+    const int parts = motion_attn_out_parts(M, C);
+    if (parts >= 1 && (long long)M * parts <= 4LL * c.NI * h->wsH * h->wsW) {
+      a.ln_sums_out = h->F_LNP;
+      c.ln_parts = parts;
+    }
+  }
+  return motion_attn(c.st, a);
+}
+
 int motion(Ctx& c, const Motion& m, int level, __half* x) {
   vs_unet* h = c.h;
   const int hw_all = c.H * c.W, C = m.C, M = c.NI * hw_all;
@@ -561,14 +582,15 @@
   }
   RUN(linear(c, xin, M, m.proj_in, nullptr, h->T, use_fold(m.f_qkv[0])));
   for (int i = 0; i < 2; ++i) {
+    const bool ln_out = i == 0 ? use_fold(m.f_qkv[1]) : use_fold(m.f_ff);
     if (use_fold(m.f_qkv[i])) {
-      RUN(ln_linear(c, h->T, M, C, m.f_qkv[i], 3 * C, EPI_LINEAR, hw, Ft, h->QKV, 3 * C));
-    } else {
-      RUN(layernorm(c.st, h->T, M, C, m.ln[i].g, m.ln[i].b, h->pe[level], hw, Ft, h->TN));
-      GemmArgs g; g.A = h->TN; g.K1 = C; g.lda1 = C; g.Bw = m.wqkv[i]; g.M = M; g.N = 3 * C; g.out = h->QKV; g.ldc = 3 * C; RUN(gemm_tc(c.st, g));
-    }
+      RUN(motion_attn_block(c, m, i, M, hw, Ft, ln_out));
+      continue;
+    }
+    RUN(layernorm(c.st, h->T, M, C, m.ln[i].g, m.ln[i].b, h->pe[level], hw, Ft, h->TN));
+    GemmArgs g; g.A = h->TN; g.K1 = C; g.lda1 = C; g.Bw = m.wqkv[i]; g.M = M; g.N = 3 * C; g.out = h->QKV; g.ldc = 3 * C; RUN(gemm_tc(c.st, g));
     RUN(temporal_attention(c.st, h->QKV, h->ATT, c.B, Ft, hw, C, h->cfg.motion_num_heads));
-    RUN(linear(c, h->ATT, M, m.out[i], h->T, h->T, i == 0 ? use_fold(m.f_qkv[1]) : use_fold(m.f_ff)));
+    RUN(linear(c, h->ATT, M, m.out[i], h->T, h->T, ln_out));
   }
   if (use_fold(m.f_ff)) {
     RUN(ln_linear(c, h->T, M, C, m.f_ff, 8 * C, EPI_GEGLU, hw, 0, h->HH, 4 * C));
diff --git a/videoswap_b200/ops.py b/videoswap_b200/ops.py
--- a/videoswap_b200/ops.py
+++ b/videoswap_b200/ops.py
@@ -417,6 +417,26 @@
     return out
 
 
+def motion_attn_out_parts(M, C):
+    return int(_lib.lib().vs_motion_attn_out_parts(int(M), int(C)))
+
+
+def motion_attn(x, heads, wf, c, u, cpe, wo, bo, ln_parts=None, ln_stats=None, ln_sums_out=None, qkv=None, att=None):
+    _chk16(x, wf, wo)
+    B, F, hw, Cc = x.shape
+    M = B * F * hw
+    if qkv is None:
+        qkv = torch.empty((M, 3 * Cc), dtype=torch.float16, device=x.device)
+    if att is None:
+        att = torch.empty((M, Cc), dtype=torch.float16, device=x.device)
+    if ln_parts is None and ln_stats is None:
+        ln_stats = torch.empty((M, 2), dtype=torch.float32, device=x.device)
+    n = 0 if ln_parts is None else ln_parts.shape[0]
+    _lib.call("vs_motion_attn", _stream(), _p(x), B, F, hw, Cc, heads, _p(wf), _p(c), _p(u), _p(cpe), _p(ln_parts), n,
+              _p(ln_stats), _p(wo), _p(bo), _p(ln_sums_out), _p(qkv), _p(att))
+    return x
+
+
 def conv_in(x, w, bias, scratch="alloc"):
     _chk16(x, w)
     _chk32(bias)
```
